# Qervas/cn_chess_ai

Measured on AMD Instinct MI355X. Metric: env steps/sec + DQN updates/sec at 8192 parallel games, 1/2/4/8 MI355X, higher is better.
Workload: dtype f32

## Files before the change

### cn_chess_ai_amd/csrc/xq_dqn.hip

```cpp
#include "xq_internal.h"
#include <hip/hip_ext.h>
#include "xq_gemm.hip.h"
#include "xq_screen.hip.h"
#include "xq_gemm_dma.hip.h"
#include "xq_l0grad.hip.h"

#include <algorithm>
#include <cfloat>
#include <cmath>
#include <limits>
#include <mutex>
#include <random>
#include <unordered_map>

struct TdStep; struct ScreenPlan;
namespace xq {
struct TailArgs; struct ClipRecord; struct TdStatsRecord; struct ShadowJob;
struct Screen {
    int mode = XQ_QMAX_FULL;
    int refine_stage = -1;
    DevBuf<uint16_t> wb;
    DevBuf<uint16_t> ab;
    DevBuf<float> p1, p2;
    DevBuf<float> R, na;
    DevBuf<unsigned> wmax;
    int static_net = -1;
    DevBuf<unsigned long long> stats;
    int stat_blocks = 0;
    unsigned long long carry[2] = {0, 0};
    unsigned long long host_steps = 0, host_samples = 0;
    PinnedBuf<unsigned long long> guard_host;
    Event guard_ev;
    bool guard_pending = false;
    unsigned long long guard_samples = 0, guard_queued_at = 0;
    bool stage_whole = false;
    unsigned long long seen[3] = {0, 0, 0};
    int hold = 0;
    bool rebase = false;
    unsigned long long fallbacks = 0;
    void set_mode(int m) { mode = m; hold = 0; }
    void rows_rewritten(int net) { if (static_net == net) static_net = -1; }
    int reserve(int NO, int Hl, int n, const void* params, const void* acts);
    void totals_of(const unsigned long long* h, unsigned long long sums[2]) const;  int totals(unsigned long long sums[2]) const;
    void guard_decide(const unsigned long long totals[2]);  int guard_tick(bool* screened);  int guard_queue(int n, hipStream_t s);
    int shadow_job(const xq_dqn* d, int sel_net, int parity, hipStream_t s, ShadowJob* shadow);
    int plan(xq_dqn* d, const TdStep& s, ScreenPlan* P);
};
}
struct xq_dqn {
    int ns = 0, nl = 0;
    int L[XQ_MAX_LAYERS + 1] = {0};
    size_t nw = 0, nb = 0;
    size_t wo[XQ_MAX_LAYERS] = {0}, bo[XQ_MAX_LAYERS] = {0};
    double lr = 1e-3, gamma = 0.99;
    uint64_t seed = 0;
    xq::Stream stream;
    xq::Stream side;
    hipStream_t cur = nullptr;
    int ncu = 256;
    xq::Event ev_fork, ev_join, ev_delta;
    xq::Event ev_qmax;
    xq::DevBuf<float> params[2];
    uint64_t params_version = 0;
    int precision = XQ_PRECISION_F32;
    xq::DevBuf<uint16_t> params_bf[2];
    xq::DevBuf<uint16_t> acts_bf[XQ_MAX_LAYERS];
    xq::DevBuf<uint16_t> tacts_bf[2];
    xq::DevBuf<uint16_t> t2acts_bf[2];
    xq::DevBuf<uint16_t> sel_acts_bf[XQ_MAX_LAYERS];
    xq::DevBuf<uint16_t> deltas_bf[XQ_MAX_LAYERS];
    xq::DevBuf<float> t2acts[2];
    xq::DevBuf<int> partial_idx;
    xq::DevBuf<float> acts[XQ_MAX_LAYERS];
    xq::DevBuf<float> tacts[2];
    xq::DevBuf<float> deltas[XQ_MAX_LAYERS];
    xq::DevBuf<float> dsc;
    xq::DevBuf<int32_t> act_mb;
    xq::DevBuf<float> q90;
    xq::DevBuf<float> sel_acts[XQ_MAX_LAYERS];
    xq::DevBuf<float> sel_q90;
    struct SelKeep {
        xq::DevBuf<float> z1;  xq::DevBuf<uint32_t> prev_boards;
        bool valid = false;  const uint32_t* boards = nullptr;  int n = 0;
        int calls = 0;  bool pays = false;
    } sel_keep[2];
    void sel_invalidate() { sel_keep[0].valid = sel_keep[1].valid = false; }
    xq::DevBuf<float> qh_slabs[2];
    bool small_tiles = false;
    bool l0_derive = false;
    xq::Screen scr;
    xq::DevBuf<float> partial;
    xq::DevBuf<float> zmax;  xq::DevBuf<int> zidx;
    xq::DevBuf<float> qsa, yv, lossv;
    xq::DevBuf<uint32_t> gboards;
    int last_n = 0;
    xq::DevBuf<float> grads_td;  size_t n_grads_td = 0;
    size_t g_w0 = 0, g_wh[XQ_MAX_LAYERS] = {0}, g_wout = 0, g_bh[XQ_MAX_LAYERS] = {0}, g_bout = 0;
    xq::DevBuf<float> grads_full;
    int opt_kind = XQ_OPT_SGD;
    double opt_b1 = 0.9, opt_b2 = 0.999, opt_eps = 1e-8;
    uint64_t opt_t = 0;
    xq::DevBuf<float> adam_m, adam_v;
    double clip_max_norm = 0.0;
    xq::DevBuf<double> clip_partials;
    xq::DevBuf<xq::ClipRecord> clip_rec;
    double target_tau = 0.0;
    bool tgt_rest_synced = false;
    int loss_kind = XQ_LOSS_SQUARED;
    double loss_kappa = 1.0;
    float loss_kappa32 = 1.0f;
    xq::DevBuf<xq::TdStatsRecord> td_stats_rec;
    xq::DevBuf<float> slabs;
    xq::DevBuf<float> slabs_l0;
    xq::DevBuf<uint16_t> l0_planes;
    xq::DevBuf<uint16_t> l0_sel;
    bool l0_split_done = false;
    bool l0_sel_done = false;
    bool l0_mfma = true;
    xq_comm* comm = nullptr;
    bool fused_apply = false;
    struct PendingSlab { const float* src = nullptr; int nslabs = 0; long long stride = 0; };
    PendingSlab pend_w0, pend_hidden[XQ_MAX_LAYERS], pend_wout, pend_bout, pend_bh;
    xq::DevBuf<float> bias_work;
    xq::DevBuf<float> xdense, qfull, tfull;
    xq::DevBuf<uint32_t> hb;
    xq::DevBuf<int32_t> ha;  xq::DevBuf<float> hr;  xq::DevBuf<uint8_t> hd;
    xq::DevBuf<uint32_t> ns_boards, ns_next;
    xq::DevBuf<int32_t> ns_action, ns_m, ns_first, ns_last;
    xq::DevBuf<float> ns_reward;
    xq::DevBuf<uint8_t> ns_done;
    int nstep_rows = 0;
    xq::DevBuf<uint8_t> ns_flag;
    int mirror_rows = 0;
    xq::DevBuf<uint8_t> ns_cflag;
    int colour_swap_rows = 0;
    bool colour_swap_sided = false;
    int bootstrap = XQ_BOOTSTRAP_ALL;
    xq::DevBuf<float> z96, z96_slabs;
    xq::DevBuf<int> legal_nmoves;
    xq::DevBuf<uint8_t> hside, ns_side;
    int legal_rows = 0;
    int zero_sum = 0;
    int view = XQ_VIEW_ABSOLUTE;
    xq::DevBuf<uint8_t> ns_vflag, ns_vflag_next;
    int view_rows = 0;
    xq::Profiler prof;
    xq::TailArgs* tail = nullptr;
    bool tail_open = false;
    bool td_tail = true;
    int exchange_overlap = -1;
    bool late_gate = false;
    bool exch_calibrated = false, exch_late = false;
    double exch_allreduce_us = 0.0, exch_threshold_us = 0.0;
    size_t tail_lds = 0;  double tail_flops = 0, tail_bytes = 0;

    bool fused() const { return fused_apply && comm == nullptr; }
    bool bf16() const { return precision != XQ_PRECISION_F32; }
    bool bf16_bwd() const { return precision == XQ_PRECISION_BF16_FULL; }
    uint16_t* wl_bf(int net, int l) const { return params_bf[net] + (l == 0 ? 0 : (size_t)L[0] * L[1] + (wo[l] - wo[1])); }
    float* w0t(int net) const { return params[net]; }
    float* wrest(int net) const { return params[net] + (size_t)L[0] * L[1]; }
    float* wl(int net, int l) const { return l == 0 ? w0t(net) : wrest(net) + (wo[l] - wo[1]); }
    float* bl(int net, int l) const { return params[net] + nw + bo[l]; }
    int nout() const { return L[nl]; }
    int hlast() const { return L[nl - 1]; }
};

namespace xq {

Profiler* dqn_profiler(xq_dqn* d) { return &d->prof; }
int dqn_fused_apply(const xq_dqn* d) { return d->fused_apply ? 1 : 0; }
int dqn_view(const xq_dqn* d) { return d->view; }
xq_comm* dqn_comm(const xq_dqn* d) { return d->comm; }
hipStream_t dqn_stream(xq_dqn* d) { return d->stream; }
void dqn_shape(const xq_dqn* d, int* n_in, int* n_out) { *n_in = d->L[0]; *n_out = d->nout(); }
hipEvent_t dqn_qmax_event(xq_dqn* d) { return d->ev_qmax; }
uint64_t dqn_params_version(const xq_dqn* d) { return d->params_version; }

struct ProfScope {
    Profiler& p; hipStream_t s; int h; double flops, bytes;
    ProfScope(xq_dqn* d, const char* name, double fl, double by, bool attach = false) : p(d->prof), s(d->cur), flops(fl), bytes(by) {
        h = -1;
        if (!name || d->tail_open || !p.enabled) return;
        if (d->cur != d->stream && d->cur != d->side) {
            char nm[48];
            snprintf(nm, sizeof nm, "%s@select", name);
            h = p.begin(nm, s, attach);
        } else {
            h = p.begin(name, s, attach);
        }
    }
    hipEvent_t start() const { return h >= 0 ? p.recs[h].a : nullptr; }
    hipEvent_t stop() const { return h >= 0 ? p.recs[h].b : nullptr; }
    ~ProfScope() { p.end(h, s, flops, bytes); }
};

struct LaunchNow {
    xq_dqn* d; bool was_open;
    explicit LaunchNow(xq_dqn* d_) : d(d_), was_open(d_->tail_open) { d->tail_open = false; }
    ~LaunchNow() { d->tail_open = was_open; }
};
struct OnStream {
    xq_dqn* d; hipStream_t was;
    OnStream(xq_dqn* d_, hipStream_t s) : d(d_), was(d_->cur) { d->cur = s; }
    ~OnStream() { d->cur = was; }
};
struct SmallTiles {
    xq_dqn* d; bool was;
    SmallTiles(xq_dqn* d_, bool small) : d(d_), was(d_->small_tiles) { d->small_tiles = small; }
    ~SmallTiles() { d->small_tiles = was; }
};

}

#include "xq_l0.hip.h"
#include "xq_tail.hip.h"
#include "xq_refine.hip.h"
#include "xq_nstep.hip.h"
#include "xq_mirror.hip.h"
#include "xq_colour_swap.hip.h"
#include "xq_view.hip.h"
#include "xq_legal.hip.h"

namespace xq {

static inline int vec_ok(const void* p, long long ld) { return (((uintptr_t)p) % 16 == 0) && (ld % 4 == 0); }

template <int AL, int BL, int EPI, int DT = DT_F32>
static int launch_gemm(xq_dqn* d, GemmArgs g, int splits, const char* name, int* used_splits = nullptr, bool force_small = false) {
    if (used_splits) *used_splits = 0;
    if (g.M <= 0 || g.N <= 0 || g.K <= 0) return fail(XQ_ERR_INVALID_ARGUMENT, "empty GEMM %s (%d x %d x %d)", name, g.M, g.N, g.K);
    g.a_vec = vec_ok(g.A, g.lda);
    g.b_vec = vec_ok(g.B, g.ldb);
    if (splits < 1) splits = 1;
    g.k_chunk = round_up((g.K + splits - 1) / splits, GBK);
    splits = (g.K + g.k_chunk - 1) / g.k_chunk;
    if (splits < 1) splits = 1;
    const int groups = g.grouped > 1 ? g.grouped : 1;
    const long long t128 = (long long)((g.M + 127) / 128) * ((g.N + 127) / 128) * (g.grouped ? groups : splits);
    const bool big = (!force_small && !d->small_tiles && t128 >= 512);
    const double kk = DT == DT_BF16 ? 2.0 * g.K : (double)g.K;
    if (d->tail_open) {
        TailArgs& T = *d->tail;
        const bool is_delta = AL == L_KCONTIG && BL == L_MCONTIG && EPI == EPI_DELTA, is_grad = AL == L_MCONTIG && BL == L_MCONTIG && EPI == EPI_STORE;
        if (DT != DT_F32 || big || g.grouped || !(is_delta || is_grad) || (is_delta && (T.n_delta || splits != 1)) || (is_grad && T.n_grad))
            return fail(XQ_ERR_RUNTIME, "GEMM %s cannot join the fused tail launch", name);
        const int gx = (g.M + 63) / 64, gy = (g.N + 63) / 64;
        if (is_delta) { T.delta = g; T.delta_gx = gx; T.n_delta = gx * gy; }
        else { T.grad = g; T.grad_gx = gx; T.grad_gy = gy; T.n_grad = gx * gy * splits; }
        d->tail_flops += 2.0 * g.M * g.N * kk;
        d->tail_bytes += 4.0 * ((double)g.M * g.K + (double)g.N * g.K + (double)g.M * g.N);
        d->tail_lds = std::max(d->tail_lds, 2 * (size_t)g_tile_floats(64) * sizeof(float));
        if (used_splits) *used_splits = splits;
        return XQ_OK;
    }
    ProfScope ps(d, name, 2.0 * g.M * g.N * kk, 4.0 * ((double)g.M * g.K + (double)g.N * g.K + (double)g.M * g.N));
    if (g.grouped) {
        if (splits != 1) return fail(XQ_ERR_INVALID_ARGUMENT, "grouped GEMM cannot be split-K");
        if (groups > 3) return fail(XQ_ERR_INVALID_ARGUMENT, "at most 3 grouped products");
        for (int k = 0; k + 1 < groups; ++k) {
            g.b_vec = g.b_vec && vec_ok(g.Bx[k], g.ldb);
            g.a_vec = g.a_vec && vec_ok(g.Ax[k], g.lda);
        }
        ps.flops *= groups; ps.bytes *= groups;
    }
    const int gz = g.grouped ? groups : splits;
    if (big) {
        dim3 grid((g.M + 127) / 128, (g.N + 127) / 128, gz);
        hipLaunchKernelGGL((gemm_f32_kernel<AL, BL, EPI, 2, 2, DT>), grid, dim3(256), 0, d->cur, g);
    } else {
        dim3 grid((g.M + 63) / 64, (g.N + 63) / 64, gz);
        hipLaunchKernelGGL((gemm_f32_kernel<AL, BL, EPI, 1, 1, DT>), grid, dim3(256), 0, d->cur, g);
    }
    XQ_HIP(hipGetLastError());
    if (used_splits) *used_splits = splits;
    return XQ_OK;
}

static int ensure_max_dynamic_lds(const void* kernel, int bytes) {
    static std::mutex m;
    static std::unordered_map<const void*, int> granted;
    std::lock_guard<std::mutex> lock(m);
    int& have = granted[kernel];
    if (have >= bytes) return XQ_OK;
    XQ_HIP(hipFuncSetAttribute(kernel, hipFuncAttributeMaxDynamicSharedMemorySize, bytes));
    have = bytes;
    return XQ_OK;
}
template <class F> static int ensure_max_dynamic_lds(F* kernel, int bytes) { return ensure_max_dynamic_lds(reinterpret_cast<const void*>(kernel), bytes); }

template <int DT, int AL, int BL, int EPI, int TI, int TJ>
static int launch_dma_gemm(xq_dqn* d, const Bf16GemmArgs& g, int gz, const char* name) {
    constexpr int lds = bg_lds_bytes(TI, TJ);
    XQ_TRY(ensure_max_dynamic_lds(gemm_dma_kernel<DT, AL, BL, EPI, TI, TJ>, lds));
    const int groups = g.groups > 1 ? g.groups : 1;
    const double es = DT == DT_F32 ? 4.0 : 2.0;
    ProfScope ps(d, name, 2.0 * g.M * g.N * (double)g.K * groups, es * groups * ((double)g.M * g.K + (double)g.N * g.K + 2.0 * g.M * g.N));
    hipLaunchKernelGGL((gemm_dma_kernel<DT, AL, BL, EPI, TI, TJ>), dim3(g.M / (128 * TI), g.N / (64 * TJ), gz), dim3(512), lds, d->cur, g);
    XQ_HIP(hipGetLastError());
    return XQ_OK;
}
template <int AL, int BL, int EPI>
static int launch_bf16_gemm(xq_dqn* d, const Bf16GemmArgs& g, int gz, const char* name) {
    return launch_dma_gemm<DT_BF16, AL, BL, EPI, 2, 2>(d, g, gz, name);
}

template <class T> static int reserve_zeroed(DevBuf<T>& b, size_t count, hipStream_t s) {
    bool grew = false;
    XQ_TRY(b.reserve(count, &grew));
    if (grew) XQ_HIP(hipMemsetAsync(b, 0, count * sizeof(T), s));
    return XQ_OK;
}

static int ensure_capacity(xq_dqn* d, int n) {
    const size_t cap = (size_t)n;
    int maxh = 0;
    for (int l = 0; l + 1 < d->nl; ++l) maxh = std::max(maxh, d->L[l + 1]);
    for (int l = 0; l + 1 < d->nl; ++l) {
        XQ_TRY(d->acts[l].reserve(cap * d->L[l + 1]));
        XQ_TRY(d->deltas[l].reserve(cap * d->L[l + 1]));
    }
    for (auto& t : d->tacts) XQ_TRY(reserve_zeroed(t, (size_t)round_up(n, 128) * (size_t)maxh, d->stream));
    const int ntn = (d->nout() + 63) / 64;
    XQ_TRY(d->q90.reserve(cap * 96));
    XQ_TRY(d->partial.reserve((size_t)round_up(n, 512) * (size_t)ntn * 2));
    for (DevBuf<float>* b : {&d->qsa, &d->yv, &d->lossv, &d->dsc}) XQ_TRY(b->reserve(cap));
    XQ_TRY(d->act_mb.reserve(cap));
    XQ_TRY(d->zmax.reserve(cap * kReduceParts));
    XQ_TRY(d->zidx.reserve(cap * kReduceParts));
    return d->gboards.reserve(cap * kBoardWords);
}

static int ensure_ext_capacity(xq_dqn* d, int n, bool want_double) {
    int maxh = 0;
    for (int l = 0; l + 1 < d->nl; ++l) maxh = std::max(maxh, d->L[l + 1]);
    const size_t rows = (size_t)round_up(n, 512);
    if (d->bf16()) {
        for (int l = 0; l + 1 < d->nl; ++l) XQ_TRY(d->acts_bf[l].reserve(rows * d->L[l + 1]));
        for (int i = 0; i < 2; ++i) {
            XQ_TRY(reserve_zeroed(d->tacts_bf[i], rows * (size_t)maxh, d->stream));
            XQ_TRY(reserve_zeroed(d->t2acts_bf[i], rows * (size_t)maxh, d->stream));
        }
    }
    if (d->bf16_bwd())
        for (int l = 0; l + 1 < d->nl; ++l) XQ_TRY(d->deltas_bf[l].reserve(rows * d->L[l + 1]));
    if (want_double) {
        for (auto& t : d->t2acts) XQ_TRY(reserve_zeroed(t, rows * (size_t)maxh, d->stream));
        const int ntn = (d->nout() + 63) / 64;
        XQ_TRY(d->partial_idx.reserve(rows * (size_t)ntn * 2));
    }
    return XQ_OK;
}

static SlotSrc explicit_slots(const int32_t* slots) {
    SlotSrc s; memset(&s, 0, sizeof s); s.slots = slots; return s;
}

void Screen::totals_of(const unsigned long long* h, unsigned long long sums[2]) const {
    sums[0] = carry[0]; sums[1] = carry[1];
    for (int i = 0; i < stat_blocks; ++i) { sums[0] += h[2 * i]; sums[1] += h[2 * i + 1]; }
}
int Screen::totals(unsigned long long sums[2]) const {
    std::vector<unsigned long long> h((size_t)2 * stat_blocks);
    if (stat_blocks) {
        XQ_HIP(hipDeviceSynchronize());
        XQ_HIP(hipMemcpy(h.data(), stats, h.size() * sizeof(unsigned long long), hipMemcpyDeviceToHost));
    }
    totals_of(h.data(), sums);
    return XQ_OK;
}
int Screen::reserve(int NO, int Hl, int n, const void* params, const void* acts) {
    const size_t wrows = (size_t)round_up(NO, 128);
    bool grew = false;
    XQ_TRY(wb.reserve(wrows * Hl, &grew));
    if (grew) {
        XQ_HIP(hipMemset(wb, 0, wrows * Hl * sizeof(uint16_t)));
        static_net = -1;
    }
    grew = false;
    XQ_TRY(wmax.reserve(6, &grew));
    if (grew) XQ_HIP(hipMemset(wmax, 0, 6 * sizeof(unsigned)));
    XQ_TRY(guard_ev.create(hipEventDisableTiming));
    const size_t rows = (size_t)round_up(n, 512), G = (size_t)4 * ((NO + 127) / 128);
    grew = false;
    XQ_TRY(ab.reserve(rows * Hl, &grew));
    if (grew) XQ_HIP(hipMemset(ab, 0, rows * Hl * sizeof(uint16_t)));
    XQ_TRY(p1.reserve(G * rows, &grew));
    XQ_TRY(p2.reserve(G * rows, &grew));
    XQ_TRY(R.reserve((size_t)((NO + 63) / 64) * rows, &grew));
    XQ_TRY(na.reserve(rows, &grew));
    if (grew)
        if (const char* e = getenv("XQ_DEBUG_PTRS")) if (e[0] == '1')
            fprintf(stderr, "[xq] screening buffers: P1 %p P2 %p R %p ab %p na %p params %p acts %p\n", (void*)p1.p, (void*)p2.p,
                    (void*)R.p, (void*)ab.p, (void*)na.p, params, acts);
    const int blocks = (int)(rows / kRefineSamples);
    if (blocks > stat_blocks) {
        if (stat_blocks) {
            unsigned long long sums[2];
            XQ_TRY(totals(sums));
            carry[0] = sums[0]; carry[1] = sums[1];
            guard_pending = false;
        }
        stat_blocks = 0;
        XQ_TRY(stats.reserve((size_t)2 * blocks));
        XQ_HIP(hipMemset(stats, 0, stats.n * sizeof(unsigned long long)));
        XQ_TRY(guard_host.reserve((size_t)2 * blocks));
        memset(guard_host, 0, guard_host.n * sizeof(unsigned long long));
        stat_blocks = blocks;
    }
    return XQ_OK;
}

struct ChainJob {
    int net;
    const uint32_t* boards;
    float* const* outs;
    uint16_t* const* outs_bf;
    uint32_t* gathered;
    uint16_t* last_bf;
// ... 126 lines not shown
    if (njobs == 1 && jobs[0].sel_keep && !d->bf16() && !shadow && !src.implicit && !src.slots) XQ_TRY(l0_select_forward(d, jobs[0], n));
    else XQ_TRY(l0_forward(d, jobs, njobs, src, n, shadow));
    for (int l = 1; l + 1 < d->nl; ++l) XQ_TRY(hidden_forward(d, jobs, njobs, l, n, stop_ev));
    return XQ_OK;
}

static int head_slabs(xq_dqn* d, size_t floats, float** slab) {
    DevBuf<float>& b = d->qh_slabs[d->cur == d->stream ? 0 : 1];
    XQ_TRY(b.reserve(floats));
    *slab = b;
    return XQ_OK;
}
static int q_head_finish(xq_dqn* d, const float* slab, long long slab_stride, int nslabs, int n, int n_out, int nc, const float* bias, float* q, int ldq,
                         const char* name = nullptr) {
    ProfScope ps(d, name, (double)n * n_out * nslabs, 4.0 * n * n_out * (nslabs + 1));
    hipLaunchKernelGGL(q_head_finish_kernel, dim3((unsigned)(((long long)n * n_out + 255) / 256)), dim3(256), 0, d->cur, slab, slab_stride, nslabs, n, n_out, nc,
                       bias, q, ldq);
    XQ_HIP(hipGetLastError());
    return XQ_OK;
}

static int q_head(xq_dqn* d, int net, const float* a_last, int n, int n_out, float* q, int ldq, const char* name,
                  const uint16_t* a_last_bf = nullptr) {
    GemmArgs g; memset(&g, 0, sizeof g);
    g.M = n; g.N = n_out; g.bias = d->bl(net, d->nl - 1);
    if (a_last_bf) {
        g.K = d->hlast() / 2;
        g.A = reinterpret_cast<const float*>(a_last_bf); g.lda = d->hlast() / 2;
        g.B = reinterpret_cast<const float*>(d->wl_bf(net, d->nl - 1)); g.ldb = d->hlast() / 2;
        g.C = q; g.ldc = ldq;
        return launch_gemm<L_KCONTIG, L_KCONTIG, EPI_BIAS_TANH, DT_BF16>(d, g, 1, name);
    }
    g.K = d->hlast();
    g.A = a_last; g.lda = d->hlast();
    g.B = d->wl(net, d->nl - 1); g.ldb = d->hlast();
    g.libm_tanh = 1;
    if (n_out <= 96 && n >= 2048 && (g.K % 128) == 0) {
        const int nc = round_up(n_out, 4);
        const int nslabs = g.K / 64;
        const size_t need = (size_t)nslabs * n * nc;
        float* slab = nullptr;
        XQ_TRY(head_slabs(d, need, &slab));
        g.C = slab; g.ldc = nc; g.slab_stride = (long long)n * nc;
        XQ_TRY((launch_gemm<L_KCONTIG, L_KCONTIG, EPI_STORE>(d, g, nslabs, name, nullptr, true)));
        return q_head_finish(d, slab, g.slab_stride, nslabs, n, n_out, nc, g.bias, q, ldq);
    }
    g.C = q; g.ldc = ldq;
    return launch_gemm<L_KCONTIG, L_KCONTIG, EPI_BIAS_TANH>(d, g, 1, name);
}

static int ensure_select_capacity(xq_dqn* d, int n) {
    for (int l = 0; l + 1 < d->nl; ++l) XQ_TRY(d->sel_acts[l].reserve((size_t)n * d->L[l + 1]));
    XQ_TRY(d->sel_q90.reserve((size_t)n * 96));
    for (int l = 0; d->bf16() && l + 1 < d->nl; ++l) XQ_TRY(d->sel_acts_bf[l].reserve((size_t)round_up(n, 128) * d->L[l + 1]));
    return XQ_OK;
}

int dqn_q90_boards(xq_dqn* d, const uint32_t* boards_dev, int n, float** q90_dev, int* q_stride, hipStream_t on, QSource* qs) {
    if (d->nout() < 96) return fail(XQ_ERR_INVALID_ARGUMENT, "self-play select needs >= 96 outputs");
    if (qs) memset(qs, 0, sizeof *qs);
    float* outs[XQ_MAX_LAYERS];
    uint16_t* outs_bf[XQ_MAX_LAYERS] = {nullptr};
    const bool bf = d->bf16();
    if (on) XQ_TRY(ensure_select_capacity(d, n));
    else {
        XQ_TRY(ensure_capacity(d, n));
        XQ_TRY(ensure_ext_capacity(d, n, false));
    }
    chain_views(d, on ? d->sel_acts : d->acts, on ? d->sel_acts_bf : d->acts_bf, XQ_MAX_LAYERS, !bf, outs, outs_bf);
    float* q = on ? d->sel_q90 : d->q90;
    OnStream on_stream(d, on ? on : d->cur);
    SmallTiles small(d, on != nullptr);
    ChainJob job{XQ_NET_ONLINE, boards_dev, outs, outs_bf, nullptr};
    xq_dqn::SelKeep& K = d->sel_keep[on ? 1 : 0];
    K.calls += 1;
    const bool kept = d->l0_derive && !bf && (d->L[1] & 3) == 0 && (K.pays || K.calls >= 2);
    if (kept) {
        if ((size_t)n * d->L[1] > K.z1.n) K.valid = false;
        job.sel_keep = (K.valid && K.boards == boards_dev && K.n == n) ? 2 : 1;
        K.valid = false;
        XQ_TRY(K.z1.reserve((size_t)n * d->L[1]));
        XQ_TRY(K.prev_boards.reserve((size_t)n * kBoardWords));
    }
    const int Hl = d->hlast();
    const bool ride = !bf && d->nl >= 3 && n >= 2048 && (n & 63) == 0 && (Hl % 128) == 0 && (d->L[d->nl - 2] & 31) == 0 && d->nout() >= 128 &&
                      vec_ok(d->wl(XQ_NET_ONLINE, d->nl - 1), Hl) && vec_ok(d->wl(XQ_NET_ONLINE, d->nl - 2), d->L[d->nl - 2]);
    if (ride) {
        const int nslabs = Hl / 64;
        float* slab = nullptr;
        XQ_TRY(head_slabs(d, (size_t)nslabs * n * 96, &slab));
        job.head_slabs = slab;
        outs[d->nl - 2] = nullptr;
        XQ_TRY(chain_boards(d, &job, 1, explicit_slots(nullptr), n));
        if (qs) {
            qs->slabs = slab; qs->slab_stride = (long long)n * 96; qs->nslabs = nslabs; qs->bias = d->bl(XQ_NET_ONLINE, d->nl - 1);
            q = nullptr;
        } else XQ_TRY(q_head_finish(d, slab, (long long)n * 96, nslabs, n, 96, 96, d->bl(XQ_NET_ONLINE, d->nl - 1), q, 96, "gemm_q90_select"));
    } else {
        XQ_TRY(chain_boards(d, &job, 1, explicit_slots(nullptr), n));
        XQ_TRY(q_head(d, XQ_NET_ONLINE, outs[d->nl - 2], n, 96, q, 96, "gemm_q90_select", bf ? outs_bf[d->nl - 2] : nullptr));
    }
    if (kept) { K.valid = true; K.boards = boards_dev; K.n = n; }
    *q90_dev = q;
    *q_stride = 96;
    return XQ_OK;
}

static int check_reference_topology(const xq_dqn* d) {
    for (int l = d->nl - 2; l >= 0; --l) {
        const int inputSize = d->L[l + 1], outputSize = d->L[l];
        if (d->L[l + 2] < inputSize || outputSize < d->L[l + 1] ||
            d->wo[l + 1] + (size_t)(inputSize - 1) * outputSize + (size_t)(d->L[l + 1] - 1) >= d->nw)
            return fail(XQ_ERR_UNDEFINED_UPSTREAM,
                        "bug-compatible backprop reads out of bounds upstream for this topology (layer %d)", l);
    }
    return XQ_OK;
}

static bool l0_mfma_shape(const xq_dqn* d, int n) { return d->l0_mfma && (d->L[1] % 64) == 0 && n >= 256; }
static int l0_chunk_of(int n) { return n >= 16384 ? 2048 : 1024; }
static int ensure_l0_mfma(xq_dqn* d, int n) {
    const int H = d->L[1], chunk = l0_chunk_of(n), kpad = (n + chunk - 1) / chunk * chunk;
    XQ_TRY(reserve_zeroed(d->l0_planes, l0m_plane_elems(H, kpad), d->cur));
    return reserve_zeroed(d->l0_sel, l0sel_elems(kpad), d->cur);
}

static bool grad_bf16_ok(const xq_dqn* d, int M, int N, int K);
static int hidden_deltas(xq_dqn* d, int n, const float* dnext, int ld_next, int k_nz, int mode, int l_start = -1, int l_stop = 0) {
    const float* up = dnext;
    int ld_up = ld_next, nz = k_nz;
    if (l_start < 0) l_start = d->nl - 2;
    for (int l = l_start; l >= l_stop; --l) {
        GemmArgs g; memset(&g, 0, sizeof g);
        g.M = n; g.N = d->L[l + 1];
        const int kfull = (mode == XQ_BACKPROP_REFERENCE) ? d->L[l + 1] : d->L[l + 2];
        g.K = std::min(kfull, nz);
        if (d->bf16_bwd() && up == d->deltas[l + 1] && (n % kBgBM) == 0 && (g.N % kBgBN) == 0 && (g.K % kBgBK) == 0) {
            Bf16GemmArgs b; memset(&b, 0, sizeof b);
            b.M = n; b.N = g.N; b.K = g.K; b.k_chunk = b.K;
            b.A = d->deltas_bf[l + 1]; b.lda = ld_up;
            b.B = d->wl_bf(XQ_NET_ONLINE, l + 1); b.ldb = (mode == XQ_BACKPROP_REFERENCE) ? d->L[l] : d->L[l + 1];
            b.C = d->deltas[l]; b.ldc = d->L[l + 1];
            b.Cb = d->deltas_bf[l]; b.ldcb = d->L[l + 1];
            b.Hb = d->acts_bf[l]; b.ldh = d->L[l + 1];
            XQ_TRY((launch_bf16_gemm<L_KCONTIG, L_MCONTIG, BG_DELTA>(d, b, 1, "gemm_hidden_delta")));
            up = d->deltas[l]; ld_up = d->L[l + 1]; nz = d->L[l + 1];
            continue;
        }
        g.A = up; g.lda = ld_up;
        g.B = d->wrest(XQ_NET_ONLINE) + (d->wo[l + 1] - d->wo[1]);
        g.ldb = (mode == XQ_BACKPROP_REFERENCE) ? d->L[l] : d->L[l + 1];
        g.C = d->deltas[l]; g.ldc = d->L[l + 1];
        g.H = d->acts[l]; g.ldh = d->L[l + 1];
        if (l == 0 && l0_mfma_shape(d, n) && (n % l0_chunk_of(n)) == 0) {
            const long long t128 = (long long)((g.M + 127) / 128) * ((g.N + 127) / 128);
            if (d->small_tiles || t128 < 512) {
                XQ_TRY(ensure_l0_mfma(d, n));
                g.split_planes = d->l0_planes; g.split_ld = n; g.split_plane_stride = (long long)d->L[1] * n;
                d->l0_split_done = true;
            }
        }
        XQ_TRY((launch_gemm<L_KCONTIG, L_MCONTIG, EPI_DELTA>(d, g, 1, "gemm_hidden_delta")));
        if (d->bf16_bwd() && l >= 1) {
            const int k_below = std::min(mode == XQ_BACKPROP_REFERENCE ? d->L[l] : d->L[l + 1], d->L[l + 1]);
            const bool delta_below = (n % kBgBM) == 0 && (d->L[l] % kBgBN) == 0 && (k_below % kBgBK) == 0;
            if (delta_below || grad_bf16_ok(d, d->L[l + 1], d->L[l], n)) {
                hipLaunchKernelGGL(f32_to_bf16_kernel, dim3(std::min((n * d->L[l + 1] + 255) / 256, 1024)), dim3(256), 0, d->cur, d->deltas[l].p,
                                   d->deltas_bf[l].p, (long long)n * d->L[l + 1]);
                XQ_HIP(hipGetLastError());
            }
        }
        up = d->deltas[l]; ld_up = d->L[l + 1]; nz = d->L[l + 1];
    }
    return XQ_OK;
}

static int pick_splits(int M, int N, int K) {
    const int tiles = ((M + 63) / 64) * ((N + 63) / 64);
    int s = (512 + tiles - 1) / tiles;
    s = std::min(s, std::max(1, K / 128));
    return std::max(1, std::min(s, 32));
}

static bool grad_bf16_ok(const xq_dqn* d, int M, int N, int K) {
    return d->bf16_bwd() && (M % kBgBM) == 0 && (N % kBgBN) == 0 && K >= kBgBK && (K % kBgBK) == 0;
}
static int grad_splits(const xq_dqn* d, int M, int N, int K) {
    if (!grad_bf16_ok(d, M, N, K)) return pick_splits(M, N, K);
    const int tiles = (M / kBgBM) * (N / kBgBN);
    int s = std::max(1, d->ncu / tiles);
    s = std::min(s, 16);
    while (s > 1 && (K % (s * kBgBK)) != 0) --s;
    return s;
}

static int launch_reduce_slabs(xq_dqn* d, const float* slabs, int nslabs, long long len, float* dst) {
    ProfScope ps(d, "reduce_slabs", (double)nslabs * len, 4.0 * (nslabs + 1) * len);
    hipLaunchKernelGGL(reduce_slabs_kernel, dim3((unsigned)std::min<long long>((len + 255) / 256, 2048)), dim3(256), 0, d->cur, slabs, nslabs,
                       len, len, dst);
    XQ_HIP(hipGetLastError());
    return XQ_OK;
}

template <int AL>
static int grad_gemm(xq_dqn* d, GemmArgs g, float* dst, const char* name, float* slab_base = nullptr,
                     xq_dqn::PendingSlab* defer = nullptr, const uint16_t* a_bf = nullptr, const uint16_t* b_bf = nullptr) {
    const bool use_bf = AL == L_MCONTIG && a_bf && b_bf && grad_bf16_ok(d, g.M, g.N, g.K);
    const int splits = use_bf ? grad_splits(d, g.M, g.N, g.K) : pick_splits(g.M, g.N, g.K);
    const long long len = (long long)g.M * g.N;
    float* slabs = slab_base;
    if (splits > 1 && !slabs) { XQ_TRY(d->slabs.reserve((size_t)splits * (size_t)len)); slabs = d->slabs; }
    float* C = splits > 1 ? slabs : dst;
    const long long slab_stride = splits > 1 ? len : 0;
    int used = splits;
    if (use_bf) {
        Bf16GemmArgs b; memset(&b, 0, sizeof b);
        b.M = g.M; b.N = g.N; b.K = g.K; b.A = a_bf; b.lda = g.lda; b.B = b_bf; b.ldb = g.ldb; b.k_chunk = g.K / splits;
        b.C = C; b.ldc = g.N; b.slab_stride = slab_stride;
        XQ_TRY((launch_bf16_gemm<L_MCONTIG, L_MCONTIG, BG_STORE>(d, b, splits, name)));
    } else {
        g.C = C; g.ldc = g.N; g.slab_stride = slab_stride;
        XQ_TRY((launch_gemm<AL, L_MCONTIG, EPI_STORE>(d, g, splits, name, &used, true)));
    }
    if (splits <= 1) return XQ_OK;
    if (defer) { defer->src = slabs; defer->nslabs = used; defer->stride = len; return XQ_OK; }
    return launch_reduce_slabs(d, slabs, used, len, dst);
}

struct BiasJobs {
    ColsumJobs J;
    BiasJobs() { memset(&J, 0, sizeof J); }
    void add(const float* X, long long ld, int C, float* dst) {
        const int k = J.njobs++;
        J.X[k] = X; J.ld[k] = ld; J.C[k] = C; J.dst[k] = dst;
    }
};
static int bias_grads(xq_dqn* d, BiasJobs& bj, int n, xq_dqn::PendingSlab* defer = nullptr) {
    ColsumJobs& J = bj.J;
    if (J.njobs == 0) return XQ_OK;
    J.n = n;
    J.R = std::max(1, std::min(64, n / 64));
    J.rows_per = (n + J.R - 1) / J.R;
    long long off = 0;
    int maxc = 0;
    for (int k = 0; k < J.njobs; ++k) { J.poff[k] = off; off += J.C[k]; maxc = std::max(maxc, J.C[k]); }
    J.wld = off;
    off *= J.R;
    XQ_TRY(d->bias_work.reserve((size_t)off));
    J.work = d->bias_work;
    if (defer) { defer->src = J.work; defer->nslabs = J.R; defer->stride = J.wld; }
    double tot = 0;
    for (int k = 0; k < J.njobs; ++k) tot += (double)n * J.C[k];
    if (d->tail_open) {
        TailArgs& T = *d->tail;
        T.cj = J; T.cj_gx = (maxc + 63) / 64; T.cj_gy = J.R; T.n_colsum = T.cj_gx * T.cj_gy * J.njobs;
        d->tail_flops += tot; d->tail_bytes += 4.0 * tot;
        return XQ_OK;
    }
    ProfScope ps(d, "bias_grad_colsum", tot, 4.0 * tot);
    hipLaunchKernelGGL(colsum_partial_kernel, dim3((maxc + 63) / 64, J.R, J.njobs), dim3(256), 0, d->cur, J);
    XQ_HIP(hipGetLastError());
    if (defer) return XQ_OK;
    hipLaunchKernelGGL(colsum_final_kernel, dim3((maxc + 63) / 64, J.njobs), dim3(256), 0, d->cur, J);
    XQ_HIP(hipGetLastError());
    return XQ_OK;
}

struct L0SegShape { int HS, nsets; size_t lds; };
static L0SegShape l0_seg_shape(int H, int chunk) {
    L0SegShape s;
    s.HS = (H > 256 && H % 256 == 0) ? 256 : H;
    s.nsets = 4;
    while (s.nsets > 1 && (size_t)s.nsets * 14 * s.HS * sizeof(float) > 60 * 1024) s.nsets >>= 1;
    s.lds = (size_t)s.nsets * 14 * s.HS * sizeof(float) + (size_t)chunk * sizeof(uint16_t);
    return s;
}

static int l0_gradient(xq_dqn* d, int n, float* dst, xq_dqn::PendingSlab* defer) {
    const int H = d->L[1];
    const int chunk = l0_chunk_of(n);
    const int nchunks = (n + chunk - 1) / chunk;
    const long long len = (long long)kStateSize * H;
    float* out = dst;
    if (nchunks > 1) {
        XQ_TRY(d->slabs_l0.reserve((size_t)nchunks * (size_t)len));
        out = d->slabs_l0;
    }
    if (l0_mfma_shape(d, n)) {
        const int kpad = nchunks * chunk;
        XQ_TRY(ensure_l0_mfma(d, n));
        const size_t need_sel = l0sel_elems(kpad);
        const long long plane_stride = (long long)H * kpad;
        {
            LaunchNow now(d);
            if (!d->l0_sel_done) {
                ProfScope ps(d, "l0_sel_words", 0.0, (double)n * 48 + 2.0 * need_sel);
                hipLaunchKernelGGL(l0_sel_kernel, dim3(kpad / 64), dim3(256), 0, d->cur, d->gboards, n, kpad, d->l0_sel);
            }
            if (!d->l0_split_done) {
                ProfScope ps(d, "l0_delta_split", 8.0 * n * H, (double)n * H * 4 + 6.0 * H * kpad);
                hipLaunchKernelGGL(delta_split_kernel, dim3(kpad / 64, H / 64), dim3(256), 0, d->cur, d->deltas[0], n, H, d->l0_planes, plane_stride, kpad);
            }
            d->l0_sel_done = d->l0_split_done = false;
        }
        XQ_HIP(hipGetLastError());
        const size_t shmem = l0m_lds_bytes();
        const double fl = 2.0 * 80 * 16 * (double)H * kpad * 3, by = 6.0 * H * kpad + 2.0 * need_sel + 4.0 * nchunks * len;
        if (d->tail_open) {
            TailArgs& T = *d->tail;
            T.l0_n = n; T.l0_H = H; T.l0_chunk = chunk; T.l0_nch = nchunks; T.l0_partial = out;
            T.l0_sel = d->l0_sel; T.l0_planes = d->l0_planes; T.l0_plane_stride = plane_stride; T.l0_kpad = kpad; T.l0_ncb = H / kL0mCols;
            T.n_l0 = 4 * (H / kL0mCols) * nchunks;
            d->tail_flops += fl; d->tail_bytes += by;
            d->tail_lds = std::max(d->tail_lds, shmem);
        } else {
            ProfScope ps(d, "l0_grad_segsum", fl, by);
            XQ_TRY(ensure_max_dynamic_lds(l0_grad_mfma_kernel<0>, 64 * 1024));
            hipLaunchKernelGGL(l0_grad_mfma_kernel<0>, dim3(H / kL0mCols, 4, nchunks), dim3(256), shmem, d->cur, d->l0_sel, d->l0_planes, plane_stride,
                               kpad, H, chunk, out);
            XQ_HIP(hipGetLastError());
        }
    } else {
        ProfScope ps(d, "l0_grad_segsum", 2.0 * n * 32 * H, (double)n * (32.0 * H * 4 + 48) + 4.0 * nchunks * len);
        const L0SegShape shape = l0_seg_shape(H, chunk);
        const int HS = shape.HS, nsets = shape.nsets;
        const size_t shmem = shape.lds;
        if (d->tail_open) {
            TailArgs& T = *d->tail;
            T.l0_boards = d->gboards; T.l0_delta = d->deltas[0]; T.l0_n = n; T.l0_H = H; T.l0_HS = HS; T.l0_chunk = chunk; T.l0_nsets = nsets;
            T.l0_nch = nchunks; T.l0_partial = out; T.n_l0 = kSquares * nchunks * (H / HS);
            d->tail_flops += 2.0 * n * 32 * H; d->tail_bytes += (double)n * (32.0 * H * 4 + 48) + 4.0 * nchunks * len;
            d->tail_lds = std::max(d->tail_lds, shmem);
        } else {
        if (shmem > 48 * 1024) XQ_TRY(ensure_max_dynamic_lds(l0_grad_kernel, 64 * 1024));
        hipLaunchKernelGGL(l0_grad_kernel, dim3(kSquares, nchunks, H / HS), dim3(256), shmem, d->cur, d->gboards, d->deltas[0], n, H, HS,
                           chunk, nsets, out);
        XQ_HIP(hipGetLastError());
        }
    }
    if (nchunks <= 1) return XQ_OK;
    if (defer) { defer->src = d->slabs_l0; defer->nslabs = nchunks; defer->stride = len; return XQ_OK; }
    return launch_reduce_slabs(d, d->slabs_l0, nchunks, len, dst);
}

static unsigned seg_grid(SegTable& t, bool state, const SoftArgs* soft = nullptr) {
    long long mx = 0;
    for (int i = 0; i < t.nseg; ++i) {
        uintptr_t bits = (uintptr_t)t.dst[i] | (uintptr_t)t.src[i] | ((uintptr_t)t.dst_bf[i] << 1);
        if (soft) bits |= (uintptr_t)soft->tgt[i] | ((uintptr_t)soft->tgt_bf[i] << 1);
        t.vec4[i] = (bits & 15) == 0 && (t.len[i] & 3) == 0 && (t.nslabs[i] <= 0 || (t.stride[i] & 3) == 0) &&
                    (!state || (t.state_off[i] & 3) == 0);
        mx = std::max(mx, t.vec4[i] ? t.len[i] / 4 : t.len[i]);
    }
    return (unsigned)std::max<long long>(1, std::min<long long>((mx + 255) / 256, 1024));
}

static int sgd_apply(xq_dqn* d, SegTable t, double alpha, const ClipArgs* clip = nullptr, const SoftArgs* soft = nullptr) {
    const unsigned bx = seg_grid(t, false, soft);
    ProfScope ps(d, t.reduce_only ? "reduce_slabs" : "sgd_apply", 0, 0, true);
    if (soft && clip) hipExtLaunchKernelGGL(sgd_segments_clip_soft_kernel, dim3(bx, t.nseg), dim3(256), 0, d->cur, ps.start(), ps.stop(), 0, t, (float)alpha, *clip, *soft);
    else if (soft) hipExtLaunchKernelGGL(sgd_segments_soft_kernel, dim3(bx, t.nseg), dim3(256), 0, d->cur, ps.start(), ps.stop(), 0, t, (float)alpha, *soft);
    else if (clip) hipExtLaunchKernelGGL(sgd_segments_clip_kernel, dim3(bx, t.nseg), dim3(256), 0, d->cur, ps.start(), ps.stop(), 0, t, (float)alpha, *clip);
    else
    hipExtLaunchKernelGGL(sgd_segments_kernel, dim3(bx, t.nseg), dim3(256), 0, d->cur, ps.start(), ps.stop(), 0, t, (float)alpha);
    XQ_HIP(hipGetLastError());
    return XQ_OK;
}

static int adam_apply(xq_dqn* d, SegTable t, double lr, double grad_scale, const ClipArgs* clip = nullptr, const SoftArgs* soft = nullptr) {
    const unsigned bx = seg_grid(t, true, soft);
    d->opt_t += 1;
    const double tt = (double)d->opt_t;
    AdamArgs A;
    A.m = d->adam_m; A.v = d->adam_v;
    A.b1 = (float)d->opt_b1; A.omb1 = (float)(1.0 - d->opt_b1);
    A.b2 = (float)d->opt_b2; A.omb2 = (float)(1.0 - d->opt_b2);
    A.eps = (float)d->opt_eps;
    A.a = (float)(lr / (1.0 - std::pow(d->opt_b1, tt)));
    A.rbc2 = (float)(1.0 / std::sqrt(1.0 - std::pow(d->opt_b2, tt)));
    A.gs = (float)grad_scale;
    ProfScope ps(d, "adam_apply", 0, 0, true);
    if (soft && clip) hipExtLaunchKernelGGL(adam_segments_clip_soft_kernel, dim3(bx, t.nseg), dim3(256), 0, d->cur, ps.start(), ps.stop(), 0, t, A, *clip, *soft);
    else if (soft) hipExtLaunchKernelGGL(adam_segments_soft_kernel, dim3(bx, t.nseg), dim3(256), 0, d->cur, ps.start(), ps.stop(), 0, t, A, *soft);
    else if (clip) hipExtLaunchKernelGGL(adam_segments_clip_kernel, dim3(bx, t.nseg), dim3(256), 0, d->cur, ps.start(), ps.stop(), 0, t, A, *clip);
    else
    hipExtLaunchKernelGGL(adam_segments_kernel, dim3(bx, t.nseg), dim3(256), 0, d->cur, ps.start(), ps.stop(), 0, t, A);
    XQ_HIP(hipGetLastError());
    return XQ_OK;
}

static int grad_norm(xq_dqn* d, SegTable& t, double grad_scale, ClipArgs* C) {
    if (t.nseg * kNormBlocks > kNormMaxPartials) return fail(XQ_ERR_RUNTIME, "grad_norm: %d segments", t.nseg);
    float* G = d->grads_td;
    SegTable n = t;
    double bytes = 0;
    for (int i = 0; i < n.nseg; ++i) {
        n.dst[i] = G + n.state_off[i];
        n.dst_bf[i] = nullptr;
        bytes += 4.0 * n.len[i] * (n.nslabs[i] > 0 ? n.nslabs[i] + 1 : 1);
    }
    seg_grid(n, false);
    {
        ProfScope ps(d, "grad_norm", 0, bytes, true);
        hipExtLaunchKernelGGL(grad_norm_kernel, dim3(kNormBlocks, n.nseg), dim3(256), 0, d->cur, ps.start(), ps.stop(), 0, n, d->clip_partials.p);
        XQ_HIP(hipGetLastError());
    }
    for (int i = 0; i < t.nseg; ++i) { t.src[i] = G + t.state_off[i]; t.nslabs[i] = 0; t.stride[i] = 0; }
    C->partials = d->clip_partials; C->npart = t.nseg * kNormBlocks;
    C->max_norm = d->clip_max_norm; C->abs_scale = std::fabs(grad_scale);
    C->rec = d->clip_rec;
    return XQ_OK;
}

static void layout_td_grads(xq_dqn* d) {
    size_t off = 0;
    d->g_w0 = off; off += (size_t)d->L[0] * d->L[1];
    for (int l = 1; l + 1 < d->nl; ++l) { d->g_wh[l] = off; off += (size_t)d->L[l] * d->L[l + 1]; }
    d->g_wout = off; off += (size_t)96 * d->hlast();
    d->g_bout = off; off += 96;
    for (int l = 0; l + 1 < d->nl; ++l) { d->g_bh[l] = off; off += (size_t)d->L[l + 1]; }
    d->n_grads_td = off;
}
static bool td_step_pending(const xq_dqn* d) { return d->pend_w0.nslabs > 0 || d->pend_wout.nslabs > 0 || d->pend_bh.nslabs > 0; }
template <class F>
static void for_td_segments(xq_dqn* d, F f) {
    const bool bf = d->bf16();
    const int top = d->nl - 1;
    f(d->w0t(0), bf ? d->wl_bf(0, 0) : nullptr, d->g_w0, (long long)d->L[0] * d->L[1], d->pend_w0);
    for (int l = 1; l < top; ++l) f(d->wl(0, l), bf ? d->wl_bf(0, l) : nullptr, d->g_wh[l], (long long)d->L[l] * d->L[l + 1], d->pend_hidden[l]);
    f(d->wl(0, top), bf ? d->wl_bf(0, top) : nullptr, d->g_wout, 96LL * d->hlast(), d->pend_wout);
    f(d->bl(0, 0), (uint16_t*)nullptr, d->g_bh[0], (long long)d->bo[top], d->pend_bh);
    f(d->bl(0, top), (uint16_t*)nullptr, d->g_bout, 96LL, d->pend_bout);
}
static void soft_td_segments(const xq_dqn* d, SoftArgs* Z) {
    const bool bf = d->bf16();
    const int top = d->nl - 1;
    int k = 0;
    auto add = [&](float* t, uint16_t* tb) { Z->tgt[k] = t; Z->tgt_bf[k] = tb; ++k; };
    add(d->w0t(1), bf ? d->wl_bf(1, 0) : nullptr);
    for (int l = 1; l < top; ++l) add(d->wl(1, l), bf ? d->wl_bf(1, l) : nullptr);
    add(d->wl(1, top), bf ? d->wl_bf(1, top) : nullptr);
    add(d->bl(1, 0), nullptr);
    add(d->bl(1, top), nullptr);
}
enum class ParamWrite { ONLINE_WHOLE, TARGET_HOST, TARGET_COPY, TARGET_BLEND, TD_SEGMENTS, BF16_SHADOW };
static void params_written(xq_dqn* d, ParamWrite what) {
    d->params_version += 1;
    switch (what) {
    case ParamWrite::ONLINE_WHOLE:  d->scr.rows_rewritten(XQ_NET_ONLINE); d->sel_invalidate(); d->tgt_rest_synced = false; break;
    case ParamWrite::TARGET_HOST:   d->scr.rows_rewritten(XQ_NET_TARGET); d->tgt_rest_synced = false; break;
    case ParamWrite::TARGET_COPY:   d->scr.rows_rewritten(XQ_NET_TARGET); d->tgt_rest_synced = true; break;
    case ParamWrite::TARGET_BLEND:  d->scr.rows_rewritten(XQ_NET_TARGET); break;
    case ParamWrite::TD_SEGMENTS:   d->sel_invalidate(); for (auto& K : d->sel_keep) { K.pays = K.calls >= 2; K.calls = 0; } break;
    case ParamWrite::BF16_SHADOW:   break;
    }
}

static int soft_target_whole(xq_dqn* d, double tau) {
    const long long n = (long long)(d->nw + d->nb);
    const float* p = d->params[0];
    float* t = d->params[1];
    uint16_t* tb = d->bf16() ? d->params_bf[1].p : nullptr;
    const int vec = ((((uintptr_t)p | (uintptr_t)t) & 15) == 0 && ((uintptr_t)tb & 7) == 0) ? 1 : 0;
    const long long items = vec ? (n >> 2) + 3 : n;
    const unsigned blocks = (unsigned)std::max<long long>(1, std::min<long long>((items + 255) / 256, 2048));
    params_written(d, ParamWrite::TARGET_BLEND);
    ProfScope ps(d, "soft_target", 2.0 * n, 12.0 * n + (tb ? 2.0 * d->nw : 0.0), true);
    hipExtLaunchKernelGGL(soft_target_kernel, dim3(blocks), dim3(256), 0, d->cur, ps.start(), ps.stop(), 0, p, t, tb, n, (long long)d->nw,
                          (float)tau, vec);
    XQ_HIP(hipGetLastError());
    return XQ_OK;
}

int view_boards_launch(const uint32_t* boards_dev, const uint8_t* side_dev, const uint4* meta_dev, int n, uint32_t* out_dev,
                       hipStream_t stream) {
    if (!boards_dev || !out_dev || (!side_dev && !meta_dev) || n < 0) return fail(XQ_ERR_INVALID_ARGUMENT, "view_boards: bad argument");
    if (!n) return XQ_OK;
    hipLaunchKernelGGL(view_boards_kernel, dim3((n + 63) / 64), dim3(64), 0, stream, boards_dev, side_dev, meta_dev, n, out_dev);
    XQ_HIP(hipGetLastError());
    return XQ_OK;
}

}

using namespace xq;

extern "C" {

static int dqn_init(xq_dqn* d, const int* layer_sizes, int n_sizes, double learning_rate, double gamma, uint64_t seed,
                    void* hip_stream);
static int refresh_shadow(xq_dqn* d, int net);

int xq_dqn_create(const int* layer_sizes, int n_sizes, double learning_rate, double gamma, uint64_t seed, void* hip_stream,
                  xq_dqn** out) {
    if (!out || !layer_sizes) return fail(XQ_ERR_INVALID_ARGUMENT, "xq_dqn_create: null pointer");
    if (n_sizes < 2) return fail(XQ_ERR_INVALID_ARGUMENT, "NeuralNetwork must have at least two layers (input and output).");
    if (n_sizes < 3 || n_sizes > XQ_MAX_LAYERS + 1)
        return fail(XQ_ERR_INVALID_ARGUMENT, "xq_dqn supports 1..%d hidden layers (got %d sizes)", XQ_MAX_LAYERS - 1, n_sizes);
    for (int i = 0; i < n_sizes; ++i)
        if (layer_sizes[i] <= 0) return fail(XQ_ERR_INVALID_ARGUMENT, "layer size must be positive");
    int c = 0;
    XQ_TRY(xq_device_count(&c));
    if (c == 0) return fail(XQ_ERR_NO_DEVICE, "no HIP device: libxqhip has no CPU fallback");
    xq_dqn* d = new xq_dqn();
    const int rc = dqn_init(d, layer_sizes, n_sizes, learning_rate, gamma, seed, hip_stream);
    if (rc != XQ_OK) { xq_dqn_destroy(d); return rc; }
    *out = d;
    return XQ_OK;
}

static int dqn_init(xq_dqn* d, const int* layer_sizes, int n_sizes, double learning_rate, double gamma, uint64_t seed,
                    void* hip_stream) {
    d->ns = n_sizes; d->nl = n_sizes - 1;
    for (int i = 0; i < n_sizes; ++i) d->L[i] = layer_sizes[i];
    for (int l = 0; l < d->nl; ++l) {
        d->wo[l] = d->nw; d->bo[l] = d->nb;
        d->nw += (size_t)d->L[l] * d->L[l + 1];
        d->nb += (size_t)d->L[l + 1];
    }
    d->lr = learning_rate; d->gamma = gamma; d->seed = seed;
    XQ_TRY(d->stream.open(hip_stream));
    d->cur = d->stream;
    {
        hipDeviceProp_t prop; int dev = 0;
        if (hipGetDevice(&dev) == hipSuccess && hipGetDeviceProperties(&prop, dev) == hipSuccess && prop.multiProcessorCount > 0)
            d->ncu = prop.multiProcessorCount;
    }
    XQ_TRY(d->side.open_owned(hipStreamNonBlocking));
    for (Event* ev : {&d->ev_fork, &d->ev_join, &d->ev_delta, &d->ev_qmax}) XQ_TRY(ev->create(stream_event_flags()));
    int widest = 0;
    for (int i = 0; i < n_sizes; ++i) widest = std::max(widest, layer_sizes[i]);
    const size_t pad = (size_t)128 * widest;
    for (auto& p : d->params) {
        XQ_TRY(p.alloc(d->nw + d->nb + pad));
        XQ_HIP(hipMemsetAsync(p, 0, p.n * sizeof(float), d->stream));
    }
    layout_td_grads(d);
    XQ_TRY(d->grads_td.alloc(d->n_grads_td));
    XQ_HIP(hipMemsetAsync(d->grads_td, 0, d->n_grads_td * sizeof(float), d->stream));
    std::vector<double> w(d->nw), b(d->nb, 0.0);
    std::mt19937_64 gen(seed);
    std::uniform_real_distribution<double> dis(-0.05, 0.05);
    for (size_t i = 0; i < d->nw; ++i) w[i] = dis(gen);
    XQ_TRY(xq_dqn_set_params(d, XQ_NET_ONLINE, w.data(), b.data()));
    return xq_dqn_update_target(d);
}

int xq_dqn_destroy(xq_dqn* d) {
    if (!d) return XQ_OK;
    d->prof.collect();
    d->side.close();
    d->stream.close();
    delete d->tail;
    delete d;
    return XQ_OK;
}

int xq_dqn_stream(const xq_dqn* d, void** s) {
    if (!d || !s) return fail(XQ_ERR_INVALID_ARGUMENT, "null pointer");
    *s = (void*)(hipStream_t)d->stream;
    return XQ_OK;
}

int xq_dqn_num_params(const xq_dqn* d, size_t* nw, size_t* nb) {
    if (!d) return fail(XQ_ERR_INVALID_ARGUMENT, "null dqn");
    if (nw) *nw = d->nw;
    if (nb) *nb = d->nb;
    return XQ_OK;
}

int xq_dqn_set_params(xq_dqn* d, int net, const double* w, const double* b) {
    if (!d || !w || !b || net < 0 || net > 1) return fail(XQ_ERR_INVALID_ARGUMENT, "xq_dqn_set_params: bad argument");
    std::vector<float> p(d->nw + d->nb);
    const int L0 = d->L[0], L1 = d->L[1];
    for (int j = 0; j < L1; ++j)
        for (int i = 0; i < L0; ++i) p[(size_t)i * L1 + j] = (float)w[(size_t)j * L0 + i];
    for (size_t i = d->wo[1]; i < d->nw; ++i) p[i] = (float)w[i];
    for (size_t i = 0; i < d->nb; ++i) p[d->nw + i] = (float)b[i];
    XQ_HIP(hipStreamSynchronize(d->stream));
    params_written(d, net == XQ_NET_ONLINE ? ParamWrite::ONLINE_WHOLE : ParamWrite::TARGET_HOST);
    XQ_HIP(hipMemcpy(d->params[net], p.data(), p.size() * sizeof(float), hipMemcpyHostToDevice));
    XQ_TRY(refresh_shadow(d, net));
    XQ_HIP(hipStreamSynchronize(d->stream));
    return XQ_OK;
}

int xq_dqn_get_params(xq_dqn* d, int net, double* w, double* b) {
    if (!d || net < 0 || net > 1) return fail(XQ_ERR_INVALID_ARGUMENT, "xq_dqn_get_params: bad argument");
    std::vector<float> p(d->nw + d->nb);
    XQ_HIP(hipStreamSynchronize(d->stream));
    XQ_HIP(hipMemcpy(p.data(), d->params[net], p.size() * sizeof(float), hipMemcpyDeviceToHost));
    const int L0 = d->L[0], L1 = d->L[1];
    if (w) {
        for (int j = 0; j < L1; ++j)
            for (int i = 0; i < L0; ++i) w[(size_t)j * L0 + i] = (double)p[(size_t)i * L1 + j];
// ... 25 lines not shown
    if (!d) return fail(XQ_ERR_INVALID_ARGUMENT, "null dqn");
    d->l0_derive = on != 0;
    return XQ_OK;
}

int xq_dqn_set_l0_grad_mode(xq_dqn* d, int mode) {
    if (!d || (mode != 0 && mode != 1)) return fail(XQ_ERR_INVALID_ARGUMENT, "xq_dqn_set_l0_grad_mode: 0 (segmented sums) or 1 (matrix pipe)");
    d->l0_mfma = mode == 1;
    return XQ_OK;
}

int xq_dqn_set_refine_stage(xq_dqn* d, int mode) {
    if (!d || mode < -1 || mode > 1) return fail(XQ_ERR_INVALID_ARGUMENT, "xq_dqn_set_refine_stage: -1 (by the screen's counters), 0 (never) or 1 (whenever the launch has room)");
    d->scr.refine_stage = mode;
    return XQ_OK;
}

int xq_dqn_set_td_tail(xq_dqn* d, int on) {
    if (!d) return fail(XQ_ERR_INVALID_ARGUMENT, "null dqn");
    d->td_tail = on != 0;
    return XQ_OK;
}

int xq_dqn_set_exchange_overlap(xq_dqn* d, int mode) {
    if (!d || mode < -1 || mode > 1) return fail(XQ_ERR_INVALID_ARGUMENT, "xq_dqn_set_exchange_overlap: mode -1, 0 or 1");
    d->exchange_overlap = mode;
    return XQ_OK;
}

int xq_dqn_set_qmax_mode(xq_dqn* d, int mode) {
    if (!d || (mode != XQ_QMAX_FULL && mode != XQ_QMAX_SCREENED)) return fail(XQ_ERR_INVALID_ARGUMENT, "bad qmax mode");
    d->scr.set_mode(mode);
    return XQ_OK;
}

int xq_dqn_qmax_stats(xq_dqn* d, uint64_t stats[4]) {
    if (!d || !stats) return fail(XQ_ERR_INVALID_ARGUMENT, "null");
    unsigned long long h[2] = {0, 0};
    XQ_TRY(d->scr.totals(h));
    stats[0] = d->scr.host_steps; stats[1] = d->scr.host_samples; stats[2] = h[0]; stats[3] = h[1];
    return XQ_OK;
}

int xq_dqn_qmax_guard(xq_dqn* d, uint64_t* fallbacks, int* hold_steps_left) {
    if (!d) return fail(XQ_ERR_INVALID_ARGUMENT, "null dqn");
    if (fallbacks) *fallbacks = d->scr.fallbacks;
    if (hold_steps_left) *hold_steps_left = d->scr.hold;
    return XQ_OK;
}

int xq_dqn_set_precision(xq_dqn* d, int precision) {
    if (!d || (precision != XQ_PRECISION_F32 && precision != XQ_PRECISION_BF16 && precision != XQ_PRECISION_BF16_FULL))
        return fail(XQ_ERR_INVALID_ARGUMENT, "bad precision");
    if (td_step_pending(d))
        return fail(XQ_ERR_RUNTIME, "xq_dqn_set_precision: a TD step is waiting for its apply_grads");
    if (precision != XQ_PRECISION_F32) {
        for (int l = 1; l <= d->nl - 1; ++l)
            if (d->L[l] & 1) return fail(XQ_ERR_INVALID_ARGUMENT, "bf16 Q-net needs even hidden widths (layer %d has %d)", l, d->L[l]);
        int widest = 0;
        for (int i = 0; i < d->ns; ++i) widest = std::max(widest, d->L[i]);
        const size_t pad = (size_t)128 * widest;
        for (auto& p : d->params_bf) XQ_TRY(reserve_zeroed(p, d->nw + pad, d->stream));
    }
    d->precision = precision;
    params_written(d, ParamWrite::BF16_SHADOW);
    XQ_TRY(refresh_shadow(d, 0));
    return refresh_shadow(d, 1);
}

static int chain_dense(xq_dqn* d, int net, const float* x, int n, float* const* outs) {
    GemmArgs g; memset(&g, 0, sizeof g);
    g.M = n; g.N = d->L[1]; g.K = d->L[0];
    g.A = x; g.lda = d->L[0];
    g.B = d->w0t(net); g.ldb = d->L[1];
    g.C = outs[0]; g.ldc = d->L[1];
    g.bias = d->bl(net, 0);
    g.libm_tanh = !XQ_L0_FAST_TANH;
    XQ_TRY((launch_gemm<L_KCONTIG, L_MCONTIG, EPI_BIAS_TANH>(d, g, 1, "gemm_l0_dense_fwd")));
    const ChainJob job{net, nullptr, outs};
    bool aligned;
    for (int l = 1; l + 1 < d->nl; ++l)
        XQ_TRY((launch_gemm<L_KCONTIG, L_KCONTIG, EPI_BIAS_TANH>(d, hidden_f32_args(d, &job, 1, l, n, &aligned), 1, "gemm_hidden_fwd")));
    return XQ_OK;
}

static int upload_dense(xq_dqn* d, const double* src, size_t count, DevBuf<float>& dev) {
    XQ_TRY(dev.reserve(count));
    std::vector<float> tmp(count);
    for (size_t i = 0; i < count; ++i) tmp[i] = (float)src[i];
    XQ_HIP(hipStreamSynchronize(d->stream));
    XQ_HIP(hipMemcpy(dev, tmp.data(), count * sizeof(float), hipMemcpyHostToDevice));
    return XQ_OK;
}

int xq_dqn_forward(xq_dqn* d, int net, const double* states, int n, double* q_host) {
    if (!d || !states || !q_host || n <= 0 || net < 0 || net > 1)
        return fail(XQ_ERR_INVALID_ARGUMENT, "Input size does not match network input layer size.");
    XQ_TRY(ensure_capacity(d, n));
    XQ_TRY(upload_dense(d, states, (size_t)n * d->L[0], d->xdense));
    XQ_TRY(d->qfull.reserve((size_t)n * d->nout()));
    float* outs[XQ_MAX_LAYERS];
    for (int l = 0; l + 1 < d->nl; ++l) outs[l] = d->acts[l];
    XQ_TRY(chain_dense(d, net, d->xdense, n, outs));
    XQ_TRY(q_head(d, net, outs[d->nl - 2], n, d->nout(), d->qfull, d->nout(), "gemm_q_full"));
    std::vector<float> q((size_t)n * d->nout());
    XQ_HIP(hipMemcpyAsync(q.data(), d->qfull, q.size() * sizeof(float), hipMemcpyDeviceToHost, d->stream));
    XQ_HIP(hipStreamSynchronize(d->stream));
    for (size_t i = 0; i < q.size(); ++i) q_host[i] = (double)q[i];
    return XQ_OK;
}

int xq_dqn_forward_boards_dev(xq_dqn* d, int net, const uint32_t* boards_dev, int n, int n_out, float* q_dev, int ldq) {
    if (!d || !boards_dev || !q_dev || n <= 0 || net < 0 || net > 1 || n_out <= 0 || n_out > d->nout() || ldq < n_out)
        return fail(XQ_ERR_INVALID_ARGUMENT, "xq_dqn_forward_boards_dev: bad argument");
    XQ_TRY(ensure_capacity(d, n));
    XQ_TRY(ensure_ext_capacity(d, n, false));
    float* outs[XQ_MAX_LAYERS];
    uint16_t* outs_bf[XQ_MAX_LAYERS] = {nullptr};
    chain_views(d, d->acts, d->acts_bf, XQ_MAX_LAYERS, true, outs, outs_bf);
    ChainJob job{net, boards_dev, outs, outs_bf, nullptr};
    XQ_TRY(chain_boards(d, &job, 1, explicit_slots(nullptr), n));
    return q_head(d, net, outs[d->nl - 2], n, n_out, q_dev, ldq, n_out <= 96 ? "gemm_q90_select" : "gemm_q_full",
                  d->bf16() ? outs_bf[d->nl - 2] : nullptr);
}

int xq_dqn_select_q_dev(xq_dqn* d, const uint32_t* boards_dev, int n, float* q_dev) {
    if (!d || !boards_dev || !q_dev || n <= 0) return fail(XQ_ERR_INVALID_ARGUMENT, "xq_dqn_select_q_dev: bad argument");
    float* q = nullptr;
    int stride = 0;
    XQ_TRY(dqn_q90_boards(d, boards_dev, n, &q, &stride, nullptr, nullptr));
    XQ_HIP(hipMemcpyAsync(q_dev, q, (size_t)n * 96 * sizeof(float), hipMemcpyDeviceToDevice, d->stream));
    return XQ_OK;
}

int xq_dqn_backpropagate(xq_dqn* d, const double* states, const double* targets, int n, double lr, double grad_scale, int mode) {
    if (!d || !states || !targets || n <= 0) return fail(XQ_ERR_INVALID_ARGUMENT, "Input size does not match network input layer size.");
    if (mode != XQ_BACKPROP_REFERENCE && mode != XQ_BACKPROP_TEXTBOOK) return fail(XQ_ERR_INVALID_ARGUMENT, "bad backprop mode");
    if (mode == XQ_BACKPROP_REFERENCE) XQ_TRY(check_reference_topology(d));
    XQ_TRY(ensure_capacity(d, n));
    const int NO = d->nout();
    XQ_TRY(upload_dense(d, states, (size_t)n * d->L[0], d->xdense));
    XQ_TRY(upload_dense(d, targets, (size_t)n * NO, d->tfull));
    XQ_TRY(d->qfull.reserve((size_t)n * NO));
    XQ_TRY(d->grads_full.reserve(d->nw + d->nb));
    float* outs[XQ_MAX_LAYERS];
    for (int l = 0; l + 1 < d->nl; ++l) outs[l] = d->acts[l];
    XQ_TRY(chain_dense(d, XQ_NET_ONLINE, d->xdense, n, outs));
    XQ_TRY(q_head(d, XQ_NET_ONLINE, outs[d->nl - 2], n, NO, d->qfull, NO, "gemm_q_full"));
    const long long total = (long long)n * NO;
    hipLaunchKernelGGL(out_delta_dense_kernel, dim3((unsigned)std::min<long long>((total + 255) / 256, 4096)), dim3(256), 0,
                       d->cur, d->qfull, d->tfull, total, d->tfull);
    XQ_HIP(hipGetLastError());
    const float* dout = d->tfull;
    XQ_TRY(hidden_deltas(d, n, dout, NO, NO, mode));
    float* gw = d->grads_full;
    float* gb = d->grads_full + d->nw;
    BiasJobs bj;
    {
        GemmArgs g; memset(&g, 0, sizeof g);
        g.M = d->L[0]; g.N = d->L[1]; g.K = n;
        g.A = d->xdense; g.lda = d->L[0];
        g.B = d->deltas[0]; g.ldb = d->L[1];
        XQ_TRY((grad_gemm<L_MCONTIG>(d, g, gw, "gemm_grad_l0_dense")));
        bj.add(d->deltas[0], d->L[1], d->L[1], gb + d->bo[0]);
    }
    for (int l = 1; l < d->nl; ++l) {
        const float* dl = (l == d->nl - 1) ? dout : d->deltas[l];
        const int ldd = (l == d->nl - 1) ? NO : d->L[l + 1];
        GemmArgs g; memset(&g, 0, sizeof g);
        g.M = d->L[l + 1]; g.N = d->L[l]; g.K = n;
        g.A = dl; g.lda = ldd;
        g.B = d->acts[l - 1]; g.ldb = d->L[l];
        XQ_TRY((grad_gemm<L_MCONTIG>(d, g, gw + d->wo[l], "gemm_grad_dense")));
        bj.add(dl, ldd, d->L[l + 1], gb + d->bo[l]);
    }
    XQ_TRY(bias_grads(d, bj, n));
    SegTable t; memset(&t, 0, sizeof t);
    t.nseg = 1; t.dst[0] = d->params[0]; t.src[0] = d->grads_full; t.len[0] = (long long)(d->nw + d->nb);
    params_written(d, ParamWrite::ONLINE_WHOLE);
    XQ_TRY(sgd_apply(d, t, lr * grad_scale));
    XQ_TRY(refresh_shadow(d, XQ_NET_ONLINE));
    XQ_HIP(hipStreamSynchronize(d->stream));
    return XQ_OK;
}

struct PerOpts {
    const float* is_w; const float* is_wmax;
    float* prio; unsigned* pmax_live;
    float eps, alpha;
};
static int td_grads_impl(xq_dqn* d, const uint32_t* boards, const uint32_t* next_boards, const int32_t* action_to,
                         const float* reward, const uint8_t* done, SlotSrc slots, int n, int td_net, int mode, const PerOpts* per,
                         const float* discount = nullptr, const uint8_t* next_player = nullptr);

int xq_dqn_td_grads(xq_dqn* d, const uint32_t* boards, const uint32_t* next_boards, const int32_t* action_to,
                    const float* reward, const uint8_t* done, const int32_t* slots, int n, int td_net, int mode) {
    return td_grads_impl(d, boards, next_boards, action_to, reward, done, explicit_slots(slots), n, td_net, mode, nullptr);
}
int xq_dqn_td_grads_sided(xq_dqn* d, const uint32_t* boards, const uint32_t* next_boards, const int32_t* action_to,
                          const float* reward, const uint8_t* done, const uint8_t* next_player, const int32_t* slots, int n, int td_net, int mode) {
    if (!next_player) return fail(XQ_ERR_INVALID_ARGUMENT, "xq_dqn_td_grads_sided: null next_player");
    return td_grads_impl(d, boards, next_boards, action_to, reward, done, explicit_slots(slots), n, td_net, mode, nullptr, nullptr, next_player);
}


struct GradPlan {
    bool defer;
    int out_chunks;  long long len_out;  size_t out_lds;
    size_t off_out, off_h[XQ_MAX_LAYERS];
};
static const int kOutGradChunk = 256;
static int plan_gradients(xq_dqn* d, int n, bool defer, GradPlan* P) {
    const int Hl = d->hlast();
    memset(P, 0, sizeof *P);
    P->defer = defer;
    P->out_chunks = (n + kOutGradChunk - 1) / kOutGradChunk;
    P->len_out = 96LL * Hl + 96;
    P->out_lds = (size_t)16 * Hl * sizeof(float) + (size_t)kOutGradChunk * sizeof(uint16_t);
    if (P->out_lds > 64 * 1024 || (Hl & 3))
        return fail(XQ_ERR_INVALID_ARGUMENT, "last hidden layer width %d unsupported by the output-gradient kernel (multiple of 4, <= 960)", Hl);
    if (!l0_mfma_shape(d, n) && l0_seg_shape(d->L[1], l0_chunk_of(n)).lds > 64 * 1024)
        return fail(XQ_ERR_INVALID_ARGUMENT, "first hidden layer too wide for the layer-0 gradient kernel (%d)", d->L[1]);
    size_t need = 0;
    auto place = [&](int nslabs, size_t len) {
        const size_t floats = nslabs > 1 ? (size_t)nslabs * len : 0, at = defer ? need : 0;
        need = defer ? need + floats : std::max(need, floats);
        return at;
    };
    P->off_out = place(P->out_chunks, (size_t)P->len_out);
    for (int l = d->nl - 2; l >= 1; --l) P->off_h[l] = place(grad_splits(d, d->L[l + 1], d->L[l], n), (size_t)d->L[l + 1] * (size_t)d->L[l]);
    XQ_TRY(d->slabs.reserve(need));
    d->pend_w0 = d->pend_wout = d->pend_bout = d->pend_bh = xq_dqn::PendingSlab();
    for (auto& p : d->pend_hidden) p = xq_dqn::PendingSlab();
    return XQ_OK;
}

static int out_gradient(xq_dqn* d, const GradPlan& P, int n, const float* alast, float* G) {
    const int Hl = d->hlast(), nchunks = P.out_chunks;
    float* dst = G + d->g_wout;
    float* out = nchunks > 1 ? d->slabs + P.off_out : dst;
    const double fl = 2.0 * n * Hl, by = (double)n * (Hl * 4 + 8) + 4.0 * nchunks * P.len_out;
    if (d->tail_open) {
        TailArgs& T = *d->tail;
        T.og_act = d->act_mb; T.og_dsc = d->dsc; T.og_alast = alast; T.og_n = n; T.og_H = Hl; T.og_chunk = kOutGradChunk; T.og_partial = out;
        T.n_out = 24 * nchunks;
        d->tail_flops += fl; d->tail_bytes += by;
        d->tail_lds = std::max(d->tail_lds, P.out_lds);
    } else {
        ProfScope ps(d, "out_grad_segsum", fl, by);
        hipLaunchKernelGGL(out_grad_kernel, dim3(24, nchunks), dim3(256), P.out_lds, d->cur, d->act_mb, d->dsc, alast, n, Hl, kOutGradChunk, out);
        XQ_HIP(hipGetLastError());
    }
    if (nchunks <= 1) return XQ_OK;
    if (P.defer) {
        d->pend_wout.src = out; d->pend_wout.nslabs = nchunks; d->pend_wout.stride = P.len_out;
        d->pend_bout.src = out + 96LL * Hl; d->pend_bout.nslabs = nchunks; d->pend_bout.stride = P.len_out;
        return XQ_OK;
    }
    return launch_reduce_slabs(d, out, nchunks, P.len_out, dst);
}
static int hidden_weight_gradient(xq_dqn* d, const GradPlan& P, int l, int n, float* const* outs, float* G) {
    GemmArgs g; memset(&g, 0, sizeof g);
    g.M = d->L[l + 1]; g.N = d->L[l]; g.K = n;
    g.A = d->deltas[l]; g.lda = d->L[l + 1];
    g.B = outs[l - 1]; g.ldb = d->L[l];
    const bool bf = d->bf16_bwd();
    return grad_gemm<L_MCONTIG>(d, g, G + d->g_wh[l], "gemm_grad_hidden", d->slabs + P.off_h[l], P.defer ? &d->pend_hidden[l] : nullptr,
                                bf ? d->deltas_bf[l].p : nullptr, bf ? d->acts_bf[l - 1].p : nullptr);
}
static int hidden_bias_gradients(xq_dqn* d, const GradPlan& P, int n, float* G) {
    BiasJobs bj;
    for (int l = 0; l <= d->nl - 2; ++l) bj.add(d->deltas[l], d->L[l + 1], d->L[l + 1], G + d->g_bh[l]);
    return bias_grads(d, bj, n, P.defer ? &d->pend_bh : nullptr);
}

static int side_gradients(xq_dqn* d, const GradPlan& P, int n, float* const* outs, float* G) {
    const int nl = d->nl;
    XQ_TRY(out_gradient(d, P, n, outs[nl - 2], G));
    bool waited = false;
    for (int l = nl - 2; l >= 1; --l) {
        if (l < nl - 2 && !waited) { XQ_HIP(hipStreamWaitEvent(d->cur, d->ev_delta, 0)); waited = true; }
        XQ_TRY(hidden_weight_gradient(d, P, l, n, outs, G));
    }
    if (!waited) XQ_HIP(hipStreamWaitEvent(d->cur, d->ev_delta, 0));
    return hidden_bias_gradients(d, P, n, G);
}

struct TailGrid {
    xq_dqn* d;
    explicit TailGrid(xq_dqn* d_) : d(d_) {
        if (!d->tail) d->tail = new TailArgs();
        memset(d->tail, 0, sizeof(TailArgs));
        d->tail_open = true; d->tail_lds = 0; d->tail_flops = d->tail_bytes = 0;
    }
    ~TailGrid() { d->tail_open = false; }
    int launch(bool last, const char* name) {
        d->tail_open = false;
        const TailArgs& T = *d->tail;
        const long long total = (long long)T.n_l0 + T.n_grad + T.n_delta + T.n_out + T.n_colsum + T.n_sel;
        if (total <= 0) return XQ_OK;
        ProfScope ps(d, name, d->tail_flops, d->tail_bytes, true);
        const auto kern = last ? (T.l0_planes != nullptr ? td_tail_kernel<TAIL_L0 | TAIL_GRAD | TAIL_OUT | TAIL_COLSUM, true>
                                                         : td_tail_kernel<TAIL_L0 | TAIL_GRAD | TAIL_OUT | TAIL_COLSUM>)
                               : (T.n_sel ? td_tail_kernel<TAIL_GRAD | TAIL_DELTA | TAIL_OUT | TAIL_SEL> : td_tail_kernel<TAIL_GRAD | TAIL_DELTA | TAIL_OUT>);
        if (d->tail_lds > 48 * 1024) XQ_TRY(ensure_max_dynamic_lds(kern, 64 * 1024));
        hipExtLaunchKernelGGL(kern, dim3((unsigned)total), dim3(256), d->tail_lds, d->cur, ps.start(), ps.stop(), 0, T);
        XQ_HIP(hipGetLastError());
        return XQ_OK;
    }
};
static bool tail_eligible(xq_dqn* d, int n) {
    if (!d->td_tail || d->bf16()) return false;
    for (int l = 0; l + 2 < d->nl; ++l)
        if (!d->small_tiles && (long long)((n + 127) / 128) * ((d->L[l + 1] + 127) / 128) >= 512) return false;
    return true;
}
static int reduce_pending(xq_dqn* d) {
    SegTable t; memset(&t, 0, sizeof t);
    float* G = d->grads_td;
    int k = 0;
    for_td_segments(d, [&](float*, uint16_t*, size_t goff, long long len, xq_dqn::PendingSlab& p) {
        if (p.nslabs > 0) { t.dst[k] = G + goff; t.src[k] = p.src; t.len[k] = len; t.nslabs[k] = p.nslabs; t.stride[k] = p.stride; ++k; }
        p = xq_dqn::PendingSlab();
    });
    if (k == 0) return XQ_OK;
    t.nseg = k; t.reduce_only = 1;
    return sgd_apply(d, t, 0.0);
}
static int tail_launches(xq_dqn* d, int n, float* const* outs, float* G, int mode) {
    const int nl = d->nl;
    GradPlan P;
    XQ_TRY(plan_gradients(d, n, true, &P));
    const bool defer_grad = nl == 3;
    int waiting = -1;
    for (int l = nl - 3; l >= 0; --l) {
        TailGrid grid(d);
        XQ_TRY(hidden_deltas(d, n, d->deltas[l + 1], d->L[l + 2], d->L[l + 2], mode, l, l));
        if (defer_grad) { if (waiting >= 0) XQ_TRY(hidden_weight_gradient(d, P, waiting, n, outs, G)); waiting = l + 1; }
        else XQ_TRY(hidden_weight_gradient(d, P, l + 1, n, outs, G));
        if (l == nl - 3) XQ_TRY(out_gradient(d, P, n, outs[nl - 2], G));
        if (l == 0 && l0_mfma_shape(d, n)) {
            XQ_TRY(ensure_l0_mfma(d, n));
            TailArgs& T = *d->tail;
            const int chunk0 = l0_chunk_of(n), kpad = (n + chunk0 - 1) / chunk0 * chunk0;
            T.sel_boards = d->gboards; T.sel_n = n; T.sel_kpad = kpad; T.sel_out = d->l0_sel; T.n_sel = kpad / 64;
            d->tail_bytes += (double)n * 48 + 2.0 * l0sel_elems(kpad);
            d->tail_lds = std::max(d->tail_lds, (size_t)64 * 13 * sizeof(uint32_t));
            d->l0_sel_done = true;
        }
        XQ_TRY(grid.launch(false, "td_tail_deltas"));
    }
    TailGrid grid(d);
    XQ_TRY(l0_gradient(d, n, G + d->g_w0, &d->pend_w0));
    if (waiting >= 0) XQ_TRY(hidden_weight_gradient(d, P, waiting, n, outs, G));
    if (nl < 3) XQ_TRY(out_gradient(d, P, n, outs[nl - 2], G));
    XQ_TRY(hidden_bias_gradients(d, P, n, G));
    return grid.launch(true, "td_tail_l0");
}
static int tail_gradients(xq_dqn* d, int n, float* const* outs, float* G, int mode) {
    int rc = tail_launches(d, n, outs, G, mode);
    if (d->late_gate) {
        if (hipEventRecord(d->ev_qmax, d->stream) != hipSuccess && rc == XQ_OK) rc = fail(XQ_ERR_RUNTIME, "hipEventRecord failed");
    }
    if (rc == XQ_OK && !d->fused()) {
        rc = reduce_pending(d);
        if (rc == XQ_OK && d->comm) {
            ProfScope ps(d, "rccl_allreduce_grads", 0, 4.0 * d->n_grads_td);
            rc = comm_allreduce_on(d->comm, G, d->n_grads_td, d->stream);
        }
    }
    return rc;
}


struct ScreenPlan { bool screened, top2; int parity; ShadowJob shadow; };
struct TdStep {
    const int32_t* action_to; const float* reward; const uint8_t* done; SlotSrc slots; const PerOpts* per;
    const uint32_t* next_boards; const uint8_t* next_player; bool legal;
    float gamma;
    int n, mode, sel_net, nl, Hl, NO; bool dbl, bf;
    bool big_tiles;
    int n_partial;
    size_t bias_lds;
    ScreenPlan scr;
    float* outs[XQ_MAX_LAYERS]; uint16_t* outs_bf[XQ_MAX_LAYERS];
    float* touts[XQ_MAX_LAYERS]; uint16_t* touts_bf[XQ_MAX_LAYERS];
    float* t2outs[XQ_MAX_LAYERS]; uint16_t* t2outs_bf[XQ_MAX_LAYERS];
    const float* view; long long view_ld; int view_kmax;
};

void Screen::guard_decide(const unsigned long long h[2]) {
    const double ds = (double)(guard_samples - seen[0]);
    if (ds > 0 && ((double)(h[0] - seen[1]) > kScreenMaxPairs * ds || (double)(h[1] - seen[2]) > kScreenMaxWhole * ds)) {
        hold = kScreenHoldSteps;
        fallbacks += 1;
        rebase = true;
    }
    if (ds > 0) {
        const double share = (double)(h[1] - seen[2]) / ds;
        if (share > 0.25) stage_whole = true; else if (share < 0.10) stage_whole = false;
    }
    seen[0] = guard_samples; seen[1] = h[0]; seen[2] = h[1];
}
int Screen::guard_tick(bool* screened) {
    if (guard_pending && !rebase && host_steps % kScreenCheckEvery == 0 && host_steps != guard_queued_at) {
        XQ_HIP(hipEventSynchronize(guard_ev));
        guard_pending = false;
        unsigned long long h[2];
        totals_of(guard_host, h);
        guard_decide(h);
    }
    *screened = hold == 0;
    if (hold > 0) --hold;
    return XQ_OK;
}
int Screen::guard_queue(int n, hipStream_t s) {
    host_steps += 1; host_samples += (unsigned long long)n;
    const bool boundary = host_steps % kScreenCheckEvery == 0;
    if (rebase && guard_pending && boundary) {
        XQ_HIP(hipEventSynchronize(guard_ev));
        guard_pending = false; rebase = false;
        unsigned long long h[2];
        totals_of(guard_host, h);
        seen[0] = guard_samples; seen[1] = h[0]; seen[2] = h[1];
    }
    if ((boundary || rebase) && !guard_pending) {
// ... 126 lines not shown
    }
    return scr.guard_queue(n, d->cur);
}

static int qmax_exact(xq_dqn* d, const TdStep& s, bool bf_frag, bool gate_early) {
    const int n = s.n, NO = s.NO, Hl = s.Hl, nl = s.nl;
    const bool bf = s.bf, dbl = s.dbl;
    long long part_ld = n;
    int n_part = s.n_partial;
    if (bf && (Hl == 256 || Hl == 512) && n >= 1024) {
        ScreenArgs a; memset(&a, 0, sizeof a);
        a.W = d->wl_bf(s.sel_net, nl - 1); a.A = s.touts_bf[nl - 2]; a.a_frag = bf_frag ? 1 : 0; a.bias = d->bl(s.sel_net, nl - 1);
        a.P1 = d->partial; a.P2 = reinterpret_cast<float*>(d->partial_idx.p);
        screen_geometry(NO, n, Hl, d->ncu, a);
        part_ld = a.ldp = screen_padded_samples(n, Hl);
        n_part = 2 * a.nchunks;
        ProfScope ps(d, "gemm_qmax_rowmax", 2.0 * NO * (double)n * Hl, 2.0 * ((double)NO * Hl + (double)n * Hl) + 8.0 * n_part * n, true);
        XQ_TRY(launch_screen(d, a, dbl ? SCR_ARG : SCR_MAX, ps.start(), ps.stop()));
    } else {
        GemmArgs g; memset(&g, 0, sizeof g);
        g.M = NO; g.N = n;
        g.K = bf ? Hl / 2 : Hl; g.lda = g.ldb = g.K;
        g.A = bf ? reinterpret_cast<const float*>(d->wl_bf(s.sel_net, nl - 1)) : d->wl(s.sel_net, nl - 1);
        g.B = bf ? reinterpret_cast<const float*>(s.touts_bf[nl - 2]) : s.touts[nl - 2];
        g.bias = d->bl(s.sel_net, nl - 1);
        g.partial = d->partial;
        g.partial_idx = dbl ? d->partial_idx : nullptr;
        if (s.big_tiles && (g.K % GBK) == 0 && vec_ok(g.A, g.lda) && vec_ok(g.B, g.ldb) && s.bias_lds <= 40 * 1024) {
            const int tiles_m = (NO + 127) / 128, total = tiles_m * ((n + 127) / 128);
            const int grid = colmax_persistent_grid(d, g, tiles_m, total);
            ProfScope ps(d, "gemm_qmax_rowmax", 2.0 * g.M * g.N * Hl, (bf ? 2.0 : 4.0) * ((double)g.M * Hl + (double)g.N * Hl) + 8.0 * tiles_m * g.N);
            const auto kern = bf ? (dbl ? gemm_colmax_persistent_kernel<2, 2, DT_BF16, CM_ARG> : gemm_colmax_persistent_kernel<2, 2, DT_BF16, CM_MAX>)
                                 : (dbl ? gemm_colmax_persistent_kernel<2, 2, DT_F32, CM_ARG> : gemm_colmax_persistent_kernel<2, 2, DT_F32, CM_MAX>);
            hipLaunchKernelGGL(kern, dim3(grid), dim3(256), s.bias_lds, d->cur, g, tiles_m, total);
            XQ_HIP(hipGetLastError());
        } else if (bf) XQ_TRY((launch_gemm<L_KCONTIG, L_KCONTIG, EPI_COLMAX, DT_BF16>(d, g, 1, "gemm_qmax_rowmax")));
        else XQ_TRY((launch_gemm<L_KCONTIG, L_KCONTIG, EPI_COLMAX>(d, g, 1, "gemm_qmax_rowmax")));
    }
    if (!d->late_gate && !gate_early) XQ_HIP(hipEventRecord(d->ev_qmax, d->stream));
    {
        ProfScope ps(d, "colmax_reduce", (double)n * n_part, (dbl ? 8.0 : 4.0) * n * (n_part + kReduceParts));
        hipLaunchKernelGGL(colmax_reduce_kernel, dim3((n + 63) / 64, kReduceParts), dim3(256), 0, d->cur, d->partial,
                           dbl ? d->partial_idx : nullptr, n_part, n, part_ld, d->zmax, d->zidx);
        XQ_HIP(hipGetLastError());
    }
    return XQ_OK;
}

static int qmax_legal(xq_dqn* d, const TdStep& s, bool gate_early) {
    const int n = s.n, nl = s.nl, Hl = s.Hl;
    const int want = (n >= 2048 && (Hl % 128) == 0) ? std::min(Hl / 64, (int)kLegalMaxSlabs) : 1;
    const int nets = s.dbl ? 2 : 1;
    const long long slab_stride = (long long)n * 96;
    XQ_TRY(d->z96_slabs.reserve((size_t)nets * want * slab_stride));
    XQ_TRY(d->z96.reserve((size_t)slab_stride));
    XQ_TRY(d->legal_nmoves.reserve((size_t)n));
    int used[2] = {want, want};
    for (int k = 0; k < nets; ++k) {
        GemmArgs g; memset(&g, 0, sizeof g);
        g.M = n; g.N = 96; g.K = Hl;
        g.A = k == 0 ? s.touts[nl - 2] : s.t2outs[nl - 2]; g.lda = Hl;
        g.B = d->wl(k == 0 ? s.sel_net : XQ_NET_TARGET, nl - 1); g.ldb = Hl;
        g.C = d->z96_slabs + (size_t)k * want * slab_stride; g.ldc = 96; g.slab_stride = slab_stride;
        XQ_TRY((launch_gemm<L_KCONTIG, L_KCONTIG, EPI_STORE>(d, g, want, "gemm_legal_head", &used[k], true)));
    }
    if (used[0] < 1 || used[0] > want || (s.dbl && used[1] != used[0])) return fail(XQ_ERR_RUNTIME, "legal head: %d k-slabs for %d asked", used[0], want);
    LegalArgs A; memset(&A, 0, sizeof A);
    A.next_boards = s.next_boards; A.action_to = s.action_to; A.done = s.done; A.side = s.next_player;
    A.sel_slabs = d->z96_slabs; A.sel_bias = d->bl(s.sel_net, nl - 1);
    if (s.dbl) { A.ev_slabs = d->z96_slabs + (size_t)want * slab_stride; A.ev_bias = d->bl(XQ_NET_TARGET, nl - 1); }
    A.slab_stride = slab_stride; A.nslabs = used[0];
    A.z96 = d->z96; A.zmax = d->zmax; A.zidx = d->zidx; A.n_moves = d->legal_nmoves;
    A.no_move_zmax = d->zero_sum ? -__builtin_inff() : 0.f;
    ProfScope ps(d, "legal_qmax", 0.0, (double)n * (48 + 6 + 384.0 * nets * used[0] + 384 + 12), true);
    hipExtLaunchKernelGGL(legal_qmax_kernel, dim3((n + 3) / 4), dim3(256), 0, d->cur, ps.start(), ps.stop(), 0, A, s.slots, n);
    XQ_HIP(hipGetLastError());
    if (!d->late_gate && !gate_early) XQ_HIP(hipEventRecord(d->ev_qmax, d->stream));
    return XQ_OK;
}

static int td_delta(xq_dqn* d, const TdStep& s, int zparts) {
    const int n = s.n, nl = s.nl, Hl = s.Hl;
    const int lt = nl - 2;
    ProfScope ps(d, "td_target_delta", 4.0 * n * Hl, (double)n * (Hl * 16 + s.n_partial * 4));
    TdExtra X; memset(&X, 0, sizeof X);
    X.nout = s.NO;
    if (s.dbl && !s.legal) {
        X.double_dqn = 1; X.partial_idx = d->zidx;
        X.bout_t = d->bl(XQ_NET_TARGET, nl - 1);
        if (s.bf) { X.wout_t_bf = d->wl_bf(XQ_NET_TARGET, nl - 1); X.alast_t_bf = s.t2outs_bf[lt]; }
        else { X.wout_t = d->wl(XQ_NET_TARGET, nl - 1); X.alast_t = s.t2outs[lt]; }
    }
    if (s.bf) X.wout_bf = d->wl_bf(XQ_NET_ONLINE, nl - 1);
    if (d->bf16_bwd()) X.dtop_bf = d->deltas_bf[lt];
    if (const PerOpts* per = s.per) {
        X.is_w = per->is_w; X.is_wmax = per->is_wmax; X.prio = per->prio; X.pmax_live = per->pmax_live;
        X.per_eps = per->eps; X.per_alpha = per->alpha;
    }
    if (d->loss_kind == XQ_LOSS_HUBER)
        hipLaunchKernelGGL(td_delta_huber_kernel, dim3((n + 3) / 4), dim3(256), 0, d->cur, n, s.slots, s.action_to, s.reward, s.done,
                           s.outs[lt], Hl, d->wl(XQ_NET_ONLINE, nl - 1), d->bl(XQ_NET_ONLINE, nl - 1), d->zmax, zparts,
                           s.gamma, s.view, s.view_ld, s.view_kmax, d->deltas[lt], d->dsc, d->act_mb, d->qsa, d->yv, d->lossv, X,
                           d->loss_kappa32);
    else
        hipLaunchKernelGGL(td_delta_kernel, dim3((n + 3) / 4), dim3(256), 0, d->cur, n, s.slots, s.action_to, s.reward, s.done,
                           s.outs[lt], Hl, d->wl(XQ_NET_ONLINE, nl - 1), d->bl(XQ_NET_ONLINE, nl - 1), d->zmax, zparts,
                           s.gamma, s.view, s.view_ld, s.view_kmax, d->deltas[lt], d->dsc, d->act_mb, d->qsa, d->yv, d->lossv, X);
    XQ_HIP(hipGetLastError());
    return XQ_OK;
}

static int td_gradients_fork(xq_dqn* d, const TdStep& s) {
    const int n = s.n, nl = s.nl;
    float* G = d->grads_td;
    GradPlan P;
    XQ_TRY(plan_gradients(d, n, d->fused(), &P));
    xq_dqn::PendingSlab* defer_w0 = P.defer ? &d->pend_w0 : nullptr;
    XQ_HIP(hipEventRecord(d->ev_fork, d->stream));
    XQ_HIP(hipStreamWaitEvent(d->side, d->ev_fork, 0));
    if (nl >= 3) XQ_TRY(hidden_deltas(d, n, d->deltas[nl - 2], d->L[nl - 1], d->L[nl - 1], s.mode, nl - 3));
    XQ_HIP(hipEventRecord(d->ev_delta, d->stream));
    const size_t n0 = (size_t)d->L[0] * d->L[1];
    if (!d->comm) XQ_TRY(l0_gradient(d, n, G + d->g_w0, defer_w0));
    {
        OnStream side(d, d->side);
        XQ_TRY(side_gradients(d, P, n, s.outs, G));
    }
    if (d->comm) XQ_TRY(comm_allreduce_on(d->comm, G + n0, d->n_grads_td - n0, d->side));
    XQ_HIP(hipEventRecord(d->ev_join, d->side));
    if (d->comm) {
        XQ_TRY(l0_gradient(d, n, G + d->g_w0, defer_w0));
        XQ_TRY(comm_allreduce_on(d->comm, G, n0, d->stream));
    }
    XQ_HIP(hipStreamWaitEvent(d->stream, d->ev_join, 0));
    return XQ_OK;
}

static int td_grads_impl(xq_dqn* d, const uint32_t* boards, const uint32_t* next_boards, const int32_t* action_to,
                         const float* reward, const uint8_t* done, SlotSrc slots, int n, int td_net, int mode, const PerOpts* per,
                         const float* discount, const uint8_t* next_player) {
    if (!d || !boards || !next_boards || !action_to || !reward || !done || n <= 0)
        return fail(XQ_ERR_INVALID_ARGUMENT, "xq_dqn_td_grads: bad argument");
    if (td_net != XQ_TD_ONLINE_NET && td_net != XQ_TD_TARGET_NET && td_net != XQ_TD_DOUBLE) return fail(XQ_ERR_INVALID_ARGUMENT, "bad td_net");
    if (mode != XQ_BACKPROP_REFERENCE && mode != XQ_BACKPROP_TEXTBOOK) return fail(XQ_ERR_INVALID_ARGUMENT, "bad backprop mode");
    if (d->nout() < 96) return fail(XQ_ERR_INVALID_ARGUMENT, "TD path needs >= 96 outputs (action.to indexes outputs 0..89)");
    if (mode == XQ_BACKPROP_REFERENCE) XQ_TRY(check_reference_topology(d));
    const bool dbl = td_net == XQ_TD_DOUBLE, bf = d->bf16();
    const bool legal = d->bootstrap == XQ_BOOTSTRAP_LEGAL;
    if (legal && bf) return fail(XQ_ERR_INVALID_ARGUMENT, "the legal-move bootstrap needs an fp32 net (xq_dqn_set_precision)");
    if (legal && !next_player)
        return fail(XQ_ERR_INVALID_ARGUMENT, "the legal-move bootstrap needs the side to move in s': use xq_dqn_td_grads_sided / xq_dqn_td_update_host_sided");
    d->legal_rows = 0;
    d->l0_split_done = d->l0_sel_done = false;
    d->late_gate = d->comm != nullptr && tail_eligible(d, n) &&
                   (d->exchange_overlap == 1 ||
                    (d->exchange_overlap < 0 && (d->exch_calibrated ? d->exch_late : comm_world(d->comm) > 1)));
    XQ_TRY(ensure_capacity(d, n));
    XQ_TRY(ensure_ext_capacity(d, n, dbl));
    const int nl = d->nl, Hl = d->hlast(), NO = d->nout();
    if (bf && (Hl & 1)) return fail(XQ_ERR_INVALID_ARGUMENT, "bf16 Q-net needs even layer widths");
    TdStep s;
    s.action_to = action_to; s.reward = reward; s.done = done; s.slots = slots; s.per = per;
    s.next_boards = next_boards; s.next_player = next_player; s.legal = legal;
    s.gamma = discount ? *discount : d->zero_sum ? -(float)d->gamma : (float)d->gamma;
    d->nstep_rows = 0;
    d->mirror_rows = 0;
    d->colour_swap_rows = 0;
    d->view_rows = 0;
    s.n = n; s.mode = mode; s.nl = nl; s.Hl = Hl; s.NO = NO; s.dbl = dbl; s.bf = bf; s.sel_net = td_net == XQ_TD_TARGET_NET ? XQ_NET_TARGET : XQ_NET_ONLINE;
    chain_views(d, d->acts, d->acts_bf, XQ_MAX_LAYERS, true, s.outs, s.outs_bf);
    chain_views(d, d->tacts, d->tacts_bf, 2, !bf, s.touts, s.touts_bf);
    chain_views(d, d->t2acts, d->t2acts_bf, 2, !bf, s.t2outs, s.t2outs_bf);
    s.big_tiles = (long long)((NO + 127) / 128) * ((n + 127) / 128) >= 512;
    s.n_partial = 2 * (s.big_tiles ? (NO + 127) / 128 : (NO + 63) / 64);
    s.bias_lds = (size_t)((NO + 127) / 128) * 128 * sizeof(float);
    s.view = d->wrest(XQ_NET_ONLINE) + (d->wo[nl - 1] - d->wo[1]);
    s.view_ld = mode == XQ_BACKPROP_REFERENCE ? d->L[nl - 2] : d->L[nl - 1]; s.view_kmax = mode == XQ_BACKPROP_REFERENCE ? d->L[nl - 1] : NO;
    XQ_TRY(d->scr.plan(d, s, &s.scr));
    const bool screened = s.scr.screened;
    const bool bf_frag = bf && nl >= 3 && (Hl == 256 || Hl == 512) && n >= 1024 && (n % kBgBM) == 0 && (d->L[nl - 2] % kBgBK) == 0;
    ChainJob jobs[3] = {{XQ_NET_ONLINE, boards, s.outs, s.outs_bf, d->gboards, nullptr, false},
                        {s.sel_net, next_boards, s.touts, s.touts_bf, nullptr, screened ? d->scr.ab : nullptr, s.scr.top2 || bf_frag},
                        {XQ_NET_TARGET, next_boards, s.t2outs, s.t2outs_bf, nullptr, nullptr, false}};
    const bool gate_early = (screened || bf || legal) && !d->late_gate;
    hipEvent_t fork = gate_early ? d->ev_qmax : nullptr;
    XQ_TRY(chain_boards(d, jobs, dbl ? 3 : 2, slots, n, screened ? &s.scr.shadow : nullptr, &fork));
    if (fork) XQ_HIP(hipEventRecord(fork, d->stream));
    bool td_fused = false;
    if (legal) XQ_TRY(qmax_legal(d, s, gate_early));
    else if (screened) XQ_TRY(qmax_screened(d, s, &td_fused));
    else XQ_TRY(qmax_exact(d, s, bf_frag, gate_early));
    if (!td_fused) XQ_TRY(td_delta(d, s, legal || screened ? 1 : kReduceParts));
    d->last_n = n;
    if (legal) d->legal_rows = n;
    if (tail_eligible(d, n)) return tail_gradients(d, n, s.outs, d->grads_td, mode);
    return td_gradients_fork(d, s);
}

static const double kExchangeThresholdUs = 41.0;

int xq_dqn_calibrate_exchange(xq_dqn* d, double threshold_us, double* allreduce_us, int* late) {
    if (!d) return fail(XQ_ERR_INVALID_ARGUMENT, "null dqn");
    if (!d->comm) return fail(XQ_ERR_INVALID_ARGUMENT, "xq_dqn_calibrate_exchange: no communicator attached");
    if (d->n_grads_td == 0) layout_td_grads(d);
    DevBuf<float> scratch;
    XQ_TRY(scratch.alloc(d->n_grads_td));
    float ms = 0.f;
    const int reps = 20;
    {
        struct SyncOnExit {
            hipStream_t s;
            ~SyncOnExit() { (void)hipStreamSynchronize(s); }
        } drained{d->stream};
        Event e0, e1;
        XQ_HIP(hipMemsetAsync(scratch, 0, d->n_grads_td * sizeof(float), d->stream));
        XQ_TRY(e0.create(hipEventDefault));
        XQ_TRY(e1.create(hipEventDefault));
        for (int i = 0; i < 4; ++i) XQ_TRY(comm_allreduce_on(d->comm, scratch, d->n_grads_td, d->stream));
        XQ_HIP(hipEventRecord(e0, d->stream));
        for (int i = 0; i < reps; ++i) XQ_TRY(comm_allreduce_on(d->comm, scratch, d->n_grads_td, d->stream));
        XQ_HIP(hipEventRecord(e1, d->stream));
        XQ_HIP(hipEventSynchronize(e1));
        XQ_HIP(hipEventElapsedTime(&ms, e0, e1));
    }
    uint64_t ns = (uint64_t)((double)ms * 1e6 / reps + 0.5);
    if (ns == 0) ns = 1;
    XQ_TRY(xq_comm_sum_u64(d->comm, &ns));
    d->exch_allreduce_us = (double)ns / 1e3 / (double)comm_world(d->comm);
    d->exch_threshold_us = threshold_us >= 0.0 ? threshold_us : kExchangeThresholdUs;
    d->exch_late = d->exch_allreduce_us > d->exch_threshold_us;
    d->exch_calibrated = true;
    if (allreduce_us) *allreduce_us = d->exch_allreduce_us;
    if (late) *late = d->exch_late ? 1 : 0;
    return XQ_OK;
}

int xq_dqn_exchange_calibration(const xq_dqn* d, int* calibrated, double* allreduce_us, double* threshold_us, int* late) {
    if (!d) return fail(XQ_ERR_INVALID_ARGUMENT, "null dqn");
    if (calibrated) *calibrated = d->exch_calibrated ? 1 : 0;
    if (allreduce_us) *allreduce_us = d->exch_allreduce_us;
    if (threshold_us) *threshold_us = d->exch_threshold_us;
    if (late) *late = d->exch_late ? 1 : 0;
    return XQ_OK;
}

int xq_dqn_set_comm(xq_dqn* d, xq_comm* comm) {
    if (!d) return fail(XQ_ERR_INVALID_ARGUMENT, "null dqn");
    if (td_step_pending(d))
        return fail(XQ_ERR_RUNTIME, "xq_dqn_set_comm: a TD step is waiting for its apply_grads");
    d->comm = comm;
    d->exch_calibrated = false;
    if (comm && comm_world(comm) > 1 && d->exchange_overlap < 0) XQ_TRY(xq_dqn_calibrate_exchange(d, -1.0, nullptr, nullptr));
    return XQ_OK;
}
int xq_allreduce_grads(xq_dqn* d, xq_comm* comm) {
    if (!d || !comm) return fail(XQ_ERR_INVALID_ARGUMENT, "null handle");
    if (td_step_pending(d))
        return fail(XQ_ERR_RUNTIME, "xq_allreduce_grads: gradient slabs are still unreduced (xq_dqn_set_fused_apply is on)");
    return comm_allreduce_on(comm, d->grads_td, d->n_grads_td, d->stream);
}

int xq_dqn_apply_grads(xq_dqn* d, double lr, double grad_scale) {
    if (!d) return fail(XQ_ERR_INVALID_ARGUMENT, "null dqn");
    SegTable t; memset(&t, 0, sizeof t);
    const float* G = d->grads_td;
    int k = 0;
    for_td_segments(d, [&](float* dst, uint16_t* dst_bf, size_t goff, long long len, xq_dqn::PendingSlab& p) {
        t.dst[k] = dst; t.dst_bf[k] = dst_bf; t.src[k] = G + goff; t.len[k] = len; t.state_off[k] = (long long)goff;
        if (p.nslabs > 0) { t.src[k] = p.src; t.nslabs[k] = p.nslabs; t.stride[k] = p.stride; }
        p = xq_dqn::PendingSlab();
        ++k;
    });
    t.nseg = k;
    params_written(d, ParamWrite::TD_SEGMENTS);
    ClipArgs C; memset(&C, 0, sizeof C);
    const bool clip = d->clip_max_norm > 0.0;
    if (clip) XQ_TRY(grad_norm(d, t, grad_scale, &C));
    const float tau32 = (float)d->target_tau;
    const bool soft = tau32 > 0.f && tau32 < 1.f;
    SoftArgs Z; memset(&Z, 0, sizeof Z);
    const bool fused_soft = soft && d->tgt_rest_synced;
    if (fused_soft) { soft_td_segments(d, &Z); Z.tau = tau32; }
    const SoftArgs* z = fused_soft ? &Z : nullptr;
    if (d->opt_kind == XQ_OPT_ADAM) XQ_TRY(adam_apply(d, t, lr, grad_scale, clip ? &C : nullptr, z));
    else XQ_TRY(sgd_apply(d, t, lr * grad_scale, clip ? &C : nullptr, z));
    if (soft && !fused_soft) return soft_target_whole(d, d->target_tau);
    if (tau32 == 1.f) return xq_dqn_update_target(d);
    return XQ_OK;
}

int xq_dqn_set_target_tau(xq_dqn* d, double tau) {
    if (!d) return fail(XQ_ERR_INVALID_ARGUMENT, "null dqn");
    if (!(tau >= 0.0 && tau <= 1.0)) return fail(XQ_ERR_INVALID_ARGUMENT, "xq_dqn_set_target_tau: tau must lie in [0, 1] (0 = off, 1 = the hard copy)");
    if (td_step_pending(d)) return fail(XQ_ERR_RUNTIME, "xq_dqn_set_target_tau: a TD step is waiting for its apply_grads");
    d->target_tau = tau;
    return XQ_OK;
}

int xq_dqn_get_target_tau(const xq_dqn* d, double* tau) {
    if (!d) return fail(XQ_ERR_INVALID_ARGUMENT, "null dqn");
    if (tau) *tau = d->target_tau;
    return XQ_OK;
}

int xq_dqn_soft_update_target(xq_dqn* d, double tau) {
    if (!d) return fail(XQ_ERR_INVALID_ARGUMENT, "null dqn");
// ... 686 lines not shown
```

### cn_chess_ai_amd/csrc/xq_gemm.hip.h

```cpp
#pragma once

#include "xq_common.h"

namespace xq {

typedef float f32x16 __attribute__((ext_vector_type(16)));
typedef float f32x4 __attribute__((ext_vector_type(4)));
typedef __bf16 bf16x8 __attribute__((ext_vector_type(8)));

enum { DT_F32 = 0, DT_BF16 = 1 };
__device__ __forceinline__ float bf16_round(float v) { return (float)(__bf16)v; }
__device__ __forceinline__ uint16_t bf16_bits(float v) { return __builtin_bit_cast(uint16_t, (__bf16)v); }
__device__ __forceinline__ float bf16_to_float(uint16_t b) { return __builtin_bit_cast(float, (uint32_t)b << 16); }
__device__ __forceinline__ float tanh_fast(float x) { return 1.f - 2.f * __frcp_rn(1.f + __expf(2.f * x)); }
#ifndef XQ_FAST_TANH
#define XQ_FAST_TANH 1
#endif
__device__ __forceinline__ float tanh_hidden(float x) {
#if XQ_FAST_TANH
    const float ax = fabsf(x);
    const float e = __builtin_amdgcn_exp2f(ax * 2.8853900817779268f);
    const float r = 1.f - 2.f * __builtin_amdgcn_rcpf(e + 1.f);
    const float x2 = ax * ax;
    const float p = ax * __builtin_fmaf(x2, __builtin_fmaf(x2, 0.13333334f, -0.33333334f), 1.f);
    return __builtin_copysignf(ax < 0.05f ? p : r, x);
#else
    return tanhf(x);
#endif
}

__host__ __device__ __forceinline__ long long scr_afrag_index(int sample, int k, int K) {
    return ((long long)((sample >> 5) * (K >> 4) + (k >> 4)) * 2 + ((k >> 3) & 1)) * 256 + (sample & 31) * 8 + (k & 7);
}

enum { L_KCONTIG = 0, L_MCONTIG = 1 };
enum { EPI_STORE = 0, EPI_BIAS_TANH = 1, EPI_COLMAX = 2, EPI_DELTA = 3, EPI_HEAD = 4 };

constexpr int GBK = 32;
constexpr int G_LDK = GBK + 4;
__host__ __device__ constexpr int g_tile_floats(int rows) { return rows * G_LDK > 32 * (rows + 4) ? rows * G_LDK : 32 * (rows + 4); }

struct GemmArgs {
    int M, N, K;
    const float* A; long long lda;
    const float* B; long long ldb;
    float* C; long long ldc;
    const float* bias;
    const float* H; long long ldh;
    float* partial;
    int k_chunk;
    long long slab_stride;
    int a_vec, b_vec;
    int grouped;
    const float* Ax[2]; const float* Bx[2]; float* Cx[2]; const float* biasx[2];
    uint16_t* Cb; long long ldcb; uint16_t* Cbx[2];
    int cb_frag;
    int* partial_idx;
    float* partial2;
    int bias_padded;
    int prio_split;
    int prio_tiles;
    const float* head_W; long long head_ldw; float* head_slabs; long long head_slab_stride; int head_ld;
    int libm_tanh;
    uint16_t* split_planes; long long split_plane_stride; int split_ld;
};

template <int LAYOUT, int ROWS, bool FAST, int J0 = 0, int J1 = ROWS / 32>
__device__ __forceinline__ void stage_load(const GemmArgs& g, const float* __restrict__ X, long long ld, int vec_ok,
                                           int rows0, int R, int k0, int kend, float4 (&v)[ROWS / 32]) {
    constexpr int NV = ROWS / 32;
    constexpr int TPR = ROWS / 4;
    constexpr int KPP = 256 / TPR;
    const int tid = (int)threadIdx.x & 255;
    if (FAST && LAYOUT == L_KCONTIG) {
        const float* p = X + (long long)(rows0 + (tid >> 3)) * ld + k0 + (tid & 7) * 4;
#pragma unroll
        for (int j = J0; j < J1; ++j) {
            const float4 x = *reinterpret_cast<const float4*>(p + (long long)(32 * j) * ld);
            v[j].x = x.x; v[j].y = x.y; v[j].z = x.z; v[j].w = x.w;
        }
        return;
    }
    if (FAST && LAYOUT == L_MCONTIG) {
        const float* p = X + (long long)(k0 + (tid / TPR)) * ld + rows0 + (tid % TPR) * 4;
#pragma unroll
        for (int j = J0; j < J1; ++j) {
            const float4 x = *reinterpret_cast<const float4*>(p + (long long)(KPP * j) * ld);
            v[j].x = x.x; v[j].y = x.y; v[j].z = x.z; v[j].w = x.w;
        }
        return;
    }
    if (LAYOUT == L_KCONTIG) {
        const int kq = (tid & 7) * 4;
        const int k = k0 + kq;
#pragma unroll
        for (int j = 0; j < NV; ++j) {
            const int row = rows0 + (tid >> 3) + 32 * j;
            float4 x = make_float4(0.f, 0.f, 0.f, 0.f);
            if (row < R) {
                const float* p = X + (long long)row * ld + k;
                if (vec_ok && k + 3 < kend) {
                    x = *reinterpret_cast<const float4*>(p);
                } else {
                    if (k + 0 < kend) x.x = p[0];
                    if (k + 1 < kend) x.y = p[1];
                    if (k + 2 < kend) x.z = p[2];
                    if (k + 3 < kend) x.w = p[3];
                }
            }
            v[j] = x;
        }
    } else if (LAYOUT == L_MCONTIG) {
        const int mq = (tid % TPR) * 4;
        const int row = rows0 + mq;
#pragma unroll
        for (int j = 0; j < NV; ++j) {
            const int k = k0 + (tid / TPR) + KPP * j;
            float4 x = make_float4(0.f, 0.f, 0.f, 0.f);
            if (k < kend) {
                const float* p = X + (long long)k * ld + row;
                if (vec_ok && row + 3 < R) {
                    x = *reinterpret_cast<const float4*>(p);
                } else {
                    if (row + 0 < R) x.x = p[0];
                    if (row + 1 < R) x.y = p[1];
                    if (row + 2 < R) x.z = p[2];
                    if (row + 3 < R) x.w = p[3];
                }
            }
            v[j] = x;
        }
    }
}

template <int LAYOUT, int ROWS>
__device__ __forceinline__ void stage_store(float* __restrict__ Xs, const float4 (&v)[ROWS / 32]) {
    constexpr int NV = ROWS / 32, TPR = ROWS / 4, KPP = 256 / TPR, LDM = ROWS + 4;
    const int tid = (int)threadIdx.x & 255;
    if (LAYOUT == L_KCONTIG) {
        const int kq = (tid & 7) * 4;
#pragma unroll
        for (int j = 0; j < NV; ++j) {
            const int row = (tid >> 3) + 32 * j;
            *reinterpret_cast<float4*>(&Xs[row * G_LDK + kq]) = v[j];
        }
    } else {
        const int mq = (tid % TPR) * 4;
#pragma unroll
        for (int j = 0; j < NV; ++j) {
            const int kr = (tid / TPR) + KPP * j;
            *reinterpret_cast<float4*>(&Xs[kr * LDM + mq]) = v[j];
        }
    }
}

template <int LAYOUT, int ROWS, int T>
__device__ __forceinline__ void frag_read(const float* __restrict__ Xs, int wbase, int c, int r, int h, float (&f)[T][4]) {
    constexpr int LDM = ROWS + 4;
    if (LAYOUT == L_KCONTIG) {
#pragma unroll
        for (int i = 0; i < T; ++i) {
            const float4 x = *reinterpret_cast<const float4*>(&Xs[(wbase + i * 32 + r) * G_LDK + c * 8 + 4 * h]);
            f[i][0] = x.x; f[i][1] = x.y; f[i][2] = x.z; f[i][3] = x.w;
        }
    } else {
#pragma unroll
        for (int i = 0; i < T; ++i)
#pragma unroll
            for (int t = 0; t < 4; ++t) f[i][t] = Xs[(c * 8 + 4 * h + t) * LDM + wbase + i * 32 + r];
    }
}

template <int TM, int TN, int DT>
__device__ __forceinline__ void chunk_mma(const float (&fa)[TM][4], const float (&fb)[TN][4], f32x16 (&acc)[TM][TN]) {
    if (DT == DT_BF16) {
#pragma unroll
        for (int i = 0; i < TM; ++i)
#pragma unroll
            for (int j = 0; j < TN; ++j) {
                const f32x4 a = {fa[i][0], fa[i][1], fa[i][2], fa[i][3]};
                const f32x4 b = {fb[j][0], fb[j][1], fb[j][2], fb[j][3]};
                acc[i][j] = __builtin_amdgcn_mfma_f32_32x32x16_bf16(__builtin_bit_cast(bf16x8, a), __builtin_bit_cast(bf16x8, b),
                                                                    acc[i][j], 0, 0, 0);
            }
    } else {
#pragma unroll
        for (int t = 0; t < 4; ++t)
#pragma unroll
            for (int i = 0; i < TM; ++i)
#pragma unroll
                for (int j = 0; j < TN; ++j)
                    acc[i][j] = __builtin_amdgcn_mfma_f32_32x32x2f32(fa[i][t], fb[j][t], acc[i][j], 0, 0, 0);
    }
}

template <int ASL, int BL, int BM, int BN, int TM, int TN, int DT = DT_F32>
__device__ __forceinline__ void tile_mma(const float* __restrict__ As, const float* __restrict__ Bs, int wm, int wn, int r, int h,
                                         f32x16 (&acc)[TM][TN]) {
    float fa0[TM][4], fb0[TN][4], fa1[TM][4], fb1[TN][4];
    frag_read<ASL, BM, TM>(As, wm * 32 * TM, 0, r, h, fa0);
    frag_read<BL, BN, TN>(Bs, wn * 32 * TN, 0, r, h, fb0);
#pragma unroll
    for (int c = 0; c < GBK / 8; c += 2) {
        frag_read<ASL, BM, TM>(As, wm * 32 * TM, c + 1, r, h, fa1);
        frag_read<BL, BN, TN>(Bs, wn * 32 * TN, c + 1, r, h, fb1);
        __builtin_amdgcn_sched_barrier(0);
        chunk_mma<TM, TN, DT>(fa0, fb0, acc);
        if (c + 2 < GBK / 8) {
            frag_read<ASL, BM, TM>(As, wm * 32 * TM, c + 2, r, h, fa0);
            frag_read<BL, BN, TN>(Bs, wn * 32 * TN, c + 2, r, h, fb0);
            __builtin_amdgcn_sched_barrier(0);
        }
        chunk_mma<TM, TN, DT>(fa1, fb1, acc);
    }
}

template <int AL, int BL, int TM, int TN, bool FAST, int DT = DT_F32>
__device__ __forceinline__ void gemm_mainloop(const GemmArgs& g, float* __restrict__ As, float* __restrict__ Bs, int m0, int n0,
                                              int kbeg, int kend, f32x16 (&acc)[TM][TN]) {
    constexpr int BM = 64 * TM, BN = 64 * TN;
    const int tid = (int)threadIdx.x & 255;
    const int lane = tid & 63, wid = tid >> 6;
    const int r = lane & 31, h = lane >> 5;
    const int wm = wid >> 1, wn = wid & 1;
    float4 va[BM / 32], vb[BN / 32];
    if (kbeg < kend) {
        stage_load<AL, BM, FAST>(g, g.A, g.lda, g.a_vec, m0, g.M, kbeg, kend, va);
        stage_load<BL, BN, FAST>(g, g.B, g.ldb, g.b_vec, n0, g.N, kbeg, kend, vb);
    }
    for (int k0 = kbeg; k0 < kend; k0 += GBK) {
        __syncthreads();
        stage_store<AL, BM>(As, va);
        stage_store<BL, BN>(Bs, vb);
        __syncthreads();
        if (k0 + GBK < kend) {
            stage_load<AL, BM, FAST>(g, g.A, g.lda, g.a_vec, m0, g.M, k0 + GBK, kend, va);
            stage_load<BL, BN, FAST>(g, g.B, g.ldb, g.b_vec, n0, g.N, k0 + GBK, kend, vb);
        }
        tile_mma<AL, BL, BM, BN, TM, TN, DT>(As, Bs, wm, wn, r, h, acc);
    }
}

template <int TM, int TN>
__device__ __forceinline__ void epilogue_colmax(const GemmArgs& g, const f32x16 (&acc)[TM][TN], int m0, int n0, int tile_m) {
    const int lane = (int)threadIdx.x & 63, wid = (int)threadIdx.x >> 6;
    const int r = lane & 31, h = lane >> 5;
    const int wm = wid >> 1, wn = wid & 1;
    const float NEG = -__builtin_inff();
    const bool want_idx = g.partial_idx != nullptr;
    float cm[TN];
    int ci[TN];
#pragma unroll
    for (int j = 0; j < TN; ++j) { cm[j] = NEG; ci[j] = 0x7fffffff; }
#pragma unroll
    for (int i = 0; i < TM; ++i) {
        const int mb = m0 + wm * 32 * TM + i * 32 + 4 * h;
        float bm[16];
        if (g.bias_padded) {
#pragma unroll
            for (int gq = 0; gq < 4; ++gq) {
                const float4 x = *reinterpret_cast<const float4*>(g.bias + mb + 8 * gq);
                bm[4 * gq] = x.x; bm[4 * gq + 1] = x.y; bm[4 * gq + 2] = x.z; bm[4 * gq + 3] = x.w;
            }
        } else {
#pragma unroll
            for (int q = 0; q < 16; ++q) { const int m = mb + (q & 3) + 8 * (q >> 2); bm[q] = g.bias[m < g.M ? m : g.M - 1]; }
        }
#pragma unroll
        for (int q = 0; q < 16; ++q) {
            const int row = mb + (q & 3) + 8 * (q >> 2);
            const bool ok = row < g.M;
#pragma unroll
            for (int j = 0; j < TN; ++j) {
                const float v = ok ? acc[i][j][q] + bm[q] : NEG;
                if (want_idx) { if (v > cm[j]) { cm[j] = v; ci[j] = row; } }
                else cm[j] = fmaxf(cm[j], v);
            }
        }
    }
#pragma unroll
    for (int j = 0; j < TN; ++j) {
        const float ov = __shfl_xor(cm[j], 32, 64);
        const int oi = __shfl_xor(ci[j], 32, 64);
        float v = fmaxf(cm[j], ov);
        int idx = ci[j];
        if (want_idx && (ov > cm[j] || (ov == cm[j] && oi < ci[j]))) idx = oi;
        const int n = n0 + wn * 32 * TN + j * 32 + r;
        if (h == 0 && n < g.N) {
            g.partial[((long long)tile_m * 2 + wm) * g.N + n] = v;
            if (want_idx) g.partial_idx[((long long)tile_m * 2 + wm) * g.N + n] = idx;
        }
    }
}

template <int AL, int BL, int EPI, int TM, int TN, int DT = DT_F32>
__device__ __forceinline__ void gemm_f32_block(const GemmArgs& g_in, int bx, int by, int bz, float* __restrict__ As, float* __restrict__ Bs) {
    constexpr int BM = 64 * TM, BN = 64 * TN;
    GemmArgs g = g_in;
    if (g_in.grouped && bz >= 1) {
        const int k = bz - 1;
        g.A = g_in.Ax[k]; g.B = g_in.Bx[k]; g.C = g_in.Cx[k]; g.bias = g_in.biasx[k]; g.Cb = g_in.Cbx[k];
    }

    const int tid = (int)threadIdx.x;
    const int lane = tid & 63, wid = tid >> 6;
    const int r = lane & 31, h = lane >> 5;
    const int wm = wid >> 1, wn = wid & 1;
    const int m0 = bx * BM, n0 = by * BN;
    const int kbeg = g.grouped ? 0 : bz * g.k_chunk;
    const int kend = min(g.K, kbeg + g.k_chunk);

    f32x16 acc[TM][TN];
#pragma unroll
    for (int i = 0; i < TM; ++i)
#pragma unroll
        for (int j = 0; j < TN; ++j)
#pragma unroll
            for (int q = 0; q < 16; ++q) acc[i][j][q] = 0.f;

    const bool interior = (m0 + BM <= g.M) && (n0 + BN <= g.N) && (((kend - kbeg) & (GBK - 1)) == 0) && g.a_vec && g.b_vec;
    if (interior) gemm_mainloop<AL, BL, TM, TN, true, DT>(g, As, Bs, m0, n0, kbeg, kend, acc);
    else gemm_mainloop<AL, BL, TM, TN, false, DT>(g, As, Bs, m0, n0, kbeg, kend, acc);

    if (EPI == EPI_COLMAX) {
        epilogue_colmax<TM, TN>(g, acc, m0, n0, bx);
        return;
    }
    if (EPI == EPI_HEAD) {
        float4 vb0[4], vb1[4];
        stage_load<L_KCONTIG, 128, true>(g, g.head_W, g.head_ldw, 1, 0, 128, n0, n0 + 64, vb0);
        stage_load<L_KCONTIG, 128, true>(g, g.head_W, g.head_ldw, 1, 0, 128, n0 + 32, n0 + 64, vb1);
        const int n = n0 + wn * 32 + r;
        const int mb = m0 + wm * 32 + 4 * h;
        const float bias = g.bias[n];
        float v[16];
#pragma unroll
        for (int q = 0; q < 16; ++q) {
            v[q] = tanh_hidden(acc[0][0][q] + bias);
            if (g.C) g.C[(long long)(mb + (q & 3) + 8 * (q >> 2)) * g.ldc + n] = v[q];
        }
        f32x16 hacc[1][2];
#pragma unroll
        for (int j = 0; j < 2; ++j)
#pragma unroll
            for (int q = 0; q < 16; ++q) hacc[0][j][q] = 0.f;
#pragma unroll
        for (int kt = 0; kt < 2; ++kt) {
            __syncthreads();
            if (wn == kt) {
#pragma unroll
                for (int q = 0; q < 16; ++q) As[(wm * 32 + 4 * h + (q & 3) + 8 * (q >> 2)) * G_LDK + r] = v[q];
            }
            stage_store<L_KCONTIG, 128>(Bs, kt == 0 ? vb0 : vb1);
            __syncthreads();
            tile_mma<L_KCONTIG, L_KCONTIG, 64, 128, 1, 2>(As, Bs, wm, wn, r, h, hacc);
        }
        float* slab = g.head_slabs + (long long)by * g.head_slab_stride;
#pragma unroll
        for (int j = 0; j < 2; ++j) {
            const int col = wn * 64 + j * 32 + r;
            if (col < g.head_ld) {
#pragma unroll
                for (int q = 0; q < 16; ++q) slab[(long long)(mb + (q & 3) + 8 * (q >> 2)) * g.head_ld + col] = hacc[0][j][q];
            }
        }
        return;
    }
    float* Cz = g.grouped ? g.C : g.C + (long long)bz * g.slab_stride;
    if (DT == DT_BF16 && EPI == EPI_BIAS_TANH) {
        if (g.Cb != nullptr && (m0 + BM <= g.M) && (n0 + BN <= g.N) && (g.ldcb & 7) == 0) {
            constexpr int WR = 32 * TM, WC = 32 * TN, S = WC + 8;
            __syncthreads();
            uint16_t* stage = reinterpret_cast<uint16_t*>(wid < 2 ? As : Bs) + (wid & 1) * WR * S;
#pragma unroll
            for (int i = 0; i < TM; ++i)
#pragma unroll
                for (int j = 0; j < TN; ++j) {
                    const int n = n0 + wn * WC + j * 32 + r;
                    const float bias = g.bias[n];
#pragma unroll
                    for (int q = 0; q < 16; ++q) {
                        const int row = i * 32 + (q & 3) + 8 * (q >> 2) + 4 * h;
                        const __bf16 rb = (__bf16)tanh_fast(acc[i][j][q] + bias);
                        stage[row * S + j * 32 + r] = __builtin_bit_cast(uint16_t, rb);
                        if (Cz) Cz[(long long)(m0 + wm * WR + row) * g.ldc + n] = (float)rb;
                    }
                }
            __builtin_amdgcn_fence(__ATOMIC_RELEASE, "wavefront");
            __builtin_amdgcn_wave_barrier();
            __builtin_amdgcn_fence(__ATOMIC_ACQUIRE, "wavefront");
            constexpr int PPR = WC / 8;
#pragma unroll
            for (int c = lane; c < WR * PPR; c += 64) {
                const int row = c / PPR, part = c % PPR;
                const uint4 x = *reinterpret_cast<const uint4*>(stage + row * S + part * 8);
                *reinterpret_cast<uint4*>(g.Cb + (long long)(m0 + wm * WR + row) * g.ldcb + n0 + wn * WC + part * 8) = x;
            }
            return;
        }
#pragma unroll
        for (int i = 0; i < TM; ++i)
#pragma unroll
            for (int j = 0; j < TN; ++j) {
                const int n = n0 + wn * 32 * TN + j * 32 + r;
                if (n >= g.N) continue;
                const float bias = g.bias[n];
#pragma unroll
                for (int q = 0; q < 16; ++q) {
                    const int m = m0 + wm * 32 * TM + i * 32 + (q & 3) + 8 * (q >> 2) + 4 * h;
                    if (m >= g.M) continue;
                    float v = g.Cb ? tanh_fast(acc[i][j][q] + bias) : tanhf(acc[i][j][q] + bias);
                    if (g.Cb) {
                        const __bf16 rb = (__bf16)v;
                        g.Cb[(long long)m * g.ldcb + n] = __builtin_bit_cast(uint16_t, rb);
                        v = (float)rb;
                    }
                    if (Cz) Cz[(long long)m * g.ldc + n] = v;
                }
            }
        return;
    }
    if ((m0 + BM <= g.M) && (n0 + BN <= g.N)) {
#pragma unroll
        for (int i = 0; i < TM; ++i)
#pragma unroll
            for (int j = 0; j < TN; ++j) {
                const int n = n0 + wn * 32 * TN + j * 32 + r;
                const int mb = m0 + wm * 32 * TM + i * 32 + 4 * h;
                float bias = 0.f;
                if (EPI == EPI_BIAS_TANH) bias = g.bias[n];
                float hv[16];
                if (EPI == EPI_DELTA) {
#pragma unroll
                    for (int q = 0; q < 16; ++q) hv[q] = g.H[(long long)(mb + (q & 3) + 8 * (q >> 2)) * g.ldh + n];
                }
#pragma unroll
                for (int q = 0; q < 16; ++q) {
                    float v = acc[i][j][q];
                    if (EPI == EPI_BIAS_TANH) v = g.libm_tanh ? tanhf(v + bias) : tanh_hidden(v + bias);
                    if (EPI == EPI_DELTA) v = v * (1.f - hv[q] * hv[q]);
                    Cz[(long long)(mb + (q & 3) + 8 * (q >> 2)) * g.ldc + n] = v;
                    if (EPI == EPI_BIAS_TANH && g.Cb) {
                        const int row = mb + (q & 3) + 8 * (q >> 2);
                        g.Cb[g.cb_frag ? scr_afrag_index(row, n, g.N) : (long long)row * g.ldcb + n] = bf16_bits(v);
                    }
                    if (EPI == EPI_DELTA) hv[q] = v;
                }
                if (EPI == EPI_DELTA && g.split_planes) {
                    const int m32 = m0 + wm * 32 * TM + i * 32;
                    uint32_t w[3][8];
#pragma unroll
                    for (int q = 0; q < 16; q += 2) {
                        uint32_t pk[3] = {0u, 0u, 0u};
#pragma unroll
                        for (int e = 0; e < 2; ++e) {
                            const float x = 0.5f * hv[q + e];
                            const uint16_t hi = bf16_bits(x);
                            const float r1 = x - bf16_to_float(hi);
                            const uint16_t mid = bf16_bits(r1);
                            const float r2 = r1 - bf16_to_float(mid);
                            const uint16_t lo = bf16_bits(r2);
                            pk[0] |= (uint32_t)hi << (16 * e); pk[1] |= (uint32_t)mid << (16 * e); pk[2] |= (uint32_t)lo << (16 * e);
                        }
                        w[0][q >> 1] = pk[0]; w[1][q >> 1] = pk[1]; w[2][q >> 1] = pk[2];
                    }
#pragma unroll
                    for (int t = 0; t < 3; ++t) {
                        uint4 o[2];
#pragma unroll
                        for (int half = 0; half < 2; ++half) {
                            const auto s0 = __builtin_amdgcn_permlane32_swap(w[t][4 * half], w[t][4 * half + 2], false, false);
                            const auto s1 = __builtin_amdgcn_permlane32_swap(w[t][4 * half + 1], w[t][4 * half + 3], false, false);
                            o[half] = make_uint4(s0[0], s1[0], s0[1], s1[1]);
                        }
                        uint16_t* dst = g.split_planes + t * g.split_plane_stride + (long long)n * g.split_ld + m32 + 8 * h;
                        *reinterpret_cast<uint4*>(dst) = o[0];
                        *reinterpret_cast<uint4*>(dst + 16) = o[1];
                    }
                }
            }
        return;
    }
#pragma unroll
    for (int i = 0; i < TM; ++i)
#pragma unroll
        for (int j = 0; j < TN; ++j) {
            const int n = n0 + wn * 32 * TN + j * 32 + r;
            if (n >= g.N) continue;
            float bias = 0.f;
            if (EPI == EPI_BIAS_TANH) bias = g.bias[n];
#pragma unroll
            for (int q = 0; q < 16; ++q) {
                const int m = m0 + wm * 32 * TM + i * 32 + (q & 3) + 8 * (q >> 2) + 4 * h;
                if (m >= g.M) continue;
                float v = acc[i][j][q];
                if (EPI == EPI_BIAS_TANH) v = g.libm_tanh ? tanhf(v + bias) : tanh_hidden(v + bias);
                if (EPI == EPI_DELTA) {
                    const float a = g.H[(long long)m * g.ldh + n];
                    v = v * (1.f - a * a);
                }
                Cz[(long long)m * g.ldc + n] = v;
                if (EPI == EPI_BIAS_TANH && g.Cb) g.Cb[g.cb_frag ? scr_afrag_index(m, n, g.N) : (long long)m * g.ldcb + n] = bf16_bits(v);
            }
        }
}

template <int AL, int BL, int EPI, int TM, int TN, int DT = DT_F32>
__global__ __launch_bounds__(256) __attribute__((amdgpu_waves_per_eu(1, 2))) void gemm_f32_kernel(const GemmArgs g_in) {
    __shared__ __attribute__((aligned(16))) float As[g_tile_floats(64 * TM)];
    __shared__ __attribute__((aligned(16))) float Bs[g_tile_floats(EPI == EPI_HEAD ? 128 : 64 * TN)];
    gemm_f32_block<AL, BL, EPI, TM, TN, DT>(g_in, (int)blockIdx.x, (int)blockIdx.y, (int)blockIdx.z, As, Bs);
}

enum { CM_MAX = 0, CM_ARG = 1, CM_TOP2 = 2 };
constexpr float kColmaxPadBias = -3.0e38f;

template <int TM, int TN, int DT = DT_F32, int MODE = CM_MAX>
__global__ __launch_bounds__(256) __attribute__((amdgpu_waves_per_eu(2, 2))) void gemm_colmax_persistent_kernel(const GemmArgs g,
                                                                                                        int tiles_m, int total) {
    constexpr int BM = 64 * TM, BN = 64 * TN;
    __shared__ __attribute__((aligned(16))) float As[g_tile_floats(BM)];
    __shared__ __attribute__((aligned(16))) float Bs[g_tile_floats(BN)];
    const int tid = (int)threadIdx.x;
    const int lane = tid & 63, wid = tid >> 6;
    const int r = lane & 31, h = lane >> 5;
    const int wm = wid >> 1, wn = wid & 1;
    int t, tend, stride;
    if (g.prio_split > 0) {
        const bool hi = (int)blockIdx.x >= g.prio_split;
        if (hi) __builtin_amdgcn_s_setprio(1);
        stride = hi ? (int)gridDim.x - g.prio_split : g.prio_split;
        t = hi ? (int)blockIdx.x - g.prio_split : g.prio_tiles + (int)blockIdx.x;
        tend = hi ? g.prio_tiles : total;
    } else {
        t = (int)blockIdx.x; tend = total; stride = (int)gridDim.x;
    }
    if (t >= tend) return;
    int tm = t % tiles_m, tn = t / tiles_m;
    float4 va[BM / 32], vb[BN / 32];
    extern __shared__ __attribute__((aligned(16))) float Bias_s[];
    stage_load<L_KCONTIG, BM, true>(g, g.A, g.lda, 1, tm * BM, g.M, 0, g.K, va);
    stage_load<L_KCONTIG, BN, true>(g, g.B, g.ldb, 1, tn * BN, g.N, 0, g.K, vb);
    if (g.bias_padded) {
        const int n4 = tiles_m * BM / 4, m4 = g.M / 4;
        const float NEGF = MODE == CM_TOP2 ? kColmaxPadBias : -__builtin_inff();
        for (int c0 = 0; c0 < n4; c0 += 256 * 8) {
            float4 bv[8];
#pragma unroll
            for (int u = 0; u < 8; ++u) bv[u] = reinterpret_cast<const float4*>(g.bias)[min(c0 + u * 256 + tid, m4 - 1)];
#pragma unroll
            for (int u = 0; u < 8; ++u) {
                const int idx = c0 + u * 256 + tid;
                if (idx < n4) reinterpret_cast<float4*>(Bias_s)[idx] = idx < m4 ? bv[u] : make_float4(NEGF, NEGF, NEGF, NEGF);
            }
        }
    } else {
        for (int m = tid; m < tiles_m * BM; m += 256) Bias_s[m] = m < g.M ? g.bias[m] : (MODE == CM_TOP2 ? kColmaxPadBias : -__builtin_inff());
    }
    for (;;) {
        f32x16 acc[TM][TN];
#pragma unroll
        for (int i = 0; i < TM; ++i)
#pragma unroll
            for (int j = 0; j < TN; ++j)
#pragma unroll
                for (int q = 0; q < 16; ++q) acc[i][j][q] = 0.f;
        const int tnext = t + stride;
        for (int k0 = 0; k0 < g.K; k0 += GBK) {
            __syncthreads();
            stage_store<L_KCONTIG, BM>(As, va);
            stage_store<L_KCONTIG, BN>(Bs, vb);
            __syncthreads();
            if (k0 + GBK < g.K) {
                stage_load<L_KCONTIG, BM, true>(g, g.A, g.lda, 1, tm * BM, g.M, k0 + GBK, g.K, va);
                stage_load<L_KCONTIG, BN, true>(g, g.B, g.ldb, 1, tn * BN, g.N, k0 + GBK, g.K, vb);
            } else if (tnext < tend) {
                stage_load<L_KCONTIG, BM, true>(g, g.A, g.lda, 1, (tnext % tiles_m) * BM, g.M, 0, g.K, va);
                stage_load<L_KCONTIG, BN, true>(g, g.B, g.ldb, 1, (tnext / tiles_m) * BN, g.N, 0, g.K, vb);
            }
            tile_mma<L_KCONTIG, L_KCONTIG, BM, BN, TM, TN, DT>(As, Bs, wm, wn, r, h, acc);
        }
        const float* bt = Bias_s + tm * BM + wm * 32 * TM + 4 * h;
        if (MODE == CM_TOP2) {
            static_assert(TM == 2, "the 5-bit position code assumes 32 rows per lane");
#pragma unroll
            for (int j = 0; j < TN; ++j) {
                float m1 = kColmaxPadBias, m2 = kColmaxPadBias;
#pragma unroll
                for (int i = 0; i < TM; ++i)
#pragma unroll
                    for (int gq = 0; gq < 4; ++gq) {
                        const float4 x = *reinterpret_cast<const float4*>(bt + i * 32 + 8 * gq);
                        const float bq[4] = {x.x, x.y, x.z, x.w};
#pragma unroll
                        for (int e = 0; e < 4; ++e) {
                            const uint32_t bits = __builtin_bit_cast(uint32_t, acc[i][j][4 * gq + e] + bq[e]);
                            const float v = __builtin_bit_cast(float, (bits & ~31u) | (uint32_t)(i * 16 + 4 * gq + e));
                            m2 = __builtin_amdgcn_fmed3f(m1, m2, v);
                            m1 = fmaxf(m1, v);
                        }
                    }
                const int n = tn * BN + wn * 32 * TN + j * 32 + r;
                if (n < g.N) {
                    const long long o = (((long long)tm * 2 + wm) * 2 + h) * g.N + n;
                    g.partial[o] = m1;
                    g.partial2[o] = m2;
                }
            }
        } else {
#pragma unroll
        for (int j = 0; j < TN; ++j) {
            float c = -__builtin_inff();
            int ci = 0x7fffffff;
            const int row0 = tm * BM + wm * 32 * TM + 4 * h;
#pragma unroll
            for (int i = 0; i < TM; ++i)
#pragma unroll
                for (int gq = 0; gq < 4; ++gq) {
                    const float4 x = *reinterpret_cast<const float4*>(bt + i * 32 + 8 * gq);
                    if (MODE == CM_ARG) {
                        const float v0 = acc[i][j][4 * gq] + x.x, v1 = acc[i][j][4 * gq + 1] + x.y;
                        const float v2 = acc[i][j][4 * gq + 2] + x.z, v3 = acc[i][j][4 * gq + 3] + x.w;
                        const int rb = row0 + i * 32 + 8 * gq;
                        if (v0 > c) { c = v0; ci = rb; }
                        if (v1 > c) { c = v1; ci = rb + 1; }
                        if (v2 > c) { c = v2; ci = rb + 2; }
                        if (v3 > c) { c = v3; ci = rb + 3; }
                    } else {
                        c = fmaxf(c, acc[i][j][4 * gq] + x.x); c = fmaxf(c, acc[i][j][4 * gq + 1] + x.y);
                        c = fmaxf(c, acc[i][j][4 * gq + 2] + x.z); c = fmaxf(c, acc[i][j][4 * gq + 3] + x.w);
                    }
                }
            const float oc = __shfl_xor(c, 32, 64);
            const int n = tn * BN + wn * 32 * TN + j * 32 + r;
            if (MODE == CM_ARG) {
                const int oi = __shfl_xor(ci, 32, 64);
                const bool take = oc > c || (oc == c && oi < ci);
                if (h == 0 && n < g.N) {
                    g.partial[((long long)tm * 2 + wm) * g.N + n] = take ? oc : c;
                    g.partial_idx[((long long)tm * 2 + wm) * g.N + n] = take ? oi : ci;
                }
            } else {
                c = fmaxf(c, oc);
                if (h == 0 && n < g.N) g.partial[((long long)tm * 2 + wm) * g.N + n] = c;
            }
        }
        }
        if (tnext >= tend) break;
        t = tnext; tm = t % tiles_m; tn = t / tiles_m;
    }
}

template <int TM, int TN, int WPE>
__global__ __launch_bounds__(256) __attribute__((amdgpu_waves_per_eu(WPE, WPE))) void gemm_fwd_persistent_kernel(const GemmArgs g, int tiles_m,
                                                                                                            int tiles_n, int total) {
    constexpr int BM = 64 * TM, BN = 64 * TN;
    __shared__ __attribute__((aligned(16))) float As[g_tile_floats(BM)];
    __shared__ __attribute__((aligned(16))) float Bs[g_tile_floats(BN)];
    const int tid = (int)threadIdx.x;
    const int lane = tid & 63, wid = tid >> 6;
    const int r = lane & 31, h = lane >> 5;
    const int wm = wid >> 1, wn = wid & 1;
    const int per_group = tiles_m * tiles_n;
    int t = (int)blockIdx.x;
// ... 64 lines not shown
```

### cn_chess_ai_amd/csrc/xq_tail.hip.h

```cpp
#pragma once

namespace xq {

enum { kReduceParts = 4 };
__global__ __launch_bounds__(256) void colmax_reduce_kernel(const float* __restrict__ partial_all, const int* __restrict__ partial_idx_all,
                                                            int n_partial_all, int n, long long ld, float* __restrict__ zmax_all,
                                                            int* __restrict__ zidx_all) {
    const int per = (n_partial_all + kReduceParts - 1) / kReduceParts;
    const int t0 = (int)blockIdx.y * per;
    const int n_partial = max(0, min(per, n_partial_all - t0));
    const float* partial = partial_all + (long long)t0 * ld;
    const int* partial_idx = partial_idx_all ? partial_idx_all + (long long)t0 * ld : nullptr;
    float* zmax = zmax_all + (long long)blockIdx.y * n;
    int* zidx = zidx_all + (long long)blockIdx.y * n;
    __shared__ float sv[4][64];
    __shared__ int si[4][64];
    const int lane = (int)(threadIdx.x & 63), wid = (int)(threadIdx.x >> 6);
    const int b = (int)blockIdx.x * 64 + lane;
    const bool ok = b < n;
    float m = -__builtin_inff();
    int mi = 0x7fffffff;
    const bool arg = partial_idx != nullptr;
    int t = wid;
    for (; t + 28 < n_partial; t += 32) {
// ... 176 lines not shown
        int bb[8], cl[8];
        float dl[8];
#pragma unroll
        for (int u = 0; u < 8; ++u) {
            const int e = list[i + 4 * u];
            bb[u] = c0 + (e & 2047); cl[u] = e >> 11;
            dl[u] = dsc[bb[u]];
        }
        for (int col = lane * 4; col < H; col += 256) {
            float4 v[8];
#pragma unroll
            for (int u = 0; u < 8; ++u) {
                const float4 x = *reinterpret_cast<const float4*>(a_last + (long long)bb[u] * H + col);
                v[u].x = x.x; v[u].y = x.y; v[u].z = x.z; v[u].w = x.w;
            }
#pragma unroll
            for (int u = 0; u < 8; ++u) {
                float4* a = reinterpret_cast<float4*>(my + cl[u] * H + col);
                float4 t = *a;
                t.x += dl[u] * v[u].x; t.y += dl[u] * v[u].y; t.z += dl[u] * v[u].z; t.w += dl[u] * v[u].w;
                *a = t;
            }
        }
#pragma unroll
        for (int u = 0; u < 8; ++u) {
            if (cl[u] == 0) bs0 += dl[u]; else if (cl[u] == 1) bs1 += dl[u]; else if (cl[u] == 2) bs2 += dl[u]; else bs3 += dl[u];
        }
    }
    for (; i < cnt; i += 4) {
        const int e = list[i];
        const int b = c0 + (e & 2047), cls = e >> 11;
        const float d1 = dsc[b];
        if (cls == 0) bs0 += d1; else if (cls == 1) bs1 += d1; else if (cls == 2) bs2 += d1; else bs3 += d1;
        for (int col = lane * 4; col < H; col += 256) {
            const float4 x = *reinterpret_cast<const float4*>(a_last + (long long)b * H + col);
            float4* a = reinterpret_cast<float4*>(my + cls * H + col);
            float4 t = *a;
            t.x += d1 * x.x; t.y += d1 * x.y; t.z += d1 * x.z; t.w += d1 * x.w;
            *a = t;
        }
    }
    if (lane == 0) { bsum[wid][0] = bs0; bsum[wid][1] = bs1; bsum[wid][2] = bs2; bsum[wid][3] = bs3; }
    __syncthreads();
    float* out = partial + (long long)chunk_id * (96LL * H + 96);
    for (int i = tid; i < 4 * H; i += 256)
        out[(long long)4 * g * H + i] = ((acc[i] + acc[4 * H + i]) + acc[8 * H + i]) + acc[12 * H + i];
    if (tid < 4) out[96LL * H + 4 * g + tid] = ((bsum[0][tid] + bsum[1][tid]) + bsum[2][tid]) + bsum[3][tid];
}
__global__ __launch_bounds__(256) void out_grad_kernel(const int32_t* __restrict__ act, const float* __restrict__ dsc,
                                                       const float* __restrict__ a_last, int n, int H, int chunk,
                                                       float* __restrict__ partial) {
    extern __shared__ __attribute__((aligned(16))) float smem[];
    out_grad_block(act, dsc, a_last, n, H, chunk, partial, (int)blockIdx.x, (int)blockIdx.y, smem);
}

__global__ void out_delta_dense_kernel(const float* __restrict__ q, const float* __restrict__ t, long long total, float* __restrict__ d) {
    for (long long i = (long long)blockIdx.x * blockDim.x + threadIdx.x; i < total; i += (long long)gridDim.x * blockDim.x) {
        const float a = q[i];
        d[i] = (a - t[i]) * (1.f - a * a);
    }
}

struct ColsumJobs {
    const float* X[XQ_MAX_LAYERS + 1];
    long long ld[XQ_MAX_LAYERS + 1];
    int C[XQ_MAX_LAYERS + 1];
    float* dst[XQ_MAX_LAYERS + 1];
    long long poff[XQ_MAX_LAYERS + 1];
    int njobs, n, rows_per, R;
    float* work;
    long long wld;
};
__device__ __forceinline__ void colsum_partial_block(const ColsumJobs& J, int bx, int by, int job) {
    __shared__ float red[4][64];
    const int C = J.C[job];
    const int tx = (int)(threadIdx.x & 63), ty = (int)(threadIdx.x >> 6);
    const int c = bx * 64 + tx;
    if (bx * 64 >= C) return;
    const float* X = J.X[job];
    const long long ld = J.ld[job];
    const int r0 = by * J.rows_per, r1 = min(J.n, r0 + J.rows_per);
    float s0 = 0.f, s1 = 0.f, s2 = 0.f, s3 = 0.f;
    if (c < C) {
        int r = r0 + ty;
        for (; r + 12 < r1; r += 16) {
            s0 += X[(long long)r * ld + c];
            s1 += X[(long long)(r + 4) * ld + c];
            s2 += X[(long long)(r + 8) * ld + c];
            s3 += X[(long long)(r + 12) * ld + c];
        }
        for (; r < r1; r += 4) s0 += X[(long long)r * ld + c];
    }
    red[ty][tx] = (s0 + s1) + (s2 + s3);
    __syncthreads();
    if (ty == 0 && c < C)
        J.work[J.poff[job] + (long long)by * J.wld + c] = (red[0][tx] + red[1][tx]) + (red[2][tx] + red[3][tx]);
}
__global__ __launch_bounds__(256) void colsum_partial_kernel(ColsumJobs J) {
    colsum_partial_block(J, (int)blockIdx.x, (int)blockIdx.y, (int)blockIdx.z);
}
__global__ __launch_bounds__(256) void colsum_final_kernel(ColsumJobs J) {
    __shared__ float red[4][64];
    const int job = (int)blockIdx.y;
    const int C = J.C[job];
    const int tx = (int)(threadIdx.x & 63), ty = (int)(threadIdx.x >> 6);
    const int c = (int)blockIdx.x * 64 + tx;
    if ((int)blockIdx.x * 64 >= C) return;
    float s0 = 0.f;
    if (c < C) {
        const float* p = J.work + J.poff[job] + c;
        const int R4 = J.R & ~3;
        for (int z = ty; z < R4; z += 4) s0 += p[(long long)z * J.wld];
        if (ty == 0) for (int z = R4; z < J.R; ++z) s0 += p[(long long)z * J.wld];
    }
    red[ty][tx] = s0;
    __syncthreads();
    if (ty == 0 && c < C) J.dst[job][c] = (red[0][tx] + red[1][tx]) + (red[2][tx] + red[3][tx]);
}

enum { TAIL_DELTA = 1, TAIL_GRAD = 2, TAIL_OUT = 4, TAIL_COLSUM = 8, TAIL_L0 = 16, TAIL_SEL = 32 };
struct TailArgs {
    int n_l0, n_grad, n_delta, n_out, n_colsum, n_sel;
    GemmArgs grad;  int grad_gx, grad_gy;
    GemmArgs delta; int delta_gx;
    const int32_t* og_act; const float* og_dsc; const float* og_alast; int og_n, og_H, og_chunk; float* og_partial;
    const uint32_t* l0_boards; const float* l0_delta; int l0_n, l0_H, l0_HS, l0_chunk, l0_nsets, l0_nch; float* l0_partial;
    const uint16_t* l0_planes; long long l0_plane_stride; int l0_kpad, l0_ncb;
    const uint16_t* l0_sel;
    const uint32_t* sel_boards; int sel_n, sel_kpad; uint16_t* sel_out;
    ColsumJobs cj; int cj_gx, cj_gy;
};
template <unsigned KINDS, bool L0MFMA = false>
__global__ __launch_bounds__(256) void td_tail_kernel(const TailArgs a) {
    extern __shared__ __attribute__((aligned(16))) float tail_smem[];
    int b = (int)blockIdx.x;
    if (KINDS & TAIL_L0) {
        if (b < a.n_l0) {
            if (L0MFMA) {
                int rest = b / a.l0_ncb, cb = b % a.l0_ncb, sqg = rest & 3, ch = rest >> 2;
                if ((a.l0_nch & 7) == 0) { ch = b % a.l0_nch; rest = b / a.l0_nch; cb = rest % a.l0_ncb; sqg = rest / a.l0_ncb; }
                l0_grad_mfma_block<0>(a.l0_sel, a.l0_planes, a.l0_plane_stride, a.l0_kpad, a.l0_H, a.l0_chunk, a.l0_partial, sqg, cb, ch,
                                       reinterpret_cast<unsigned char*>(tail_smem));
                return;
            }
            const int per = kSquares * a.l0_nch;
            l0_grad_block(a.l0_boards, a.l0_delta, a.l0_n, a.l0_H, a.l0_HS, a.l0_chunk, a.l0_nsets, a.l0_partial, b % per, a.l0_nch, b / per, tail_smem);
            return;
        }
        b -= a.n_l0;
    }
    if (KINDS & TAIL_GRAD) {
        if (b < a.n_grad) {
            const int per = a.grad_gx * a.grad_gy, nz = a.n_grad / per, z = b % nz, r = b / nz;
            gemm_f32_block<L_MCONTIG, L_MCONTIG, EPI_STORE, 1, 1>(a.grad, r % a.grad_gx, r / a.grad_gx, z, tail_smem, tail_smem + g_tile_floats(64));
            return;
        }
        b -= a.n_grad;
    }
    if (KINDS & TAIL_DELTA) {
        if (b < a.n_delta) {
            gemm_f32_block<L_KCONTIG, L_MCONTIG, EPI_DELTA, 1, 1>(a.delta, b % a.delta_gx, b / a.delta_gx, 0, tail_smem, tail_smem + g_tile_floats(64));
            return;
        }
        b -= a.n_delta;
    }
    if (KINDS & TAIL_OUT) {
        if (b < a.n_out) {
            out_grad_block(a.og_act, a.og_dsc, a.og_alast, a.og_n, a.og_H, a.og_chunk, a.og_partial, b % 24, b / 24, tail_smem);
            return;
        }
        b -= a.n_out;
    }
    if (KINDS & TAIL_COLSUM) {
        if (b < a.n_colsum) {
            const int per = a.cj_gx * a.cj_gy, r = b % per;
            colsum_partial_block(a.cj, r % a.cj_gx, r / a.cj_gx, b / per);
            return;
        }
        b -= a.n_colsum;
    }
    if (KINDS & TAIL_SEL) {
        if (b < a.n_sel) l0_sel_block(a.sel_boards, a.sel_n, a.sel_kpad, a.sel_out, b, reinterpret_cast<uint32_t*>(tail_smem));
    }
}

__device__ __forceinline__ float vadd(const float a, const float b) { return a + b; }
__device__ __forceinline__ float4 vadd(const float4 a, const float4 b) { return make_float4(a.x + b.x, a.y + b.y, a.z + b.z, a.w + b.w); }
__device__ __forceinline__ void vzero(float& a) { a = 0.f; }
__device__ __forceinline__ void vzero(float4& a) { a = make_float4(0.f, 0.f, 0.f, 0.f); }
__device__ __forceinline__ void vpin(float& a) { asm volatile("" : "+v"(a)); }
__device__ __forceinline__ void vpin(float4& a) { asm volatile("" : "+v"(a.x), "+v"(a.y), "+v"(a.z), "+v"(a.w)); }
template <typename T>
struct OrderedSum {
    T s0, s1, s2, s3;
    __device__ __forceinline__ OrderedSum() { vzero(s0); vzero(s1); vzero(s2); vzero(s3); }
    template <int B>
    __device__ __forceinline__ void whole(const T* __restrict__ p, const long long st) {
        static_assert(B % 4 == 0, "whole groups of four");
        T v[B];
#pragma unroll
        for (int u = 0; u < B; ++u) v[u] = p[u * st];
        __builtin_amdgcn_sched_barrier(0);
#pragma unroll
        for (int u = 0; u < B; ++u) vpin(v[u]);
#pragma unroll
        for (int u = 0; u < B; u += 4) { s0 = vadd(s0, v[u]); s1 = vadd(s1, v[u + 1]); s2 = vadd(s2, v[u + 2]); s3 = vadd(s3, v[u + 3]); }
    }
    template <int B>
    __device__ __forceinline__ void part(const T* __restrict__ p, const long long st, const int n) {
        static_assert(B % 4 == 0, "whole groups of four");
        T v[B];
#pragma unroll
        for (int u = 0; u < B; ++u) v[u] = p[min(u, n - 1) * st];
        __builtin_amdgcn_sched_barrier(0);
#pragma unroll
        for (int u = 0; u < B; ++u) vpin(v[u]);
#pragma unroll
        for (int u = 0; u < B; u += 4) {
            if (u + 3 < n) {
                s0 = vadd(s0, v[u]); s1 = vadd(s1, v[u + 1]); s2 = vadd(s2, v[u + 2]); s3 = vadd(s3, v[u + 3]);
            } else if (u < n) {
                s0 = vadd(s0, v[u]);
                if (u + 1 < n) s0 = vadd(s0, v[u + 1]);
                if (u + 2 < n) s0 = vadd(s0, v[u + 2]);
            }
        }
    }
    template <int B>
    __device__ __forceinline__ void run(const T* __restrict__ p, const long long st, int n) {
        for (; n >= B; n -= B, p += B * st) whole<B>(p, st);
        if (n > 0) part<B>(p, st, n);
    }
    __device__ __forceinline__ T total() const { return vadd(vadd(s0, s1), vadd(s2, s3)); }
};
template <typename T>
__device__ __forceinline__ T slab_sum(const T* __restrict__ s, int nslabs, long long st, long long i) {
    constexpr int kBatch = sizeof(T) > sizeof(float) ? 32 : 64;
    const T* p = s + i;
    OrderedSum<T> o;
    if (nslabs == 8) o.template whole<8>(p, st);
    else if (nslabs == 16) o.template whole<16>(p, st);
    else if (kBatch > 32 && nslabs == 32) o.template whole<32>(p, st);
    else o.template run<kBatch>(p, st, nslabs);
    return o.total();
}
__global__ __launch_bounds__(256) void reduce_slabs_kernel(const float* __restrict__ slabs, int nslabs, long long stride, long long len, float* __restrict__ out) {
    for (long long i = (long long)blockIdx.x * blockDim.x + threadIdx.x; i < len; i += (long long)gridDim.x * blockDim.x)
        out[i] = slab_sum(slabs, nslabs, stride, i);
}

struct SegTable {
    float* dst[16];
    const float* src[16];
    long long len[16];
    int nslabs[16];
    long long stride[16];
    uint16_t* dst_bf[16];
    int nseg;
    int reduce_only;
    int vec4[16];
    long long state_off[16];
};

__global__ __launch_bounds__(256) void q_head_finish_kernel(const float* __restrict__ slabs, long long slab_stride, int nslabs, int n, int n_out, int lds_,
                                                            const float* __restrict__ bias, float* __restrict__ q, int ldq) {
    const long long i = (long long)blockIdx.x * blockDim.x + threadIdx.x;
    if (i >= (long long)n * n_out) return;
    const int m = (int)(i / n_out), j = (int)(i % n_out);
    const float* p = slabs + (long long)m * lds_ + j;
    float s = 0.f;
    for (int z = 0; z < nslabs; z += 4) {
        float t = p[z * slab_stride] + p[(z + 1) * slab_stride];
        if (z + 3 < nslabs) t += p[(z + 2) * slab_stride] + p[(z + 3) * slab_stride];
        s = z == 0 ? t : s + t;
    }
    q[(long long)m * ldq + j] = tanhf(bias[j] + s);
}

__global__ void f32_to_bf16_kernel(const float* __restrict__ src, uint16_t* __restrict__ dst, long long n) {
    for (long long i = (long long)blockIdx.x * blockDim.x + threadIdx.x; i < n; i += (long long)gridDim.x * blockDim.x)
        dst[i] = bf16_bits(src[i]);
}
__device__ __forceinline__ void store_bf16(uint16_t* db, long long i, const float v) { db[i] = bf16_bits(v); }
__device__ __forceinline__ uint32_t pack_bf16x2(const float lo, const float hi) { return (uint32_t)bf16_bits(lo) | ((uint32_t)bf16_bits(hi) << 16); }
__device__ __forceinline__ void store_bf16(uint16_t* db, long long i, const float4 v) {
    reinterpret_cast<uint2*>(db)[i] = make_uint2(pack_bf16x2(v.x, v.y), pack_bf16x2(v.z, v.w));
}

struct SoftArgs {
    float* tgt[16];
    uint16_t* tgt_bf[16];
    float tau;
};
__device__ __forceinline__ float soft_elem(const float tau, const float p, const float t) {
#pragma clang fp contract(off)
    const float d = p - t;
    return __builtin_fmaf(tau, d, t);
}
__device__ __forceinline__ float soft_elems(const float tau, const float p, const float t) { return soft_elem(tau, p, t); }
__device__ __forceinline__ float4 soft_elems(const float tau, const float4 p, const float4 t) {
    return make_float4(soft_elem(tau, p.x, t.x), soft_elem(tau, p.y, t.y), soft_elem(tau, p.z, t.z), soft_elem(tau, p.w, t.w));
}

template <class Step>
__device__ __forceinline__ float step_elems(const Step& S, const float w, const float g, float& m, float& v) { return S.elem(w, g, m, v); }
template <class Step>
__device__ __forceinline__ float4 step_elems(const Step& S, const float4 w, const float4 g, float4& m, float4& v) {
// ... 226 lines not shown
```

### cn_chess_ai_amd/workmodel.py

```python

NO = 8100
STATE = 1260
ENV_BYTES_PER_GAME = 2 * (48 + 16) + 360 + 105

PEAK_F32_MFMA_TFLOPS = 157.3
PEAK_BF16_MFMA_TFLOPS = 2500.0
PEAK_HBM_GBS = 8000.0

ROCPROF_NAMES = {
    "l0_forward_gather": "l0_forward_kernel<",
    "l0_forward_gather@select": "l0_forward_kernel<",
    "td_target_delta": "td_delta_kernel(",
    "colmax_reduce": "colmax_reduce_kernel(",
    "sgd_apply": "sgd_segments_kernel(",
    "adam_apply": "adam_segments_kernel(",
    "grad_norm": "grad_norm_kernel(",
    "env_selfplay_step": "env_kernel<2>(",
    "target_sync_copy": "__amd_rocclr_copyBuffer",
    "l0_grad_segsum": "l0_grad_kernel(",
    "out_grad_segsum": "out_grad_kernel(",
    "bias_grad_colsum": "colsum_partial_kernel(",
    "nstep_assemble": "nstep_assemble_kernel(",
    "per_writeback": "per_writeback_kernel(",
    "mirror_stage": "mirror_stage_kernel(",
# ... 2 lines not shown
    "view_boards@select": "view_boards_kernel(",
    "legal_qmax": "legal_qmax_kernel(",
    "legal_side_stage": "legal_side_stage_kernel(",
    "gemm_legal_head": "gemm_f32_kernel<0, 0, 0, 1, 1, 0>(",
}
TAIL_DELTAS, TAIL_DELTAS_SEL, TAIL_L0 = 7, 39, 30


def rocprof_kernel(name, layers, minibatch, td="online", bf16=False, l0_mfma=True, n_games=None):
    Hl, dbl, k = layers[-2], td == "double", len(layers) - 2
    mfma = l0_mfma and layers[1] % 64 == 0 and minibatch >= 256
    if name == "gemm_qmax_screen" or (name == "gemm_qmax_rowmax" and bf16 and Hl in (256, 512)):
        ku = Hl // 256
        return "screen_top2_kernel<%d, %d, %d, 0>(" % (ku, 2 // ku, 0 if name == "gemm_qmax_screen" else 1 if dbl else 2)
    if name == "gemm_qmax_rowmax":
        return "gemm_colmax_persistent_kernel<2, 2, %d, %d>(" % (1 if bf16 else 0, 1 if dbl else 0)
    if name == "gemm_hidden_fwd" and not bf16:
        chains = 3 if dbl else 2
        if minibatch % 128 == 0 and all(h % 128 == 0 for h in layers[2:-1]) and all(h % 32 == 0 for h in layers[1:-2]):
            t128 = (minibatch // 128) * (layers[2] // 128) * chains
            return "gemm_fwd_persistent_kernel<%s, 2>(" % ("2, 2" if t128 >= 512 else "1, 2")
        big = ((minibatch + 127) // 128) * ((layers[2] + 127) // 128) * chains >= 512
        return "gemm_f32_kernel<0, 0, 1, %s, 0>(" % ("2, 2" if big else "1, 1")
    if name == "gemm_hidden_fwd@select" and not bf16:
        if k == 2:
            return "gemm_f32_kernel<0, 0, 4, 1, 1, 0>("
        return ["gemm_f32_kernel<0, 0, 1, 1, 1, 0>(", "gemm_f32_kernel<0, 0, 4, 1, 1, 0>("]
    if name == "qmax_refine":
        return "qmax_refine2_kernel<" if Hl in (256, 512) else "qmax_refine_kernel<"
    if name == "td_tail_l0":
        return "td_tail_kernel<%du, %s>(" % (TAIL_L0, "true" if mfma else "false")
    if name == "td_tail_deltas":
        if k < 2:
            return None
        plain = "td_tail_kernel<%du, false>(" % TAIL_DELTAS
        last = "td_tail_kernel<%du, false>(" % (TAIL_DELTAS_SEL if mfma else TAIL_DELTAS)
        return last if k == 2 else ([plain, last] if mfma else plain)
    if name == "l0_grad_segsum" and mfma:
        return "l0_grad_mfma_kernel<0>("
    if name == "l0_delta_split":
        return "delta_split_kernel("
    if name == "l0_sel_words":
        return "l0_sel_kernel("
    return ROCPROF_NAMES.get(name)


def match_kernel(printed, want):
    p = printed
    for pre in ("void ", "xq::"):
        if p.startswith(pre):
            p = p[len(pre):]
    return p.startswith(want)


def newest_profile_set(root, config=2):
    import glob, os, re
    suffix = "" if config == 2 else "_config%d" % config
    best = None
    for pmc in glob.glob(os.path.join(root, "profiles", "r*_pmc_hbm_traffic.json")):
        m = re.match(r"(r\d+_[a-z0-9]+)(_config\d+)?_pmc_hbm_traffic\.json$", os.path.basename(pmc))
        if not m or (m.group(2) or "") != suffix:
            continue
        stats = os.path.join(root, "profiles", m.group(1) + suffix + "_kernel_stats.csv")
        if os.path.exists(stats) and (best is None or m.group(1) > best[0]):
            best = (m.group(1), stats, pmc)
    return best


def pick_splits(M, N, K):
    tiles = ((M + 63) // 64) * ((N + 63) // 64)
    s = (512 + tiles - 1) // tiles
    s = max(1, min(s, max(1, K // 128), 32))
    chunk = ((K + s - 1) // s + 31) // 32 * 32
    return (K + chunk - 1) // chunk


def step_work(layers, minibatch, n_games, plies=1, bf16=False, bf16_bwd=False, td="online", screened=True, derive=True,
              prioritized=False, l0_mfma=True, optimizer="sgd", grad_clip=False, soft_target=False, n_step=1,
              mirror=False, bootstrap="all", colour_swap=False, view=False):
    if view and colour_swap:
        raise ValueError("view and colour_swap exclude each other (xq_dqn_td_grads_replay refuses the pair)")
    if bootstrap not in ("all", "legal"):
        raise ValueError("bootstrap: 'all' or 'legal'")
    legal = bootstrap == "legal"
    if legal and bf16:
        raise ValueError("bootstrap='legal' needs an fp32 net")
    screened = screened and not legal
    h = list(layers[1:-1])
    H1, Hl, k = h[0], h[-1], len(h)
    B, n = minibatch, n_games
    dbl = td == "double"
    chains = 3 if dbl else 2
    fa = 2 if bf16 else 4
    mm_peak = PEAK_BF16_MFMA_TFLOPS if bf16 else PEAK_F32_MFMA_TFLOPS
    w = {}
    mfma0 = l0_mfma and H1 % 64 == 0 and B >= 256

    def put(name, flops, by, bound, what, peak=None):
        if bound == "mfma":
            pk, unit = (peak or mm_peak), "TFLOP/s"
        else:
            pk, unit = PEAK_HBM_GBS, "GB/s"
        w[name] = dict(flops=float(flops), hbm_bytes=float(by), bound=bound, peak=pk, peak_unit=unit, what=what)

    gathered = chains - (1 if derive and not dbl else (1 if derive and bf16 else 0))
    rows = 32 * gathered + (4 if derive else 0)
    put("l0_forward_gather", 2.0 * B * rows * H1,
        B * (chains * 48 + 48) + STATE * H1 * fa * (2 if dbl or td == "target" else 1) + chains * B * H1 * (4 if not bf16 else 2) +
        (B * H1 * 4 if bf16 else 0) + (96 * Hl * 6 if screened else 0),
        "hbm", "layer 0 of the forward chains as a gather of W0^T rows (L2-resident) + the minibatch's boards; "
               "s' derived from s when the TD rule allows")
    if k >= 2:
        fl = by = 0.0
        for l in range(1, k):
            fl += 2.0 * B * h[l - 1] * h[l] * chains
            by += chains * B * (h[l - 1] * fa + h[l] * (4 if not bf16 else 2)) + h[l - 1] * h[l] * fa * (2 if dbl or td == "target" else 1)
            if bf16:
                by += B * h[l] * 4
        if screened:
            by += B * Hl * 2
        put("gemm_hidden_fwd", fl / (k - 1), by / (k - 1), "mfma",
            "hidden products of the %d forward chains grouped in one launch per layer, bias + tanh epilogue" % chains)
    G = 2 * ((NO + 63) // 64)
    if legal:
        nets = 2 if dbl else 1
        nslabs = min(Hl // 64, 8) if B >= 2048 and Hl % 128 == 0 else 1
        put("gemm_legal_head", 2.0 * B * 96 * Hl, B * Hl * 4 + 96 * Hl * 4 + nslabs * B * 96 * 4, "mfma",
            "pre-activations of outputs 0..95 for s' as k-slabs, per launch (%d per step)" % nets)
        put("legal_qmax", 0.0, B * (48 + 6 + 384.0 * nets * nslabs + 384 + 12), "hbm",
            "move generation for the side to move in s' and the greedy pick over z[to] of its moves: the legal-move bootstrap")
        put("td_target_delta", 4.0 * B * Hl, 2 * B * Hl * 4 + 32 * B, "hbm", "Q(s,a), y, output delta, top hidden delta")
    elif screened:
        put("gemm_qmax_screen", 2.0 * NO * B * Hl, NO * Hl * 2 + B * Hl * 2 + 2 * G * B * 4 + 16 * B * 4 + B * 4, "mfma",
            "exact screen of max_a' Q(s'): all 8100 outputs once on bf16 MFMA, top-2 per 32-output group", PEAK_BF16_MFMA_TFLOPS)
        td_in_refine = Hl == 256 and not prioritized and not bf16_bwd
        by = 16 * B * 4 + 2 * G * B * 4 / 16.0 + B * Hl * 4
        if td_in_refine:
            by += 2 * B * Hl * 4 + 24 * B
        put("qmax_refine", 2.0 * B * Hl * (3 if td_in_refine else 1), by, "hbm",
            "fp32 re-evaluation of the screened candidates" + (" + TD target, output delta and top hidden delta" if td_in_refine else ""))
        if not td_in_refine:
            put("td_target_delta", 4.0 * B * Hl, 2 * B * Hl * 4 + 32 * B, "hbm", "Q(s,a), y, output delta, top hidden delta")
    else:
        fe = 2 if bf16 else 4
        tiles_m = (NO + 127) // 128
        put("gemm_qmax_rowmax", 2.0 * NO * B * Hl, fe * (NO * Hl + B * Hl) + 2 * tiles_m * B * 4 * (2 if dbl else 1), "mfma",
            "%s_a' Q(s') over all 8100 outputs, Q never written" % ("argmax" if dbl else "max"))
        put("colmax_reduce", B * 2.0 * tiles_m, 2 * tiles_m * B * 4 * (2 if dbl else 1) + 4 * B * 4 * 2, "hbm", "fold of the partial maxima")
        put("td_target_delta", 4.0 * B * Hl * (2 if dbl else 1), (2 + (1 if dbl else 0)) * B * Hl * 4 + 32 * B, "hbm",
            "Q(s,a), y, output delta, top hidden delta")
    nch_out = (B + 255) // 256
    out_fl, out_by = 2.0 * B * Hl, B * Hl * 4 + 8 * B + nch_out * (96 * Hl + 96) * 4
    if not bf16:
        if k >= 2:
            fl = by = 0.0
            launches = k - 1
            for l in range(k - 2, -1, -1):
                fl += 2.0 * B * h[l + 1] * h[l]
                by += B * h[l + 1] * 4 + h[l] * h[l + 1] * 4 + 2 * B * h[l] * 4
                if not (k == 2):
                    sp = pick_splits(h[l + 1], h[l], B)
                    fl += 2.0 * h[l + 1] * h[l] * B
                    by += sp * h[l + 1] * h[l] * 4
            fl += out_fl; by += out_by
            put("td_tail_deltas", fl / launches, by / launches, "hbm",
                "fused launch: hidden delta product || weight-gradient product of the layer above || output-layer segmented sums")
        chunk = 2048 if B >= 16384 else 1024
        nch = (B + chunk - 1) // chunk
        kpad = nch * chunk
        if mfma0:
            fl = 2.0 * 80 * 16 * H1 * kpad * 3
            by = 6.0 * H1 * kpad + 4.0 * 96 * kpad + B * H1 * 4 + nch * STATE * H1 * 4
        else:
            fl = 2.0 * B * 32 * H1
            by = B * H1 * 4 + 48 * B + nch * STATE * H1 * 4
        if k == 2:
            sp = pick_splits(h[1], h[0], B)
            fl += 2.0 * h[1] * h[0] * B
            by += B * (h[0] + h[1]) * 4 + sp * h[0] * h[1] * 4
        if k == 1:
            fl += out_fl; by += out_by
        R = max(1, min(64, B // 64))
        by += R * sum(h) * 4
        fl += B * sum(h)
        put("td_tail_l0", fl, by, "hbm",
            "fused launch: layer-0 gradient " + ("as the exact product one-hot^T x delta_0 on the bf16 matrix pipe (3-term split) || "
                                                 if mfma0 else "as per-(square, piece) segmented sums of delta rows || ")
            + ("hidden weight-gradient product || " if k == 2 else "") + "bias column sums")
        if mfma0:
            w["td_tail_l0"]["mfma_bf16_flops"] = 2.0 * 80 * 16 * H1 * kpad * 3
            if "td_tail_deltas" in w:
                w["td_tail_deltas"]["hbm_bytes"] += (6.0 * H1 * kpad + 4.0 * 96 * kpad + 48 * B) / max(1, k - 1)
        slabs = nch * STATE * H1 + nch_out * (96 * Hl + 96) + R * sum(h)
        for l in range(1, k):
            slabs += pick_splits(h[l], h[l - 1], B) * h[l] * h[l - 1]
        touched = STATE * H1 + sum(h[l] * h[l - 1] for l in range(1, k)) + 96 * Hl + 96 + sum(h)
        put("sgd_apply", 2.0 * touched, 4 * (slabs + 2 * touched), "hbm", "ordered sum of every partial-sum slab + SGD step on the touched parameters")
    else:
        eb = 2 if bf16_bwd else 4
        if k >= 2:
            fl = by = 0.0
            for l in range(k - 2, -1, -1):
                fl += 2.0 * B * h[l + 1] * h[l]
                by += B * h[l + 1] * eb + h[l] * h[l + 1] * eb + B * h[l] * (eb + 4 + (2 if bf16_bwd else 0))
            put("gemm_hidden_delta", fl / (k - 1), by / (k - 1), "mfma", "hidden delta product (delta_{l+1} . weight view) (1 - a^2)",
                PEAK_BF16_MFMA_TFLOPS if bf16_bwd else PEAK_F32_MFMA_TFLOPS)
            fl = by = 0.0
            for l in range(1, k):
                sp = max(1, min(16, 256 // max(1, (h[l] // 256) * (h[l - 1] // 128)))) if bf16_bwd else pick_splits(h[l], h[l - 1], B)
                fl += 2.0 * h[l] * h[l - 1] * B
                by += B * (h[l] + h[l - 1]) * eb + sp * h[l] * h[l - 1] * 4
            put("gemm_grad_hidden", fl / (k - 1), by / (k - 1), "mfma", "hidden weight-gradient product, split-K slabs",
                PEAK_BF16_MFMA_TFLOPS if bf16_bwd else PEAK_F32_MFMA_TFLOPS)
        chunk = 2048 if B >= 16384 else 1024
        nch = (B + chunk - 1) // chunk
        if mfma0:
            kpad = nch * chunk
            put("l0_grad_segsum", 2.0 * 80 * 16 * H1 * kpad * 3, 6.0 * H1 * kpad + 4.0 * 96 * kpad + nch * STATE * H1 * 4, "mfma",
                "layer-0 gradient as the exact product one-hot^T x delta_0 on the bf16 matrix pipe (3-term split)", PEAK_BF16_MFMA_TFLOPS)
            put("l0_delta_split", 8.0 * B * H1, B * H1 * 4 + 6.0 * H1 * kpad, "hbm", "delta_0 -> three transposed bf16 planes (hi, mid, lo)")
            put("l0_sel_words", 0.0, 48 * B + 4.0 * 96 * kpad, "hbm", "boards -> selector half-words of the one-hot operand")
        else:
            put("l0_grad_segsum", 2.0 * B * 32 * H1, B * H1 * 4 + 48 * B + nch * STATE * H1 * 4, "hbm",
                "layer-0 gradient as per-(square, piece) segmented sums of delta rows (L2 gather)")
        put("out_grad_segsum", out_fl, out_by, "hbm", "output-layer gradient rows 0..95 as segmented sums by action")
        R = max(1, min(64, B // 64))
        put("bias_grad_colsum", float(B * sum(h)), B * sum(h) * 4 + R * sum(h) * 4, "hbm", "bias gradients: column sums of every hidden delta")
        slabs = nch * STATE * H1 + nch_out * (96 * Hl + 96) + R * sum(h)
        for l in range(1, k):
            sp = max(1, min(16, 256 // max(1, (h[l] // 256) * (h[l - 1] // 128)))) if bf16_bwd else pick_splits(h[l], h[l - 1], B)
            slabs += sp * h[l] * h[l - 1]
        touched = STATE * H1 + sum(h[l] * h[l - 1] for l in range(1, k)) + 96 * Hl + 96 + sum(h)
        put("sgd_apply", 2.0 * touched, 4 * (slabs + 2 * touched) + (2 * touched if bf16 else 0), "hbm",
            "ordered sum of every partial-sum slab + SGD step on the touched parameters (+ their bf16 shadow)")
    if optimizer == "adam":
        sgd = w.pop("sgd_apply")
        put("adam_apply", 12.0 * touched, sgd["hbm_bytes"] + 16 * touched, "hbm",
            "ordered sum of every partial-sum slab + Adam step on the touched parameters and their two moments" + (" (+ their bf16 shadow)" if bf16 else ""))
    elif optimizer != "sgd":
        raise ValueError("optimizer: 'sgd' or 'adam'")
    if grad_clip:
        put("grad_norm", 3.0 * touched + slabs, 4 * (slabs + touched), "hbm",
            "ordered sum of every partial-sum slab into the gradient buffer + fp64 sum of its squares (global-norm clipping)")
        w["adam_apply" if optimizer == "adam" else "sgd_apply"]["hbm_bytes"] -= 4 * (slabs - touched)
    if soft_target:
        a = w["adam_apply" if optimizer == "adam" else "sgd_apply"]
        a["flops"] += 2.0 * touched
        a["hbm_bytes"] += 8 * touched + (2 * touched if bf16 else 0)
        a["what"] += " + soft update of the touched target parameters"
    if n_step > 1:
        put("nstep_assemble", 2.0 * B * (n_step - 1), B * (9.0 * n_step + 4 * 48 + 21), "hbm",
            "gather of the minibatch's n-step transitions into the staging batch the TD step reads")
        if prioritized:
            put("per_writeback", 0.0, 20.0 * B, "hbm", "TD-error priorities of a prioritized n-step draw back to the sampled slots")
    if mirror:
        put("mirror_stage", 0.0, B * (215.0 if n_step == 1 else 201.0), "hbm",
            "left-right reflection of the flagged minibatch rows in the staging batch the TD step reads")
        if prioritized and n_step == 1:
            put("per_writeback", 0.0, 20.0 * B, "hbm", "TD-error priorities of a prioritized mirrored draw back to the sampled slots")
    if colour_swap:
        first = n_step == 1 and not mirror
        put("colour_swap_stage", 0.0, B * ((215.0 if first else 201.0) + ((2.0 if first else 6.0) if legal else 0.0)), "hbm",
            "exchange of the colours (row -> 9 - row, Red <-> Black) of the flagged minibatch rows in the staging batch the TD step reads")
        if prioritized and first:
            put("per_writeback", 0.0, 20.0 * B, "hbm", "TD-error priorities of a prioritized colour-swapped draw back to the sampled slots")
    if view:
        first = n_step == 1 and not mirror
        put("mover_view_stage", 0.0, B * ((218.0 if first else 212.0) + (1.0 if legal else 0.0)), "hbm",
            "mover view of the minibatch in the staging batch the TD step reads: s and the action by who moved, s' by who moves next")
        if prioritized and first:
            put("per_writeback", 0.0, 20.0 * B, "hbm", "TD-error priorities of a prioritized view-mode draw back to the sampled slots")
    if legal and (n_step > 1 or mirror) and not colour_swap and not view:
        put("legal_side_stage", 0.0, 6.0 * B, "hbm", "side to move in s' of every staged row, from the ring's column (legal-move bootstrap)")
    nw =STATE * H1 + sum(h[l] * h[l - 1] for l in range(1, k)) + Hl * NO
    nb = sum(h) + NO
    put("target_sync_copy", 0.0, 8.0 * (nw + nb), "hbm", "updateTargetNetwork(): device copy of all parameters")
    put("l0_forward_gather@select", 2.0 * n * 32 * H1, 48 * n + STATE * H1 * fa + n * H1 * (2 if bf16 else 4), "hbm",
        "layer 0 of Q(s) for the boards of every game (gather)")
    ride = (not bf16) and k >= 2 and n >= 2048 and n % 64 == 0 and Hl % 128 == 0
    if k >= 2:
        fl = by = 0.0
        for l in range(1, k):
            fl += 2.0 * n * h[l - 1] * h[l]
            by += n * h[l - 1] * fa + h[l - 1] * h[l] * fa
            if l == k - 1 and ride:
                fl += 2.0 * n * Hl * 128
                by += (Hl // 64) * n * 96 * 4 + 128 * Hl * 4
            else:
                by += n * h[l] * (2 if bf16 else 4)
        put("gemm_hidden_fwd@select", fl / (k - 1), by / (k - 1), "mfma",
            "hidden products of the select chain" + ("; the last one carries the select head (Q[0..95] as k-slabs)" if ride else ""))
    if not ride:
        put("gemm_q90_select@select", 2.0 * n * Hl * 96, n * Hl * fa + 96 * Hl * fa + n * 96 * 4, "mfma", "select head Q(s)[0..95]")
    if view:
        put("view_boards@select", 0.0, (48.0 + 16.0 + 48.0) * n, "hbm", "view(board, side to move) of every game's board for the select chain")
    put("env_selfplay_step", 0.0, float(ENV_BYTES_PER_GAME) * n, "hbm",
        "fused self-play ply: legal moves, epsilon-greedy select, movePiece, reward, game over, auto-reset, transition -> ring")
    return w


def price(entry, avg_us):
    t = avg_us * 1e-6
    if entry["bound"] == "mfma":
        ach = entry["flops"] / t / 1e12
    else:
        ach = entry["hbm_bytes"] / t / 1e9
    return ach, ach / entry["peak"]
```

Before: 49.07 million.

## Fold bias-gradient column sums into delta and weight-gradient GEMM kernels

Computes the hidden-layer bias gradients as column sums inside the existing GEMMs. The layer-0 sums are formed in the delta GEMM epilogue and the deeper-layer sums during A-operand staging of the fp32 weight-gradient GEMM, which writes per-split slabs that are reduced later. This removes the separate column-sum pass that re-read every delta matrix. When the bf16 layer-0 planes are used it also skips storing delta_0. The cost is extra barriers and LDS reductions in the GEMM kernels, more per-layer pending-slab bookkeeping, and a different summation order for the bias gradients.

New measurement: 49.10 million, median of 2. Within noise of the previous version (+0.1%).

```diff
diff --git a/cn_chess_ai_amd/csrc/xq_dqn.hip b/cn_chess_ai_amd/csrc/xq_dqn.hip
--- a/cn_chess_ai_amd/csrc/xq_dqn.hip
+++ b/cn_chess_ai_amd/csrc/xq_dqn.hip
@@ -120,8 +120,12 @@
     xq_comm* comm = nullptr;
     bool fused_apply = false;
     struct PendingSlab { const float* src = nullptr; int nslabs = 0; long long stride = 0; };
-    PendingSlab pend_w0, pend_hidden[XQ_MAX_LAYERS], pend_wout, pend_bout, pend_bh;
+    PendingSlab pend_w0, pend_hidden[XQ_MAX_LAYERS], pend_wout, pend_bout, pend_bh[XQ_MAX_LAYERS];
     xq::DevBuf<float> bias_work;
+    xq::DevBuf<float> slabs_b0;
+    xq::DevBuf<float> slabs_bh;
+    bool td_fold_b0 = false;
+    bool b0_fold_done = false;
     xq::DevBuf<float> xdense, qfull, tfull;
     xq::DevBuf<uint32_t> hb;
     xq::DevBuf<int32_t> ha;  xq::DevBuf<float> hr;  xq::DevBuf<uint8_t> hd;
@@ -240,6 +244,9 @@
     const long long t128 = (long long)((g.M + 127) / 128) * ((g.N + 127) / 128) * (g.grouped ? groups : splits);
     const bool big = (!force_small && !d->small_tiles && t128 >= 512);
     const double kk = DT == DT_BF16 ? 2.0 * g.K : (double)g.K;
+    const bool grad_form = AL == L_MCONTIG && BL == L_MCONTIG && EPI == EPI_STORE && DT == DT_F32;
+    const bool delta_form = AL == L_KCONTIG && BL == L_MCONTIG && EPI == EPI_DELTA && DT == DT_F32;
+    if (g.colsum && (!(grad_form || delta_form) || big || g.grouped)) return fail(XQ_ERR_RUNTIME, "GEMM %s cannot form column sums", name);
     if (d->tail_open) {
         TailArgs& T = *d->tail;
         const bool is_delta = AL == L_KCONTIG && BL == L_MCONTIG && EPI == EPI_DELTA, is_grad = AL == L_MCONTIG && BL == L_MCONTIG && EPI == EPI_STORE;
@@ -265,6 +272,9 @@
         ps.flops *= groups; ps.bytes *= groups;
     }
     const int gz = g.grouped ? groups : splits;
+    if (g.colsum && grad_form) {
+        hipLaunchKernelGGL(gemm_grad_colsum_kernel, dim3((g.M + 63) / 64, (g.N + 63) / 64, gz), dim3(256), 0, d->cur, g);
+    } else
     if (big) {
         dim3 grid((g.M + 127) / 128, (g.N + 127) / 128, gz);
         hipLaunchKernelGGL((gemm_f32_kernel<AL, BL, EPI, 2, 2, DT>), grid, dim3(256), 0, d->cur, g);
@@ -697,11 +707,17 @@
         g.ldb = (mode == XQ_BACKPROP_REFERENCE) ? d->L[l] : d->L[l + 1];
         g.C = d->deltas[l]; g.ldc = d->L[l + 1];
         g.H = d->acts[l]; g.ldh = d->L[l + 1];
+        const bool tiles64 = d->small_tiles || (long long)((g.M + 127) / 128) * ((g.N + 127) / 128) < 512;
+        if (l == 0 && d->td_fold_b0 && tiles64 && (n % 64) == 0 && (g.N % 64) == 0) {
+            g.colsum = d->slabs_b0;
+            d->b0_fold_done = true;
+        }
         if (l == 0 && l0_mfma_shape(d, n) && (n % l0_chunk_of(n)) == 0) {
             const long long t128 = (long long)((g.M + 127) / 128) * ((g.N + 127) / 128);
             if (d->small_tiles || t128 < 512) {
                 XQ_TRY(ensure_l0_mfma(d, n));
                 g.split_planes = d->l0_planes; g.split_ld = n; g.split_plane_stride = (long long)d->L[1] * n;
+                g.skip_c = g.colsum != nullptr;
                 d->l0_split_done = true;
             }
         }
@@ -747,10 +763,14 @@
     return XQ_OK;
 }
 
+struct FoldedBias { float* dst; float* slabs; xq_dqn::PendingSlab* defer; };
+static bool grad_folds_bias(const xq_dqn* d, int M, int N, int K) { return !grad_bf16_ok(d, M, N, K); }
 template <int AL>
 static int grad_gemm(xq_dqn* d, GemmArgs g, float* dst, const char* name, float* slab_base = nullptr,
-                     xq_dqn::PendingSlab* defer = nullptr, const uint16_t* a_bf = nullptr, const uint16_t* b_bf = nullptr) {
+                     xq_dqn::PendingSlab* defer = nullptr, const uint16_t* a_bf = nullptr, const uint16_t* b_bf = nullptr,
+                     const FoldedBias* fb = nullptr) {
     const bool use_bf = AL == L_MCONTIG && a_bf && b_bf && grad_bf16_ok(d, g.M, g.N, g.K);
+    if (fb && (use_bf || AL != L_MCONTIG)) return fail(XQ_ERR_RUNTIME, "%s: this product cannot form the bias gradient", name);
     const int splits = use_bf ? grad_splits(d, g.M, g.N, g.K) : pick_splits(g.M, g.N, g.K);
     const long long len = (long long)g.M * g.N;
     float* slabs = slab_base;
@@ -765,22 +785,27 @@
         XQ_TRY((launch_bf16_gemm<L_MCONTIG, L_MCONTIG, BG_STORE>(d, b, splits, name)));
     } else {
         g.C = C; g.ldc = g.N; g.slab_stride = slab_stride;
+        if (fb) g.colsum = splits > 1 ? fb->slabs : fb->dst;
         XQ_TRY((launch_gemm<AL, L_MCONTIG, EPI_STORE>(d, g, splits, name, &used, true)));
     }
     if (splits <= 1) return XQ_OK;
-    if (defer) { defer->src = slabs; defer->nslabs = used; defer->stride = len; return XQ_OK; }
-    return launch_reduce_slabs(d, slabs, used, len, dst);
+    if (defer) { defer->src = slabs; defer->nslabs = used; defer->stride = len; }
+    else XQ_TRY(launch_reduce_slabs(d, slabs, used, len, dst));
+    if (!fb) return XQ_OK;
+    if (fb->defer) { fb->defer->src = fb->slabs; fb->defer->nslabs = used; fb->defer->stride = g.M; return XQ_OK; }
+    return launch_reduce_slabs(d, fb->slabs, used, g.M, fb->dst);
 }
 
 struct BiasJobs {
     ColsumJobs J;
-    BiasJobs() { memset(&J, 0, sizeof J); }
-    void add(const float* X, long long ld, int C, float* dst) {
+    xq_dqn::PendingSlab* pend[XQ_MAX_LAYERS + 1];
+    BiasJobs() { memset(&J, 0, sizeof J); memset(pend, 0, sizeof pend); }
+    void add(const float* X, long long ld, int C, float* dst, xq_dqn::PendingSlab* slot = nullptr) {
         const int k = J.njobs++;
-        J.X[k] = X; J.ld[k] = ld; J.C[k] = C; J.dst[k] = dst;
+        J.X[k] = X; J.ld[k] = ld; J.C[k] = C; J.dst[k] = dst; pend[k] = slot;
     }
 };
-static int bias_grads(xq_dqn* d, BiasJobs& bj, int n, xq_dqn::PendingSlab* defer = nullptr) {
+static int bias_grads(xq_dqn* d, BiasJobs& bj, int n, bool defer = false) {
     ColsumJobs& J = bj.J;
     if (J.njobs == 0) return XQ_OK;
     J.n = n;
@@ -793,7 +818,8 @@
     off *= J.R;
     XQ_TRY(d->bias_work.reserve((size_t)off));
     J.work = d->bias_work;
-    if (defer) { defer->src = J.work; defer->nslabs = J.R; defer->stride = J.wld; }
+    if (defer)
+        for (int k = 0; k < J.njobs; ++k) { bj.pend[k]->src = J.work + J.poff[k]; bj.pend[k]->nslabs = J.R; bj.pend[k]->stride = J.wld; }
     double tot = 0;
     for (int k = 0; k < J.njobs; ++k) tot += (double)n * J.C[k];
     if (d->tail_open) {
@@ -966,7 +992,11 @@
     for (int l = 0; l + 1 < d->nl; ++l) { d->g_bh[l] = off; off += (size_t)d->L[l + 1]; }
     d->n_grads_td = off;
 }
-static bool td_step_pending(const xq_dqn* d) { return d->pend_w0.nslabs > 0 || d->pend_wout.nslabs > 0 || d->pend_bh.nslabs > 0; }
+static bool td_step_pending(const xq_dqn* d) {
+    for (const auto& p : d->pend_bh) if (p.nslabs > 0) return true;
+    return d->pend_w0.nslabs > 0 || d->pend_wout.nslabs > 0;
+}
+static_assert(1 + (XQ_MAX_LAYERS - 2) + 1 + (XQ_MAX_LAYERS - 1) + 1 <= 16, "SegTable / SoftArgs hold 16 segments");
 template <class F>
 static void for_td_segments(xq_dqn* d, F f) {
     const bool bf = d->bf16();
@@ -974,7 +1004,7 @@
     f(d->w0t(0), bf ? d->wl_bf(0, 0) : nullptr, d->g_w0, (long long)d->L[0] * d->L[1], d->pend_w0);
     for (int l = 1; l < top; ++l) f(d->wl(0, l), bf ? d->wl_bf(0, l) : nullptr, d->g_wh[l], (long long)d->L[l] * d->L[l + 1], d->pend_hidden[l]);
     f(d->wl(0, top), bf ? d->wl_bf(0, top) : nullptr, d->g_wout, 96LL * d->hlast(), d->pend_wout);
-    f(d->bl(0, 0), (uint16_t*)nullptr, d->g_bh[0], (long long)d->bo[top], d->pend_bh);
+    for (int l = 0; l < top; ++l) f(d->bl(0, l), (uint16_t*)nullptr, d->g_bh[l], (long long)d->L[l + 1], d->pend_bh[l]);
     f(d->bl(0, top), (uint16_t*)nullptr, d->g_bout, 96LL, d->pend_bout);
 }
 static void soft_td_segments(const xq_dqn* d, SoftArgs* Z) {
@@ -985,7 +1015,7 @@
     add(d->w0t(1), bf ? d->wl_bf(1, 0) : nullptr);
     for (int l = 1; l < top; ++l) add(d->wl(1, l), bf ? d->wl_bf(1, l) : nullptr);
     add(d->wl(1, top), bf ? d->wl_bf(1, top) : nullptr);
-    add(d->bl(1, 0), nullptr);
+    for (int l = 0; l < top; ++l) add(d->bl(1, l), nullptr);
     add(d->bl(1, top), nullptr);
 }
 enum class ParamWrite { ONLINE_WHOLE, TARGET_HOST, TARGET_COPY, TARGET_BLEND, TD_SEGMENTS, BF16_SHADOW };
@@ -1317,6 +1347,7 @@
                        d->cur, d->qfull, d->tfull, total, d->tfull);
     XQ_HIP(hipGetLastError());
     const float* dout = d->tfull;
+    d->td_fold_b0 = false;
     XQ_TRY(hidden_deltas(d, n, dout, NO, NO, mode));
     float* gw = d->grads_full;
     float* gb = d->grads_full + d->nw;
@@ -1373,6 +1404,7 @@
     bool defer;
     int out_chunks;  long long len_out;  size_t out_lds;
     size_t off_out, off_h[XQ_MAX_LAYERS];
+    size_t off_b[XQ_MAX_LAYERS];
 };
 static const int kOutGradChunk = 256;
 static int plan_gradients(xq_dqn* d, int n, bool defer, GradPlan* P) {
@@ -1393,10 +1425,19 @@
         return at;
     };
     P->off_out = place(P->out_chunks, (size_t)P->len_out);
-    for (int l = d->nl - 2; l >= 1; --l) P->off_h[l] = place(grad_splits(d, d->L[l + 1], d->L[l], n), (size_t)d->L[l + 1] * (size_t)d->L[l]);
+    size_t need_b = 0;
+    for (int l = d->nl - 2; l >= 1; --l) {
+        const int splits = grad_splits(d, d->L[l + 1], d->L[l], n);
+        P->off_h[l] = place(splits, (size_t)d->L[l + 1] * (size_t)d->L[l]);
+        P->off_b[l] = need_b;
+        if (grad_folds_bias(d, d->L[l + 1], d->L[l], n)) need_b += (size_t)splits * (size_t)d->L[l + 1];
+    }
     XQ_TRY(d->slabs.reserve(need));
-    d->pend_w0 = d->pend_wout = d->pend_bout = d->pend_bh = xq_dqn::PendingSlab();
+    XQ_TRY(d->slabs_bh.reserve(need_b));
+    if (d->td_fold_b0) XQ_TRY(d->slabs_b0.reserve((size_t)((n + 63) / 64) * (size_t)d->L[1]));
+    d->pend_w0 = d->pend_wout = d->pend_bout = xq_dqn::PendingSlab();
     for (auto& p : d->pend_hidden) p = xq_dqn::PendingSlab();
+    for (auto& p : d->pend_bh) p = xq_dqn::PendingSlab();
     return XQ_OK;
 }
 
@@ -1430,13 +1471,25 @@
     g.A = d->deltas[l]; g.lda = d->L[l + 1];
     g.B = outs[l - 1]; g.ldb = d->L[l];
     const bool bf = d->bf16_bwd();
+    const FoldedBias fb = {G + d->g_bh[l], d->slabs_bh.p + P.off_b[l], P.defer ? &d->pend_bh[l] : nullptr};
     return grad_gemm<L_MCONTIG>(d, g, G + d->g_wh[l], "gemm_grad_hidden", d->slabs + P.off_h[l], P.defer ? &d->pend_hidden[l] : nullptr,
-                                bf ? d->deltas_bf[l].p : nullptr, bf ? d->acts_bf[l - 1].p : nullptr);
+                                bf ? d->deltas_bf[l].p : nullptr, bf ? d->acts_bf[l - 1].p : nullptr,
+                                grad_folds_bias(d, g.M, g.N, g.K) ? &fb : nullptr);
 }
 static int hidden_bias_gradients(xq_dqn* d, const GradPlan& P, int n, float* G) {
+    const bool b0_folded = d->b0_fold_done;
+    d->b0_fold_done = false;
+    if (b0_folded) {
+        const int H = d->L[1], rows = n / 64;
+        if (P.defer) { d->pend_bh[0].src = d->slabs_b0; d->pend_bh[0].nslabs = rows; d->pend_bh[0].stride = H; }
+        else XQ_TRY(launch_reduce_slabs(d, d->slabs_b0, rows, H, G + d->g_bh[0]));
+    }
     BiasJobs bj;
-    for (int l = 0; l <= d->nl - 2; ++l) bj.add(d->deltas[l], d->L[l + 1], d->L[l + 1], G + d->g_bh[l]);
-    return bias_grads(d, bj, n, P.defer ? &d->pend_bh : nullptr);
+    for (int l = 0; l <= d->nl - 2; ++l) {
+        if (l == 0 ? b0_folded : grad_folds_bias(d, d->L[l + 1], d->L[l], n)) continue;
+        bj.add(d->deltas[l], d->L[l + 1], d->L[l + 1], G + d->g_bh[l], &d->pend_bh[l]);
+    }
+    return bias_grads(d, bj, n, P.defer);
 }
 
 static int side_gradients(xq_dqn* d, const GradPlan& P, int n, float* const* outs, float* G) {
@@ -1869,6 +1922,7 @@
         return fail(XQ_ERR_INVALID_ARGUMENT, "the legal-move bootstrap needs the side to move in s': use xq_dqn_td_grads_sided / xq_dqn_td_update_host_sided");
     d->legal_rows = 0;
     d->l0_split_done = d->l0_sel_done = false;
+    d->td_fold_b0 = d->nl >= 3; d->b0_fold_done = false;
     d->late_gate = d->comm != nullptr && tail_eligible(d, n) &&
                    (d->exchange_overlap == 1 ||
                     (d->exchange_overlap < 0 && (d->exch_calibrated ? d->exch_late : comm_world(d->comm) > 1)));
diff --git a/cn_chess_ai_amd/csrc/xq_gemm.hip.h b/cn_chess_ai_amd/csrc/xq_gemm.hip.h
--- a/cn_chess_ai_amd/csrc/xq_gemm.hip.h
+++ b/cn_chess_ai_amd/csrc/xq_gemm.hip.h
@@ -63,6 +63,8 @@
     const float* head_W; long long head_ldw; float* head_slabs; long long head_slab_stride; int head_ld;
     int libm_tanh;
     uint16_t* split_planes; long long split_plane_stride; int split_ld;
+    int skip_c;
+    float* colsum;
 };
 
 template <int LAYOUT, int ROWS, bool FAST, int J0 = 0, int J1 = ROWS / 32>
@@ -215,9 +217,9 @@
     }
 }
 
-template <int AL, int BL, int TM, int TN, bool FAST, int DT = DT_F32>
+template <int AL, int BL, int TM, int TN, bool FAST, int DT = DT_F32, bool CS = false>
 __device__ __forceinline__ void gemm_mainloop(const GemmArgs& g, float* __restrict__ As, float* __restrict__ Bs, int m0, int n0,
-                                              int kbeg, int kend, f32x16 (&acc)[TM][TN]) {
+                                              int kbeg, int kend, f32x16 (&acc)[TM][TN], float4* cs = nullptr) {
     constexpr int BM = 64 * TM, BN = 64 * TN;
     const int tid = (int)threadIdx.x & 255;
     const int lane = tid & 63, wid = tid >> 6;
@@ -232,6 +234,10 @@
         __syncthreads();
         stage_store<AL, BM>(As, va);
         stage_store<BL, BN>(Bs, vb);
+        if (CS) {
+#pragma unroll
+            for (int j = 0; j < BM / 32; ++j) { cs->x += va[j].x; cs->y += va[j].y; cs->z += va[j].z; cs->w += va[j].w; }
+        }
         __syncthreads();
         if (k0 + GBK < kend) {
             stage_load<AL, BM, FAST>(g, g.A, g.lda, g.a_vec, m0, g.M, k0 + GBK, kend, va);
@@ -293,9 +299,10 @@
     }
 }
 
-template <int AL, int BL, int EPI, int TM, int TN, int DT = DT_F32>
+template <int AL, int BL, int EPI, int TM, int TN, int DT = DT_F32, bool COLSUM = false>
 __device__ __forceinline__ void gemm_f32_block(const GemmArgs& g_in, int bx, int by, int bz, float* __restrict__ As, float* __restrict__ Bs) {
     constexpr int BM = 64 * TM, BN = 64 * TN;
+    static_assert(!COLSUM || (AL == L_MCONTIG && EPI == EPI_STORE && TM == 1 && DT == DT_F32), "column sums: the 64-row m-contiguous A operand");
     GemmArgs g = g_in;
     if (g_in.grouped && bz >= 1) {
         const int k = bz - 1;
@@ -319,6 +326,20 @@
             for (int q = 0; q < 16; ++q) acc[i][j][q] = 0.f;
 
     const bool interior = (m0 + BM <= g.M) && (n0 + BN <= g.N) && (((kend - kbeg) & (GBK - 1)) == 0) && g.a_vec && g.b_vec;
+    if (COLSUM && by == 0 && g.colsum != nullptr) {
+        float4 cs = make_float4(0.f, 0.f, 0.f, 0.f);
+        if (interior) gemm_mainloop<AL, BL, TM, TN, true, DT, true>(g, As, Bs, m0, n0, kbeg, kend, acc, &cs);
+        else gemm_mainloop<AL, BL, TM, TN, false, DT, true>(g, As, Bs, m0, n0, kbeg, kend, acc, &cs);
+        __syncthreads();
+        *reinterpret_cast<float4*>(&As[(tid >> 4) * 64 + (tid & 15) * 4]) = cs;
+        __syncthreads();
+        if (tid < 64 && m0 + tid < g.M) {
+            float s[4];
+#pragma unroll
+            for (int j = 0; j < 4; ++j) s[j] = ((As[j * 64 + tid] + As[(j + 4) * 64 + tid]) + As[(j + 8) * 64 + tid]) + As[(j + 12) * 64 + tid];
+            g.colsum[(long long)bz * g.M + m0 + tid] = (s[0] + s[1]) + (s[2] + s[3]);
+        }
+    } else
     if (interior) gemm_mainloop<AL, BL, TM, TN, true, DT>(g, As, Bs, m0, n0, kbeg, kend, acc);
     else gemm_mainloop<AL, BL, TM, TN, false, DT>(g, As, Bs, m0, n0, kbeg, kend, acc);
 
@@ -439,12 +460,23 @@
                     float v = acc[i][j][q];
                     if (EPI == EPI_BIAS_TANH) v = g.libm_tanh ? tanhf(v + bias) : tanh_hidden(v + bias);
                     if (EPI == EPI_DELTA) v = v * (1.f - hv[q] * hv[q]);
-                    Cz[(long long)(mb + (q & 3) + 8 * (q >> 2)) * g.ldc + n] = v;
+                    if (!(EPI == EPI_DELTA && g.split_planes && g.skip_c)) Cz[(long long)(mb + (q & 3) + 8 * (q >> 2)) * g.ldc + n] = v;
                     if (EPI == EPI_BIAS_TANH && g.Cb) {
                         const int row = mb + (q & 3) + 8 * (q >> 2);
                         g.Cb[g.cb_frag ? scr_afrag_index(row, n, g.N) : (long long)row * g.ldcb + n] = bf16_bits(v);
                     }
                     if (EPI == EPI_DELTA) hv[q] = v;
+                }
+                if (EPI == EPI_DELTA && TM == 1 && TN == 1 && BL == L_MCONTIG && g.colsum) {
+                    float* xs = Bs + 32 * (64 + 4);
+                    float s = (((hv[0] + hv[1]) + (hv[2] + hv[3])) + ((hv[4] + hv[5]) + (hv[6] + hv[7]))) +
+                              (((hv[8] + hv[9]) + (hv[10] + hv[11])) + ((hv[12] + hv[13]) + (hv[14] + hv[15])));
+                    s += __shfl_xor(s, 32, 64);
+                    if (h == 0) xs[wm * 64 + wn * 32 + r] = s;
+                    asm volatile("s_waitcnt lgkmcnt(0)" ::: "memory");
+                    __builtin_amdgcn_s_barrier();
+                    asm volatile("" ::: "memory");
+                    if (tid < 64) g.colsum[(long long)bx * g.N + n0 + tid] = xs[tid] + xs[64 + tid];
                 }
                 if (EPI == EPI_DELTA && g.split_planes) {
                     const int m32 = m0 + wm * 32 * TM + i * 32;
@@ -510,6 +542,11 @@
     __shared__ __attribute__((aligned(16))) float As[g_tile_floats(64 * TM)];
     __shared__ __attribute__((aligned(16))) float Bs[g_tile_floats(EPI == EPI_HEAD ? 128 : 64 * TN)];
     gemm_f32_block<AL, BL, EPI, TM, TN, DT>(g_in, (int)blockIdx.x, (int)blockIdx.y, (int)blockIdx.z, As, Bs);
+}
+__global__ __launch_bounds__(256) __attribute__((amdgpu_waves_per_eu(1, 2))) void gemm_grad_colsum_kernel(const GemmArgs g_in) {
+    __shared__ __attribute__((aligned(16))) float As[g_tile_floats(64)];
+    __shared__ __attribute__((aligned(16))) float Bs[g_tile_floats(64)];
+    gemm_f32_block<L_MCONTIG, L_MCONTIG, EPI_STORE, 1, 1, DT_F32, true>(g_in, (int)blockIdx.x, (int)blockIdx.y, (int)blockIdx.z, As, Bs);
 }
 
 enum { CM_MAX = 0, CM_ARG = 1, CM_TOP2 = 2 };
diff --git a/cn_chess_ai_amd/csrc/xq_tail.hip.h b/cn_chess_ai_amd/csrc/xq_tail.hip.h
--- a/cn_chess_ai_amd/csrc/xq_tail.hip.h
+++ b/cn_chess_ai_amd/csrc/xq_tail.hip.h
@@ -352,7 +352,7 @@
     if (KINDS & TAIL_GRAD) {
         if (b < a.n_grad) {
             const int per = a.grad_gx * a.grad_gy, nz = a.n_grad / per, z = b % nz, r = b / nz;
-            gemm_f32_block<L_MCONTIG, L_MCONTIG, EPI_STORE, 1, 1>(a.grad, r % a.grad_gx, r / a.grad_gx, z, tail_smem, tail_smem + g_tile_floats(64));
+            gemm_f32_block<L_MCONTIG, L_MCONTIG, EPI_STORE, 1, 1, DT_F32, true>(a.grad, r % a.grad_gx, r / a.grad_gx, z, tail_smem, tail_smem + g_tile_floats(64));
             return;
         }
         b -= a.n_grad;
diff --git a/cn_chess_ai_amd/workmodel.py b/cn_chess_ai_amd/workmodel.py
--- a/cn_chess_ai_amd/workmodel.py
+++ b/cn_chess_ai_amd/workmodel.py
@@ -178,12 +178,18 @@
     nch_out = (B + 255) // 256
     out_fl, out_by = 2.0 * B * Hl, B * Hl * 4 + 8 * B + nch_out * (96 * Hl + 96) * 4
     if not bf16:
+        chunk = 2048 if B >= 16384 else 1024
+        b0_epi = k >= 2 and B % 64 == 0 and h[0] % 64 == 0 and ((B + 127) // 128) * ((h[0] + 127) // 128) < 512
         if k >= 2:
             fl = by = 0.0
             launches = k - 1
             for l in range(k - 2, -1, -1):
                 fl += 2.0 * B * h[l + 1] * h[l]
                 by += B * h[l + 1] * 4 + h[l] * h[l + 1] * 4 + 2 * B * h[l] * 4
+                if l == 0 and mfma0 and B % chunk == 0:
+                    by -= B * h[0] * 4
+                if l == 0 and b0_epi:
+                    by += (B // 64) * h[0] * 4
                 if not (k == 2):
                     sp = pick_splits(h[l + 1], h[l], B)
                     fl += 2.0 * h[l + 1] * h[l] * B
@@ -191,7 +197,6 @@
             fl += out_fl; by += out_by
             put("td_tail_deltas", fl / launches, by / launches, "hbm",
                 "fused launch: hidden delta product || weight-gradient product of the layer above || output-layer segmented sums")
-        chunk = 2048 if B >= 16384 else 1024
         nch = (B + chunk - 1) // chunk
         kpad = nch * chunk
         if mfma0:
@@ -207,17 +212,22 @@
         if k == 1:
             fl += out_fl; by += out_by
         R = max(1, min(64, B // 64))
-        by += R * sum(h) * 4
-        fl += B * sum(h)
+        bias_slabs = (B // 64 if b0_epi else R) * h[0] + sum(pick_splits(h[l], h[l - 1], B) * h[l] for l in range(1, k))
+        if not b0_epi:
+            by += R * h[0] * 4
+            fl += B * h[0]
+        if k == 2:
+            by += pick_splits(h[1], h[0], B) * h[1] * 4
         put("td_tail_l0", fl, by, "hbm",
             "fused launch: layer-0 gradient " + ("as the exact product one-hot^T x delta_0 on the bf16 matrix pipe (3-term split) || "
                                                  if mfma0 else "as per-(square, piece) segmented sums of delta rows || ")
-            + ("hidden weight-gradient product || " if k == 2 else "") + "bias column sums")
+            + ("hidden weight-gradient product with gb_1 folded in" if k == 2 else "")
+            + ("" if b0_epi else " || column sums of delta_0"))
         if mfma0:
             w["td_tail_l0"]["mfma_bf16_flops"] = 2.0 * 80 * 16 * H1 * kpad * 3
             if "td_tail_deltas" in w:
                 w["td_tail_deltas"]["hbm_bytes"] += (6.0 * H1 * kpad + 4.0 * 96 * kpad + 48 * B) / max(1, k - 1)
-        slabs = nch * STATE * H1 + nch_out * (96 * Hl + 96) + R * sum(h)
+        slabs = nch * STATE * H1 + nch_out * (96 * Hl + 96) + bias_slabs
         for l in range(1, k):
             slabs += pick_splits(h[l], h[l - 1], B) * h[l] * h[l - 1]
         touched = STATE * H1 + sum(h[l] * h[l - 1] for l in range(1, k)) + 96 * Hl + 96 + sum(h)
@@ -251,11 +261,17 @@
                 "layer-0 gradient as per-(square, piece) segmented sums of delta rows (L2 gather)")
         put("out_grad_segsum", out_fl, out_by, "hbm", "output-layer gradient rows 0..95 as segmented sums by action")
         R = max(1, min(64, B // 64))
-        put("bias_grad_colsum", float(B * sum(h)), B * sum(h) * 4 + R * sum(h) * 4, "hbm", "bias gradients: column sums of every hidden delta")
-        slabs = nch * STATE * H1 + nch_out * (96 * Hl + 96) + R * sum(h)
+        on_bf = lambda l: bf16_bwd and h[l] % 256 == 0 and h[l - 1] % 128 == 0 and B >= 64 and B % 64 == 0
+        b0_epi = (k >= 2 and not bf16_bwd and B % 64 == 0 and h[0] % 64 == 0
+                  and ((B + 127) // 128) * ((h[0] + 127) // 128) < 512)
+        cols = (0 if b0_epi else h[0]) + sum(h[l] for l in range(1, k) if on_bf(l))
+        if cols:
+            put("bias_grad_colsum", float(B * cols), B * cols * 4 + R * cols * 4, "hbm",
+                "bias gradients: column sums of the hidden deltas whose gradient product does not form them")
+        slabs = nch * STATE * H1 + nch_out * (96 * Hl + 96) + R * cols + ((B // 64) * h[0] if b0_epi else 0)
         for l in range(1, k):
             sp = max(1, min(16, 256 // max(1, (h[l] // 256) * (h[l - 1] // 128)))) if bf16_bwd else pick_splits(h[l], h[l - 1], B)
-            slabs += sp * h[l] * h[l - 1]
+            slabs += sp * h[l] * h[l - 1] + (0 if on_bf(l) else sp * h[l])
         touched = STATE * H1 + sum(h[l] * h[l - 1] for l in range(1, k)) + 96 * Hl + 96 + sum(h)
         put("sgd_apply", 2.0 * touched, 4 * (slabs + 2 * touched) + (2 * touched if bf16 else 0), "hbm",
             "ordered sum of every partial-sum slab + SGD step on the touched parameters (+ their bf16 shadow)")
```
